# Toptachamann/Linear_Programming_Solver

Measured on AMD Instinct MI355X. Metric: simplex_pivots_per_sec, higher is better.
Workload: dtype f64

## Files before the change

### include/lpx.h

```cpp
#ifndef LPX_H
#define LPX_H

#include <stddef.h>
#include <stdint.h>

#ifdef __cplusplus
extern "C" {
#endif

#define LPX_ABI_VERSION 5

typedef enum lpx_status {
  LPX_OPTIMAL = 0,
  LPX_UNBOUNDED = 1,
  LPX_INFEASIBLE = 2,
  LPX_AUX_UNBOUNDED = 3,
  LPX_NO_DEGENERATE_PIVOT = 4,
  LPX_BAD_ARGUMENT = 5,
  LPX_RESTORE_INDEX_FAULT = 6,
  LPX_DEVICE_ERROR = 7,
  LPX_DIVIDE_BY_ZERO = 8,
  LPX_PIVOT_LIMIT = 9
} lpx_status;

const char* lpx_status_message(int status);
const char* lpx_last_error(void);
int lpx_abi_version(void);
int lpx_device_count(void);

typedef struct lpx_state lpx_state;

int lpx_state_create(int32_t m_local, int32_t n, const double* A, int64_t lda, const double* b,
                     const double* c, double v, const int32_t* perm, int32_t row0, int32_t m_global,
                     int device, lpx_state** out);
int lpx_state_create_from_device(int32_t m_local, int32_t n, const double* dA, int64_t lda,
                                 const double* db, const double* dc, double v, const int32_t* perm,
                                 int32_t row0, int32_t m_global, int device, lpx_state** out);
void lpx_state_destroy(lpx_state* s);
int lpx_state_set_stream(lpx_state* s, void* hip_stream);

int lpx_state_use_masked_stream(lpx_state* s, int32_t reserve_units, void** stream_out);

int lpx_state_set_pricing(lpx_state* s, int32_t pricing);

int lpx_get_entering(lpx_state* s, int32_t* entering);
int lpx_get_leaving(lpx_state* s, int32_t entering, int32_t* leaving, double* ratio);
int lpx_pivot(lpx_state* s, int32_t entering, int32_t leaving);

typedef enum lpx_option {
  LPX_OPT_BLOCK = 0,
  LPX_OPT_CHAIN = 1,
  LPX_OPT_OVERLAP = 2,
  LPX_OPT_OVERLAP_SERIAL = 3,
  LPX_OPT_OVERLAP_MASK = 4,
  LPX_OPT_CHAIN_WGS = 5,
  LPX_OPT_CHAIN_FENCES = 6,
  LPX_OPT_SWEEP_ROWS = 7,
  LPX_OPT_NT = 8,
  LPX_OPT_BATCH = 9,
  LPX_OPT_CHAIN_TRACE = 10,
  LPX_OPT_UPDATE_U = 11,
  LPX_OPT_UPDATE_ROWS = 12,
  LPX_OPT_A2_OFFSET = 13,
  LPX_OPT_SWEEP_FORM = 14,
  LPX_OPT_MULTI_ONEHOP = 15,
  LPX_OPT_SWEEP_CUS = 16,
  LPX_OPT_CHAIN_CUS = 17,
  LPX_OPT_FUSED = 18,
  LPX_OPT_CHAIN_FORM = 19,
  LPX_OPT_FIXUP_SIDE = 20,
  LPX_OPT_COUNT = 21
} lpx_option;
int lpx_state_set_option(lpx_state* s, int32_t key, int64_t value);
int lpx_state_get_option(const lpx_state* s, int32_t key, int64_t* value);

typedef struct lpx_state_info {
  int32_t block;
  int32_t chain_wgs;
  int32_t chain_wgs_requested;
  int32_t chain_resident_max;
  int32_t chain_blocks_per_cu;
  int32_t chain_stream_masked;
  int32_t chain_xcd_mask;
  int32_t sweep_xcd_mask;
  int32_t overlapped;
  int32_t nontemporal;
  int32_t sweep_rows;
  int32_t sweep_kernel;
  int32_t multi_onehop;
  int32_t sweep_clock_mhz;
  int32_t sweep_cus;
  int32_t arith_fused;
} lpx_state_info;
int lpx_state_get_info(lpx_state* s, lpx_state_info* out);
const char* lpx_sweep_kernel_name(int32_t code);
int lpx_state_read_chain_trace(lpx_state* s, int64_t* ticks, int32_t cap, int32_t* ndecisions);
int lpx_state_read_chain_trace_fine(lpx_state* s, int64_t* ticks, int32_t cap, int32_t* ndecisions, int32_t* stamps);

int lpx_state_set_block(lpx_state* s, int32_t pivots_per_sweep);
int lpx_state_get_block(const lpx_state* s);

int lpx_simplex_loop(lpx_state* s, int64_t max_pivots, int64_t* pivots_done, int32_t* status,
                     int32_t* track_slot);

int lpx_state_read(lpx_state* s, double* A, int64_t lda, double* b, double* c, double* v,
                   int32_t* perm);
int lpx_state_dims(const lpx_state* s, int32_t* m_local, int32_t* n, int32_t* row0, int32_t* m_global);
int lpx_state_checksum(lpx_state* s, uint64_t out[3]);

int lpx_profile_enable(lpx_state* s, int enable);
int lpx_profile_read(lpx_state* s, int64_t* launches, double* total_ms);

#define LPX_CAND_HEADER 8
int lpx_shard_begin(lpx_state* s, int64_t max_pivots, int32_t track_slot);
int lpx_shard_propose(lpx_state* s, double* d_candidate);
int lpx_shard_commit(lpx_state* s, const double* d_gathered, int32_t nranks);
int lpx_shard_probe(lpx_state* s, const double* d_gathered, int32_t nranks);
int lpx_shard_set_comm_stream(lpx_state* s, void* hip_stream);
int lpx_shard_set_pipeline(lpx_state* s, int32_t mode);
int lpx_shard_peek(lpx_state* s, double* d_candidate, int32_t slot, int32_t pending);
int lpx_shard_decide(lpx_state* s, const double* d_gathered, int32_t nranks, int32_t slot);
int lpx_shard_update(lpx_state* s, int32_t slot);
int lpx_shard_block_peek(lpx_state* s, double* d_candidate, int32_t slot);
int lpx_shard_block_decide(lpx_state* s, const double* d_gathered, int32_t nranks, int32_t slot);
int lpx_shard_block_sweep(lpx_state* s, int32_t nslots);
#define LPX_RUNNING (-1)
int lpx_shard_poll(lpx_state* s, int64_t* pivots_done, int32_t* status);

typedef struct lpx_solve_result {
  int32_t status;
  int32_t phase1_used;
  double objective;
  double objective_rounded;
  char objective_text[64];
  int64_t pivots_phase1;
  int64_t pivots_phase2;
  int32_t x0_slot;
  int32_t reserved;
  double seconds_total;
  double seconds_pivots;
} lpx_solve_result;

typedef struct lpx_solve_options {
  int32_t device;
  int32_t has_variable_names;
  int64_t max_pivots;
  const int32_t* restore_order;
  int32_t* perm_out;
  double* x_out;
  lpx_state** keep_state;
  int32_t pricing;
  int32_t restore_order_len;
  int32_t fused;
  int32_t reserved;
} lpx_solve_options;

int lpx_solve(int32_t m, int32_t n, const double* A, int64_t lda, const double* b, const double* c,
              int32_t maximize, const lpx_solve_options* opts, lpx_solve_result* result);

#define LPX_MAX_DEVICES 8
typedef struct lpx_multi lpx_multi;
int lpx_multi_create(int32_t m, int32_t n, const double* A, int64_t lda, const double* b, const double* c, double v,
                     const int32_t* perm, const int32_t* devices, int32_t n_dev, lpx_multi** out);
void lpx_multi_destroy(lpx_multi* s);
int lpx_multi_set_option(lpx_multi* s, int32_t key, int64_t value);
int lpx_multi_set_pricing(lpx_multi* s, int32_t pricing);
int lpx_multi_get_entering(lpx_multi* s, int32_t* entering);
int lpx_multi_get_leaving(lpx_multi* s, int32_t entering, int32_t* leaving, double* ratio);
int lpx_multi_pivot(lpx_multi* s, int32_t entering, int32_t leaving);
int lpx_multi_simplex_loop(lpx_multi* s, int64_t max_pivots, int64_t* pivots_done, int32_t* status,
                           int32_t* track_slot);
int lpx_multi_read(lpx_multi* s, double* A, int64_t lda, double* b, double* c, double* v, int32_t* perm);
int lpx_multi_checksum(lpx_multi* s, uint64_t out[3]);
int lpx_multi_profile_enable(lpx_multi* s, int enable);
int lpx_multi_profile_read(lpx_multi* s, int32_t shard, int64_t* launches, double* total_ms);
int lpx_multi_get_info(lpx_multi* s, lpx_state_info* out);
int lpx_solve_multi(int32_t m, int32_t n, const double* A, int64_t lda, const double* b, const double* c,
                    int32_t maximize, const lpx_solve_options* opts, const int32_t* devices, int32_t n_dev,
                    lpx_solve_result* result);

#define LPX_BATCH_LDS_BYTES 163840
int64_t lpx_batch_lds_bytes(int32_t m, int32_t n);
int64_t lpx_batch_solve_lds_bytes(int32_t m, int32_t n);

typedef struct lpx_batch lpx_batch;
int lpx_batch_create(int32_t count, int32_t m_max, int32_t n_max, const int32_t* m, const int32_t* n,
                     const double* A, int64_t lda, int64_t strideA, const double* b, const double* c,
                     const double* v, const int32_t* perm, int device, lpx_batch** out);
void lpx_batch_destroy(lpx_batch* s);
int lpx_batch_set_option(lpx_batch* s, int32_t key, int64_t value);
int lpx_batch_set_pricing(lpx_batch* s, int32_t pricing);
int lpx_batch_simplex_loop(lpx_batch* s, int64_t max_pivots, int64_t* pivots_done, int32_t* status, int32_t* track_slot);
int lpx_batch_read(lpx_batch* s, int32_t index, double* A, int64_t lda, double* b, double* c, double* v, int32_t* perm);
int lpx_batch_count(const lpx_batch* s);
int lpx_batch_shape(const lpx_batch* s, int32_t index, int32_t* m, int32_t* n);
int lpx_batch_solve(lpx_batch* s, const int32_t* maximize, int64_t max_pivots, const int32_t* restore_order,
                    const int32_t* restore_order_len, lpx_solve_result* results);
int lpx_solve_batch(int32_t count, int32_t m_max, int32_t n_max, const int32_t* m, const int32_t* n,
                    const double* A, int64_t lda, int64_t strideA, const double* b, const double* c,
                    const int32_t* maximize, const lpx_solve_options* opts, lpx_solve_result* results,
                    int32_t* n_in_batch);

int lpx_batch_solutions(lpx_batch* s, double* x_out, int32_t* perm_out);
int lpx_solve_batch_all(int32_t count, int32_t m_max, int32_t n_max, const int32_t* m, const int32_t* n,
                        const double* A, int64_t lda, int64_t strideA, const double* b, const double* c,
                        const int32_t* maximize, const lpx_solve_options* opts, lpx_solve_result* results,
                        double* x_out, int32_t* perm_out, int32_t* n_in_batch);

typedef struct lpx_scenarios lpx_scenarios;
int lpx_scenarios_create(int32_t m, int32_t n, const double* A, int64_t lda, int device, lpx_scenarios** out);
void lpx_scenarios_destroy(lpx_scenarios* s);
int lpx_scenarios_set_option(lpx_scenarios* s, int32_t key, int64_t value);
int lpx_scenarios_set_pricing(lpx_scenarios* s, int32_t pricing);
int lpx_scenarios_solve(lpx_scenarios* s, int32_t count, const double* b, int64_t ldb, const double* c, int64_t ldc,
                        const int32_t* maximize, int64_t max_pivots, const int32_t* restore_order, int32_t restore_order_len,
                        lpx_solve_result* results, double* x_out, int32_t* perm_out);
int lpx_solve_scenarios(int32_t m, int32_t n, const double* A, int64_t lda, int32_t count, const double* b, int64_t ldb,
                        const double* c, int64_t ldc, const int32_t* maximize, const lpx_solve_options* opts,
                        lpx_solve_result* results, double* x_out, int32_t* perm_out);

#define LPX_ROUTE_COLD 0
#define LPX_ROUTE_PRIMAL 1
#define LPX_ROUTE_DUAL 2
int lpx_scenarios_set_basis(lpx_scenarios* s, const int32_t* basis, int32_t* crash_pivots_out);
// ... 20 lines not shown
```

### linear_programming_solver_amd/_lib.py

```python
import ctypes as C
import os

_HERE = os.path.dirname(os.path.abspath(__file__))
LIB_PATH = os.environ.get("LPX_LIB_PATH") or os.path.join(_HERE, "liblpx.so")

OPTIMAL, UNBOUNDED, INFEASIBLE, AUX_UNBOUNDED, NO_DEGENERATE_PIVOT, BAD_ARGUMENT, RESTORE_INDEX_FAULT, \
    DEVICE_ERROR, DIVIDE_BY_ZERO, PIVOT_LIMIT = range(10)
CAND_HEADER = 8
BATCH_LDS_BYTES = 163840
ROUTES = ("cold", "primal", "dual")
PRICING = {"reference": 0, "first-positive": 0, "dantzig": 1, 0: 0, 1: 1}

OPTIONS = {"block": 0, "chain": 1, "overlap": 2, "overlap_serial": 3, "overlap_mask": 4, "chain_wgs": 5,
           "chain_fences": 6, "sweep_rows": 7, "nt": 8, "batch": 9, "chain_trace": 10, "update_u": 11,
           "update_rows": 12, "a2_offset": 13, "sweep_form": 14, "multi_onehop": 15, "sweep_cus": 16, "chain_cus": 17,
           "fused": 18, "chain_form": 19, "fixup_side": 20}

DEFAULT_FUSED = None


def set_default_arithmetic(mode):
    global DEFAULT_FUSED
    if mode not in ("auto", "plain", "fused"):
        raise ValueError('arithmetic mode is "auto", "plain" or "fused"')
    prev = "auto" if DEFAULT_FUSED is None else "fused" if DEFAULT_FUSED else "plain"
    DEFAULT_FUSED = None if mode == "auto" else mode == "fused"
    return prev


dp = C.POINTER(C.c_double)
ip = C.POINTER(C.c_int32)
i64p = C.POINTER(C.c_int64)


class SolveResult(C.Structure):
    _fields_ = [
        ("status", C.c_int32),
        ("phase1_used", C.c_int32),
        ("objective", C.c_double),
        ("objective_rounded", C.c_double),
        ("objective_text", C.c_char * 64),
        ("pivots_phase1", C.c_int64),
        ("pivots_phase2", C.c_int64),
        ("x0_slot", C.c_int32),
        ("reserved", C.c_int32),
        ("seconds_total", C.c_double),
        ("seconds_pivots", C.c_double),
    ]


class StateInfo(C.Structure):
    _fields_ = [(k, C.c_int32) for k in (
        "block", "chain_wgs", "chain_wgs_requested", "chain_resident_max", "chain_blocks_per_cu",
        "chain_stream_masked", "chain_xcd_mask", "sweep_xcd_mask", "overlapped", "nontemporal", "sweep_rows",
        "sweep_kernel", "multi_onehop", "sweep_clock_mhz", "sweep_cus", "arith_fused")]


class SolveOptions(C.Structure):
    _fields_ = [
        ("device", C.c_int32),
        ("has_variable_names", C.c_int32),
        ("max_pivots", C.c_int64),
        ("restore_order", ip),
        ("perm_out", ip),
        ("x_out", dp),
        ("keep_state", C.POINTER(C.c_void_p)),
        ("pricing", C.c_int32),
        ("restore_order_len", C.c_int32),
        ("fused", C.c_int32),
        ("reserved", C.c_int32),
    ]


SYMBOLS = [
    ("lpx_status_message", C.c_char_p, [C.c_int]),
    ("lpx_last_error", C.c_char_p, []),
    ("lpx_abi_version", C.c_int, []),
    ("lpx_device_count", C.c_int, []),
    ("lpx_state_create", C.c_int, [C.c_int32, C.c_int32, dp, C.c_int64, dp, dp, C.c_double, ip, C.c_int32,
                                   C.c_int32, C.c_int, C.POINTER(C.c_void_p)]),
    ("lpx_state_create_from_device", C.c_int, [C.c_int32, C.c_int32, C.c_void_p, C.c_int64, C.c_void_p,
                                               C.c_void_p, C.c_double, ip, C.c_int32, C.c_int32, C.c_int,
                                               C.POINTER(C.c_void_p)]),
    ("lpx_state_destroy", None, [C.c_void_p]),
    ("lpx_state_set_stream", C.c_int, [C.c_void_p, C.c_void_p]),
    ("lpx_state_use_masked_stream", C.c_int, [C.c_void_p, C.c_int32, C.POINTER(C.c_void_p)]),
    ("lpx_state_set_pricing", C.c_int, [C.c_void_p, C.c_int32]),
    ("lpx_state_set_block", C.c_int, [C.c_void_p, C.c_int32]),
    ("lpx_state_get_block", C.c_int, [C.c_void_p]),
    ("lpx_state_set_option", C.c_int, [C.c_void_p, C.c_int32, C.c_int64]),
    ("lpx_state_get_option", C.c_int, [C.c_void_p, C.c_int32, i64p]),
    ("lpx_state_get_info", C.c_int, [C.c_void_p, C.POINTER(StateInfo)]),
    ("lpx_sweep_kernel_name", C.c_char_p, [C.c_int32]),
    ("lpx_state_read_chain_trace", C.c_int, [C.c_void_p, i64p, C.c_int32, ip]),
    ("lpx_state_read_chain_trace_fine", C.c_int, [C.c_void_p, i64p, C.c_int32, ip, ip]),
    ("lpx_get_entering", C.c_int, [C.c_void_p, ip]),
    ("lpx_get_leaving", C.c_int, [C.c_void_p, C.c_int32, ip, dp]),
    ("lpx_pivot", C.c_int, [C.c_void_p, C.c_int32, C.c_int32]),
    ("lpx_simplex_loop", C.c_int, [C.c_void_p, C.c_int64, i64p, ip, ip]),
    ("lpx_state_read", C.c_int, [C.c_void_p, dp, C.c_int64, dp, dp, dp, ip]),
    ("lpx_state_dims", C.c_int, [C.c_void_p, ip, ip, ip, ip]),
    ("lpx_state_checksum", C.c_int, [C.c_void_p, C.POINTER(C.c_uint64)]),
    ("lpx_profile_enable", C.c_int, [C.c_void_p, C.c_int]),
    ("lpx_profile_read", C.c_int, [C.c_void_p, i64p, dp]),
    ("lpx_shard_begin", C.c_int, [C.c_void_p, C.c_int64, C.c_int32]),
    ("lpx_shard_propose", C.c_int, [C.c_void_p, C.c_void_p]),
    ("lpx_shard_commit", C.c_int, [C.c_void_p, C.c_void_p, C.c_int32]),
    ("lpx_shard_probe", C.c_int, [C.c_void_p, C.c_void_p, C.c_int32]),
    ("lpx_shard_set_comm_stream", C.c_int, [C.c_void_p, C.c_void_p]),
    ("lpx_shard_set_pipeline", C.c_int, [C.c_void_p, C.c_int32]),
    ("lpx_shard_peek", C.c_int, [C.c_void_p, C.c_void_p, C.c_int32, C.c_int32]),
    ("lpx_shard_decide", C.c_int, [C.c_void_p, C.c_void_p, C.c_int32, C.c_int32]),
    ("lpx_shard_update", C.c_int, [C.c_void_p, C.c_int32]),
    ("lpx_shard_block_peek", C.c_int, [C.c_void_p, C.c_void_p, C.c_int32]),
    ("lpx_shard_block_decide", C.c_int, [C.c_void_p, C.c_void_p, C.c_int32, C.c_int32]),
    ("lpx_shard_block_sweep", C.c_int, [C.c_void_p, C.c_int32]),
    ("lpx_shard_poll", C.c_int, [C.c_void_p, i64p, ip]),
    ("lpx_multi_create", C.c_int, [C.c_int32, C.c_int32, dp, C.c_int64, dp, dp, C.c_double, ip, ip, C.c_int32,
                                   C.POINTER(C.c_void_p)]),
    ("lpx_multi_destroy", None, [C.c_void_p]),
    ("lpx_multi_set_option", C.c_int, [C.c_void_p, C.c_int32, C.c_int64]),
    ("lpx_multi_set_pricing", C.c_int, [C.c_void_p, C.c_int32]),
    ("lpx_multi_get_entering", C.c_int, [C.c_void_p, ip]),
    ("lpx_multi_get_leaving", C.c_int, [C.c_void_p, C.c_int32, ip, dp]),
    ("lpx_multi_pivot", C.c_int, [C.c_void_p, C.c_int32, C.c_int32]),
    ("lpx_multi_simplex_loop", C.c_int, [C.c_void_p, C.c_int64, i64p, ip, ip]),
    ("lpx_multi_read", C.c_int, [C.c_void_p, dp, C.c_int64, dp, dp, dp, ip]),
    ("lpx_multi_checksum", C.c_int, [C.c_void_p, C.POINTER(C.c_uint64)]),
    ("lpx_multi_profile_enable", C.c_int, [C.c_void_p, C.c_int]),
    ("lpx_multi_profile_read", C.c_int, [C.c_void_p, C.c_int32, i64p, dp]),
    ("lpx_multi_get_info", C.c_int, [C.c_void_p, C.POINTER(StateInfo)]),
    ("lpx_solve_multi", C.c_int, [C.c_int32, C.c_int32, dp, C.c_int64, dp, dp, C.c_int32, C.POINTER(SolveOptions),
                                  ip, C.c_int32, C.POINTER(SolveResult)]),
    ("lpx_solve", C.c_int, [C.c_int32, C.c_int32, dp, C.c_int64, dp, dp, C.c_int32, C.POINTER(SolveOptions),
                            C.POINTER(SolveResult)]),
    ("lpx_restore_initial_lp", C.c_int, [C.c_void_p, dp, C.c_int32, C.c_int32, ip, C.c_int32]),
    ("lpx_java_default_name_order", C.c_int, [C.c_int32, ip]),
    ("lpx_transpose", C.c_int, [C.c_int32, C.c_int32, dp, C.c_int64, dp, C.c_int64, C.c_int]),
    ("lpx_batch_lds_bytes", C.c_int64, [C.c_int32, C.c_int32]),
    ("lpx_batch_create", C.c_int, [C.c_int32, C.c_int32, C.c_int32, ip, ip, dp, C.c_int64, C.c_int64, dp, dp, dp, ip,
                                   C.c_int, C.POINTER(C.c_void_p)]),
    ("lpx_batch_destroy", None, [C.c_void_p]),
    ("lpx_batch_set_option", C.c_int, [C.c_void_p, C.c_int32, C.c_int64]),
    ("lpx_batch_set_pricing", C.c_int, [C.c_void_p, C.c_int32]),
    ("lpx_batch_simplex_loop", C.c_int, [C.c_void_p, C.c_int64, i64p, ip, ip]),
    ("lpx_batch_read", C.c_int, [C.c_void_p, C.c_int32, dp, C.c_int64, dp, dp, dp, ip]),
    ("lpx_batch_count", C.c_int, [C.c_void_p]),
    ("lpx_solve_batch", C.c_int, [C.c_int32, C.c_int32, C.c_int32, ip, ip, dp, C.c_int64, C.c_int64, dp, dp, ip,
                                  C.POINTER(SolveOptions), C.POINTER(SolveResult), ip]),
    ("lpx_batch_solve_lds_bytes", C.c_int64, [C.c_int32, C.c_int32]),
    ("lpx_batch_shape", C.c_int, [C.c_void_p, C.c_int32, ip, ip]),
    ("lpx_batch_solutions", C.c_int, [C.c_void_p, dp, ip]),
    ("lpx_batch_solve", C.c_int, [C.c_void_p, ip, C.c_int64, ip, ip, C.POINTER(SolveResult)]),
    ("lpx_solve_batch_all", C.c_int, [C.c_int32, C.c_int32, C.c_int32, ip, ip, dp, C.c_int64, C.c_int64, dp, dp, ip,
                                      C.POINTER(SolveOptions), C.POINTER(SolveResult), dp, ip, ip]),
    ("lpx_scenarios_create", C.c_int, [C.c_int32, C.c_int32, dp, C.c_int64, C.c_int, C.POINTER(C.c_void_p)]),
    ("lpx_scenarios_destroy", None, [C.c_void_p]),
    ("lpx_scenarios_set_option", C.c_int, [C.c_void_p, C.c_int32, C.c_int64]),
    ("lpx_scenarios_set_pricing", C.c_int, [C.c_void_p, C.c_int32]),
    ("lpx_scenarios_solve", C.c_int, [C.c_void_p, C.c_int32, dp, C.c_int64, dp, C.c_int64, ip, C.c_int64, ip, C.c_int32,
                                      C.POINTER(SolveResult), dp, ip]),
    ("lpx_solve_scenarios", C.c_int, [C.c_int32, C.c_int32, dp, C.c_int64, C.c_int32, dp, C.c_int64, dp, C.c_int64, ip,
                                      C.POINTER(SolveOptions), C.POINTER(SolveResult), dp, ip]),
    ("lpx_scenarios_set_basis", C.c_int, [C.c_void_p, ip, ip]),
    ("lpx_scenarios_resolve", C.c_int, [C.c_void_p, C.c_int32, dp, C.c_int64, dp, C.c_int64, ip, C.c_int64, ip, C.c_int32,
                                        C.POINTER(SolveResult), dp, ip, ip]),
    ("lpx_solve_scenarios_from_basis", C.c_int, [C.c_int32, C.c_int32, dp, C.c_int64, ip, C.c_int32, dp, C.c_int64, dp,
                                                 C.c_int64, ip, C.POINTER(SolveOptions), C.POINTER(SolveResult), dp, ip,
                                                 ip]),
# ... 30 lines not shown
```

### linear_programming_solver_amd/csrc/lpx_dispatch.cpp

```cpp
#include "lpx_kernels.h"

#include <algorithm>

namespace lpxk {

#define LPX_PICK(B, f) ((B).fused ? fused::f : plain::f)

void launch_entering(const Buffers& B, int n, hipStream_t s, const LoopStart& start) { LPX_PICK(B, launch_entering)(B, n, s, start); }
void launch_entering_dantzig(const Buffers& B, int n, bool seed, hipStream_t s, const LoopStart& start) {
  LPX_PICK(B, launch_entering_dantzig)(B, n, seed, s, start);
}
void launch_ratio_gather(const Buffers& B, int m_local, int row0, const Geometry& g, int forced_e, hipStream_t s) {
  LPX_PICK(B, launch_ratio_gather)(B, m_local, row0, g, forced_e, s);
}
void launch_reduce_partials(const Buffers& B, const Geometry& g, hipStream_t s) {
  LPX_PICK(B, launch_reduce_partials)(B, g, s);
}
void launch_select_pivot(const Buffers& B, int n, int m_global, const Geometry& g, int forced_e, int forced_l,
                         hipStream_t s) {
  LPX_PICK(B, launch_select_pivot)(B, n, m_global, g, forced_e, forced_l, s);
}
void launch_update(const Buffers& B, int m_local, int n, int row0, const Geometry& g, bool nontemporal,
                   const double* prow, const LpxCtl* up, double* A_out, double* b_out, hipStream_t s) {
  LPX_PICK(B, launch_update)(B, m_local, n, row0, g, nontemporal, prow, up, A_out, b_out, s);
}
void launch_propose(const Buffers& B, int n, int row0, int m_local, const Geometry& g, double* d_candidate,
                    hipStream_t s) {
  LPX_PICK(B, launch_propose)(B, n, row0, m_local, g, d_candidate, s);
}
void launch_commit(const Buffers& B, int n, int m_global, const double* d_gathered, int nranks, double* prow,
                   LpxCtl* up, int up_parity, hipStream_t s) {
  LPX_PICK(B, launch_commit)(B, n, m_global, d_gathered, nranks, prow, up, up_parity, s);
}
void launch_peek(const Buffers& B, int n, int m_local, int row0, const double* prow_t, const double* col_t,
                 double* col_next, const LpxCtl* pend, double* d_candidate, hipStream_t s) {
  LPX_PICK(B, launch_peek)(B, n, m_local, row0, prow_t, col_t, col_next, pend, d_candidate, s);
}
void launch_block_peek(const Buffers& B, const BlockRing& R, int n, int m_local, int row0, int np, double* d_candidate,
                       hipStream_t s) {
  LPX_PICK(B, launch_block_peek)(B, R, n, m_local, row0, np, d_candidate, s);
}
void launch_block_decide(const Buffers& B, const BlockRing& R, int n, int m_global, const double* d_gathered, int nranks,
                         int slot, hipStream_t s) {
  LPX_PICK(B, launch_block_decide)(B, R, n, m_global, d_gathered, nranks, slot, s);
}
int launch_block_chain(const Buffers& B, const BlockRing& R, int n, int m, int nb, int half, int old_half, int n_old,
                       int b_from_tableau, int seq, int dantzig, int wgs, int fences, bool trace, LpxCtl* host_snap,
                       hipStream_t s, const MgPeers* mg, hipEvent_t stop) {
  return LPX_PICK(B, launch_block_chain)(B, R, n, m, nb, half, old_half, n_old, b_from_tableau, seq, dantzig, wgs, fences, trace,
                                  host_snap, s, mg, stop);
}
void preload_block_kernels(const Buffers& B, const BlockRing& R, hipStream_t s) {
  plain::preload_block_kernels(B, R, s);
  fused::preload_block_kernels(B, R, s);
}
unsigned* sweep_fail_word(const BlockRing& R, int64_t ld) { return plain::sweep_fail_word(R, ld); }
int64_t sweep_ticket_slots(int64_t ld) { return plain::sweep_ticket_slots(ld); }
int chain_blocks_per_cu() { return std::min(plain::chain_blocks_per_cu(), fused::chain_blocks_per_cu()); }
const char* sweep_kernel_name(int code) { return plain::sweep_kernel_name(code); }
int launch_block_sweep(const Buffers& B, const BlockRing& R, int n, int m_local, int row0, int K, int rows_per_wg,
                       bool nt, hipStream_t s, const double* A_src, const double* b_src, hipEvent_t after_sweep, int cus,
                       int form, int* kernel_used, const FixSide* side, hipEvent_t stop, hipEvent_t before_sweep) {
  return LPX_PICK(B, launch_block_sweep)(B, R, n, m_local, row0, K, rows_per_wg, nt, s, A_src, b_src, after_sweep, cus,
                                         form, kernel_used, side, stop, before_sweep);
}
void launch_fill_column(double* A, int64_t ld, int m, int col, double value, hipStream_t s) {
  plain::launch_fill_column(A, ld, m, col, value, s);
}
void launch_drop_column(double* A, int64_t ld, int m, int n_old, int col, hipStream_t s) {
  plain::launch_drop_column(A, ld, m, n_old, col, s);
}
void launch_restore_objective(const Buffers& B, int n, const RestoreEntry* d_entries, int n_entries, hipStream_t s) {
  LPX_PICK(B, launch_restore_objective)(B, n, d_entries, n_entries, s);
}
void launch_checksum(const Buffers& B, int m_local, int n, int row0, unsigned long long* d_out3, hipStream_t s) {
  plain::launch_checksum(B, m_local, n, row0, d_out3, s);
}
hipError_t launch_batch_simplex(const BatchArgs& a, hipStream_t s) {
  return a.fused ? fused::launch_batch_simplex(a, s) : plain::launch_batch_simplex(a, s);
}
int batch_blocks_per_cu(int threads, int lds_bytes) {
  return std::min(plain::batch_blocks_per_cu(threads, lds_bytes), fused::batch_blocks_per_cu(threads, lds_bytes));
}
hipError_t launch_batch_solve(const BatchSolveArgs& a, hipStream_t s) {
  return a.fused ? fused::launch_batch_solve(a, s) : plain::launch_batch_solve(a, s);
}
int batch_solve_blocks_per_cu(int threads, int lds_bytes) {
  return std::min(plain::batch_solve_blocks_per_cu(threads, lds_bytes), fused::batch_solve_blocks_per_cu(threads, lds_bytes));
}
hipError_t launch_batch_scenarios(const BatchScenarioArgs& a, hipStream_t s) {
  return a.fused ? fused::launch_batch_scenarios(a, s) : plain::launch_batch_scenarios(a, s);
}
int batch_scenarios_blocks_per_cu(int threads, int lds_bytes) {
  return std::min(plain::batch_scenarios_blocks_per_cu(threads, lds_bytes), fused::batch_scenarios_blocks_per_cu(threads, lds_bytes));
}
hipError_t launch_scenarios_crash(const ScenarioCrashArgs& a, hipStream_t s) {
  return a.fused ? fused::launch_scenarios_crash(a, s) : plain::launch_scenarios_crash(a, s);
}
hipError_t launch_batch_resolve(const BatchResolveArgs& a, hipStream_t s) {
  return a.fused ? fused::launch_batch_resolve(a, s) : plain::launch_batch_resolve(a, s);
}
int batch_resolve_blocks_per_cu(int threads, int lds_bytes) {
  return std::min(plain::batch_resolve_blocks_per_cu(threads, lds_bytes), fused::batch_resolve_blocks_per_cu(threads, lds_bytes));
}
void launch_transpose(const double* dA, int64_t lda, double* dAt, int64_t ldat, int m, int n, hipStream_t s) {
  plain::launch_transpose(dA, lda, dAt, ldat, m, n, s);
}

}
```

### linear_programming_solver_amd/csrc/lpx_engine.cpp

```cpp
#include <hip/hip_runtime.h>

#include <algorithm>
#include <chrono>
#include <cmath>
#include <cstdio>
#include <cstdlib>
#include <cstring>
#include <string>
#include <vector>

#include "../../include/lpx.h"
#include "lpx_kernels.h"
#include "lpx_internal.h"

using lpxk::Buffers;
using lpxk::Geometry;
using lpxk::LpxCtl;
using lpxk::RatioRow;

thread_local std::string g_last_error;

int fail(int status, const std::string& msg) {
  g_last_error = msg;
  return status;
}

extern "C" const char* lpx_status_message(int status) {
  switch (status) {
    case LPX_UNBOUNDED: return "This linear program is unbounded";
    case LPX_INFEASIBLE: return "This linear program is infeasible";
    case LPX_AUX_UNBOUNDED: return "Auxiliary lp is unbounded";
    case LPX_NO_DEGENERATE_PIVOT: return "Can't perform degenerate pivot";
    case LPX_BAD_ARGUMENT: return "IllegalArgumentException";
    case LPX_RESTORE_INDEX_FAULT: return "ArrayIndexOutOfBoundsException";
    case LPX_DEVICE_ERROR: return "HIP device error";
    case LPX_DIVIDE_BY_ZERO: return "Division by zero";
    default: return "";
  }
}

extern "C" const char* lpx_last_error(void) { return g_last_error.c_str(); }
extern "C" int lpx_abi_version(void) { return LPX_ABI_VERSION; }

extern "C" int lpx_device_count(void) {
  int n = 0;
  if (hipGetDeviceCount(&n) != hipSuccess) return -1;
  return n;
}

static int64_t round_up(int64_t x, int64_t q) { return (x + q - 1) / q * q; }

struct OptionSpec { const char* env; int64_t dflt, lo, hi; };
static const OptionSpec kOptionSpec[LPX_OPT_COUNT] = {
    {"LPX_BLOCK", 0, 0, lpxk::kBlockMax},
    {"LPX_CHAIN", 1, 0, 1},
    {"LPX_OVERLAP", 1, 0, 1},
    {"LPX_OVERLAP_SERIAL", 0, 0, 1},
    {"LPX_OVERLAP_MASK", 1, 0, 1},
    {"LPX_CHAIN_WGS", 0, 0, lpxk::kChainMaxWgs},
    {"LPX_CHAIN_FENCES", 2, 0, 3},
    {"LPX_SWEEP_ROWS", 0, 0, 8192},
    {"LPX_NT", -1, -1, 1},
    {"LPX_BATCH", 0, 0, 4096},
    {"LPX_CHAIN_TRACE", 0, 0, 1},
    {"LPX_U", 1, 1, 4},
    {"LPX_ROWS_PER_TILE", 2, 2, 256},
    {"LPX_A2_OFFSET", 512, 0, 1 << 20},
    {"LPX_SWEEP_FORM", 0, 0, 4},
    {"LPX_MULTI_ONEHOP", 0, 0, 1},
    {"LPX_SWEEP_CUS", 0, 0, 256},
    {"LPX_CHAIN_CUS", 0, 0, 16},
    {"LPX_FUSED", 2, 0, 2},
    {"LPX_CHAIN_FORM", 1, 0, 1},
    {"LPX_FIXUP_SIDE", 4, 0, 4},
};

static const int64_t* env_defaults() {
  static int64_t d[LPX_OPT_COUNT];
  static const bool once = [] {
    for (int k = 0; k < LPX_OPT_COUNT; k++) {
      const OptionSpec& sp = kOptionSpec[k];
      int64_t v = sp.dflt;
      const char* e = getenv(sp.env);
      if (e && *e) v = std::max(sp.lo, std::min(sp.hi, (int64_t)atoll(e)));
      d[k] = v;
    }
    return true;
  }();
  (void)once;
  return d;
}

void resolve_arithmetic(lpx_state* s) {
  const int64_t v = s->opt[LPX_OPT_FUSED];
  const double bytes = 8.0 * (double)s->m * (double)s->B.ld;
  const bool by_size = s->m == s->m_global && !s->multi_shard && bytes >= 0.5 * 1073741824.0;
  s->B.fused = v == 1 || (v == 2 && by_size);
}

static Geometry choose_geometry(int m, int64_t ld, const int64_t* opt) {
  Geometry g{};
  int U = (int)opt[LPX_OPT_UPDATE_U];
  if (U != 1 && U != 2 && U != 4) U = 1;
  g.U = U;
  const int W = 512 * U;
  g.nstrips = (int)((ld + W - 1) / W);
  int R = (int)opt[LPX_OPT_UPDATE_ROWS];
  if (R < 2) R = 2;
  if (R > 256) R = 256;
  if (R & 1) R += 1;
  g.rows_per_tile = R;
  g.ntiles = m > 0 ? (m + R - 1) / R : 0;
  return g;
}

static void apply_layout_options(lpx_state* s) {
  s->g = choose_geometry(s->m, s->B.ld, s->opt);
  const int64_t bytes = (int64_t)s->m * s->B.ld * 8;
  const int64_t nt = s->opt[LPX_OPT_NT];
  s->nontemporal = nt < 0 ? bytes > (192ll << 20) : nt != 0;
  s->info.nontemporal = s->nontemporal ? 1 : 0;
}

static int enqueue_ctl_fetch(lpx_state* s) {
  HIP_TRY(hipMemcpyAsync(s->h_ctl, s->B.ctl, sizeof(LpxCtl), hipMemcpyDeviceToHost, s->stream));
  unsigned* const fw = lpxk::sweep_fail_word(s->R, s->B.ld);
  unsigned* const h_fw = reinterpret_cast<unsigned*>(reinterpret_cast<char*>(s->h_ctl) + sizeof(LpxCtl));
  if (fw) HIP_TRY(hipMemcpyAsync(h_fw, fw, sizeof(unsigned), hipMemcpyDeviceToHost, s->stream));
  return 0;
}
static int check_fetched_fail_word(lpx_state* s) {
  unsigned* const fw = lpxk::sweep_fail_word(s->R, s->B.ld);
  unsigned* const h_fw = reinterpret_cast<unsigned*>(reinterpret_cast<char*>(s->h_ctl) + sizeof(LpxCtl));
  if (fw && *h_fw) {
    const unsigned f = *h_fw;
    *h_fw = 0;
    (void)hipMemset(fw, 0, sizeof(unsigned));
    return fail(LPX_DEVICE_ERROR, "k_sweep64_pull: a hand-over wait between the two stages hit its spin bound (code " +
                                      std::to_string(f) + "); the tableau of this handle is not valid");
  }
  return 0;
}
int sync_ctl_to_host(lpx_state* s) {
  if (int rc = enqueue_ctl_fetch(s)) return rc;
  HIP_TRY(hipStreamSynchronize(s->stream));
  return check_fetched_fail_word(s);
}

int push_ctl(lpx_state* s) {
  HIP_TRY(hipMemcpyAsync(s->B.ctl, s->h_ctl, sizeof(LpxCtl), hipMemcpyHostToDevice, s->stream));
  return 0;
}

static void free_block_ring(lpx_state* s) {
  (void)hipFree(s->R.prow);
  (void)hipFree(s->R.col);
  (void)hipFree(s->R.col0);
  (void)hipFree(s->R.row0);
  (void)hipFree(s->R.up);
  (void)hipFree(s->R.chain_part_a);
  (void)hipFree(s->R.chain_part_b);
  (void)hipFree(s->R.chain_bar);
  (void)hipFree(s->R.chain_own_col);
  (void)hipFree(s->R.chain_own_prow);
  (void)hipFree(s->R.chain_own_dvc);
  (void)hipFree(s->R.chain_own_b);
  (void)hipFree(s->R.chain_own_rs);
  (void)hipFree(s->R.chain_dbg);
  (void)hipFree(s->R.census);
  (void)hipFree(const_cast<double*>(s->R.zeros));
  (void)hipFree(s->R.tickets);
  (void)hipFree(s->R.sweep_fail);
  (void)hipFree(s->R.clk);
  (void)hipFree(s->R.col_packed);
  (void)hipFree(s->R.fix_col);
  (void)hipFree(s->R.fix_row);
  (void)hipFree(s->R.mg_mail);
  (void)hipFree(s->R.mg_arrive);
  (void)hipFree(s->R.mg_candrow);
  (void)hipFree(s->R.mg_arrive2);
  (void)hipFree(s->d_cand);
  s->R = lpxk::BlockRing{};
  s->d_cand = nullptr;
}

void free_state(lpx_state* s) {
  if (!s) return;
  (void)hipSetDevice(s->device);
  if (s->stream) (void)hipStreamSynchronize(s->stream);
  for (hipEvent_t e : s->ev) (void)hipEventDestroy(e);
  (void)hipFree(s->A_base[0]);
  (void)hipFree(s->A_base[1]);
  (void)hipFree(s->b_base[0]);
  (void)hipFree(s->b_base[1]);
  (void)hipFree(s->B.c);
  (void)hipFree(s->B.prow);
  (void)hipFree(s->B.col[0]);
  (void)hipFree(s->B.col[1]);
  (void)hipFree(s->B.partial);
  (void)hipFree(s->B.perm);
  (void)hipFree(s->B.ctl);
  (void)hipFree(s->d_sum);
  (void)hipFree(s->ring);
  (void)hipFree(s->prow2);
  free_block_ring(s);
  if (s->ev_upd) (void)hipEventDestroy(s->ev_upd);

  if (s->ev_peek) (void)hipEventDestroy(s->ev_peek);
  if (s->ev_decide) (void)hipEventDestroy(s->ev_decide);
  if (s->h_ctl) (void)hipHostFree(s->h_ctl);
  if (s->h_snap) (void)hipHostFree(s->h_snap);
  for (hipEvent_t e : s->ev_batch) if (e) (void)hipEventDestroy(e);
  if (s->ov_chain) (void)hipStreamDestroy(s->ov_chain);
  if (s->ov_sweep) (void)hipStreamDestroy(s->ov_sweep);
  for (hipEvent_t e : s->ev_ov_chain) if (e) (void)hipEventDestroy(e);
  for (hipEvent_t e : s->ev_ov_sweep) if (e) (void)hipEventDestroy(e);
  for (hipEvent_t e : s->ev_ov_join) if (e) (void)hipEventDestroy(e);
  for (hipStream_t t : s->ov_fix) if (t) (void)hipStreamDestroy(t);
  for (hipEvent_t e : s->ev_ov_fix) if (e) (void)hipEventDestroy(e);
  for (hipEvent_t e : s->ev_ov_pack) if (e) (void)hipEventDestroy(e);
  if (s->own_stream) (void)hipStreamDestroy(s->own_stream);
  delete s;
}

int alloc_state(int32_t m_local, int32_t n, int32_t n_cap, int32_t row0, int32_t m_global, int device,
                       lpx_state** out) {
  if (m_local < 0 || n < 0 || n_cap < n || row0 < 0 || m_global < m_local || row0 + m_local > m_global)
    return fail(LPX_BAD_ARGUMENT, "lpx_state_create: bad dimensions");
  int ndev = 0;
  HIP_TRY(hipGetDeviceCount(&ndev));
  if (device < 0 || device >= ndev) return fail(LPX_BAD_ARGUMENT, "lpx_state_create: no such device");
  HIP_TRY(hipSetDevice(device));
  lpx_state* s = new lpx_state();
  s->device = device;
  s->m = m_local; s->n = n; s->n_cap = n_cap; s->row0 = row0; s->m_global = m_global;
  const int64_t ld = std::max<int64_t>(16, round_up(n_cap, 16));
  const int64_t mp = std::max<int64_t>(2, round_up(m_local, 2)) + 2;
  s->B.ld = ld;
  memcpy(s->opt, env_defaults(), sizeof s->opt);
  resolve_arithmetic(s);
  s->B.chain_form = (int)s->opt[LPX_OPT_CHAIN_FORM];
  apply_layout_options(s);
#define ALLOC(ptr, count, type)                                                            \
  do {                                                                                     \
    hipError_t _e = hipMalloc((void**)&(ptr), std::max<size_t>(1, (size_t)(count)) * sizeof(type)); \
    if (_e != hipSuccess) { free_state(s); return fail(LPX_DEVICE_ERROR, std::string("hipMalloc: ") + hipGetErrorString(_e)); } \
    _e = hipMemset((ptr), 0, std::max<size_t>(1, (size_t)(count)) * sizeof(type));          \
    if (_e != hipSuccess) { free_state(s); return fail(LPX_DEVICE_ERROR, std::string("hipMemset: ") + hipGetErrorString(_e)); } \
  } while (0)
  ALLOC(s->B.A, mp * ld, double);
  s->A_base[0] = s->B.A;
  ALLOC(s->B.b, mp, double);
  s->b_base[0] = s->B.b;
  ALLOC(s->B.c, ld, double);
  ALLOC(s->B.prow, ld, double);
  ALLOC(s->B.col[0], mp, double);
  ALLOC(s->B.col[1], mp, double);
  ALLOC(s->B.partial, std::max(1, (m_local + 1) / 2 + 1), RatioRow);
  ALLOC(s->B.perm, (int64_t)n_cap + m_global, int32_t);
  ALLOC(s->B.ctl, 1, LpxCtl);
  ALLOC(s->d_sum, 4, unsigned long long);
  ALLOC(s->ring, 2, LpxCtl);
  ALLOC(s->prow2, ld, double);
#undef ALLOC
  hipError_t e = hipHostMalloc((void**)&s->h_ctl, sizeof(LpxCtl) + 16, hipHostMallocDefault);
  if (e != hipSuccess) { free_state(s); return fail(LPX_DEVICE_ERROR, "hipHostMalloc failed"); }
  memset(s->h_ctl, 0, sizeof(LpxCtl) + 16);
  if (hipHostMalloc((void**)&s->h_snap, 2 * sizeof(LpxCtl), hipHostMallocDefault) != hipSuccess ||
      hipEventCreateWithFlags(&s->ev_batch[0], hipEventDisableTiming) != hipSuccess ||
      hipEventCreateWithFlags(&s->ev_batch[1], hipEventDisableTiming) != hipSuccess) {
    free_state(s);
    return fail(LPX_DEVICE_ERROR, "pinned snapshot / event allocation failed");
  }
  e = hipStreamCreateWithFlags(&s->own_stream, hipStreamNonBlocking);
  if (e != hipSuccess) { free_state(s); return fail(LPX_DEVICE_ERROR, "hipStreamCreate failed"); }
  s->stream = s->own_stream;
  if (hipEventCreateWithFlags(&s->ev_peek, hipEventDisableTiming) != hipSuccess ||
      hipEventCreateWithFlags(&s->ev_upd, hipEventDisableTiming) != hipSuccess ||
      hipEventCreateWithFlags(&s->ev_decide, hipEventDisableTiming) != hipSuccess) {
    free_state(s);
    return fail(LPX_DEVICE_ERROR, "hipEventCreate failed");
  }
  HIP_TRY(hipDeviceSynchronize());
  *out = s;
  return 0;
}

void init_ctl(lpx_state* s, double v) {
  LpxCtl& c = *s->h_ctl;
  memset(&c, 0, sizeof c);
  c.v = v;
  c.e_next = -1; c.e_cur = -1; c.l = -1;
  c.status = lpxk::kRunning;
  c.track = -1;
  c.max_pivots = -1;
  c.e_min = INT32_MAX;
  c.ticket = 0;
}

int upload_common(lpx_state* s, const double* A, int64_t lda, const double* b, const double* c, double v,
                         const int32_t* perm, hipMemcpyKind kind) {
  const int32_t m = s->m, n = s->n;
  if (m > 0 && n > 0) {
    if (lda < n) return fail(LPX_BAD_ARGUMENT, "lpx_state_create: lda < n");
    HIP_TRY(hipMemcpy2DAsync(s->B.A, s->B.ld * sizeof(double), A, lda * sizeof(double), (size_t)n * sizeof(double),
                             (size_t)m, kind, s->stream));
  }
  if (m > 0) HIP_TRY(hipMemcpyAsync(s->B.b, b, (size_t)m * sizeof(double), kind, s->stream));
  if (n > 0) HIP_TRY(hipMemcpyAsync(s->B.c, c, (size_t)n * sizeof(double), kind, s->stream));
  std::vector<int32_t> p((size_t)n + s->m_global);
  for (size_t i = 0; i < p.size(); i++) p[i] = perm ? perm[i] : (int32_t)i;
  if (!p.empty())
    HIP_TRY(hipMemcpyAsync(s->B.perm, p.data(), p.size() * sizeof(int32_t), hipMemcpyHostToDevice, s->stream));
  init_ctl(s, v);
  if (int rc = push_ctl(s)) return rc;
  HIP_TRY(hipStreamSynchronize(s->stream));
  return 0;
}

extern "C" int lpx_state_create(int32_t m_local, int32_t n, const double* A, int64_t lda, const double* b,
                                const double* c, double v, const int32_t* perm, int32_t row0, int32_t m_global,
                                int device, lpx_state** out) {
  if (!out) return fail(LPX_BAD_ARGUMENT, "lpx_state_create: out is NULL");
  *out = nullptr;
  if ((m_local > 0 && n > 0 && !A) || (m_local > 0 && !b) || (n > 0 && !c))
    return fail(LPX_BAD_ARGUMENT, "lpx_state_create: NULL array");
  lpx_state* s = nullptr;
  if (int rc = alloc_state(m_local, n, n, row0, m_global, device, &s)) return rc;
  if (int rc = upload_common(s, A, lda, b, c, v, perm, hipMemcpyHostToDevice)) { free_state(s); return rc; }
  *out = s;
  return 0;
}

extern "C" int lpx_state_create_from_device(int32_t m_local, int32_t n, const double* dA, int64_t lda,
                                            const double* db, const double* dc, double v, const int32_t* perm,
                                            int32_t row0, int32_t m_global, int device, lpx_state** out) {
  if (!out) return fail(LPX_BAD_ARGUMENT, "lpx_state_create_from_device: out is NULL");
  *out = nullptr;
  if ((m_local > 0 && n > 0 && !dA) || (m_local > 0 && !db) || (n > 0 && !dc))
    return fail(LPX_BAD_ARGUMENT, "lpx_state_create_from_device: NULL array");
  lpx_state* s = nullptr;
  if (int rc = alloc_state(m_local, n, n, row0, m_global, device, &s)) return rc;
  if (int rc = upload_common(s, dA, lda, db, dc, v, perm, hipMemcpyDeviceToDevice)) { free_state(s); return rc; }
  *out = s;
  return 0;
}

extern "C" void lpx_state_destroy(lpx_state* s) { free_state(s); }

extern "C" int lpx_state_set_stream(lpx_state* s, void* hip_stream) {
  if (!s) return fail(LPX_BAD_ARGUMENT, "NULL state");
  HIP_TRY(hipSetDevice(s->device));
  HIP_TRY(hipStreamSynchronize(s->stream));
  s->stream = hip_stream ? (hipStream_t)hip_stream : s->own_stream;
  return 0;
}

extern "C" int lpx_state_dims(const lpx_state* s, int32_t* m_local, int32_t* n, int32_t* row0, int32_t* m_global) {
  if (!s) return fail(LPX_BAD_ARGUMENT, "NULL state");
  if (m_local) *m_local = s->m;
  if (n) *n = s->n;
  if (row0) *row0 = s->row0;
  if (m_global) *m_global = s->m_global;
  return 0;
}

int launch_update_profiled(lpx_state* s, const double* prow, const LpxCtl* up,
                                  const Buffers* Bin, double* A_out, double* b_out) {
  if (!prow) prow = s->B.prow;
  if (!up) up = s->B.ctl;
  const Buffers& BB = Bin ? *Bin : s->B;
  if (s->prof > 0 && (s->prof_seq++ % s->prof) == 0) {
    if (s->ev_used + 2 > s->ev.size()) {
// ... 33 lines not shown
  if (int rc = drain_profile(s)) return rc;
  s->prof = enable > 0 ? enable : 0;
  s->prof_seq = 0;
  s->prof_launches = 0;
  s->prof_ms = 0.0;
  return 0;
}

extern "C" int lpx_profile_read(lpx_state* s, int64_t* launches, double* total_ms) {
  if (!s) return fail(LPX_BAD_ARGUMENT, "NULL state");
  HIP_TRY(hipSetDevice(s->device));
  if (int rc = drain_profile(s)) return rc;
  if (launches) *launches = s->prof_launches;
  if (total_ms) *total_ms = s->prof_ms;
  s->prof_launches = 0;
  s->prof_ms = 0.0;
  return 0;
}

void launch_seed_entering(lpx_state* s, const lpxk::LoopStart& start) {
  if (s->pricing == 1) lpxk::launch_entering_dantzig(s->B, s->n, true, s->stream, start);
  else lpxk::launch_entering(s->B, s->n, s->stream, start);
}

extern "C" int lpx_state_set_pricing(lpx_state* s, int32_t pricing) {
  if (!s || (pricing != 0 && pricing != 1)) return fail(LPX_BAD_ARGUMENT, "lpx_state_set_pricing: bad argument");
  s->pricing = pricing;
  return 0;
}

static int require_single(lpx_state* s, const char* who) {
  if (!s) return fail(LPX_BAD_ARGUMENT, std::string(who) + ": NULL state");
  if (s->row0 != 0 || s->m_global != s->m)
    return fail(LPX_BAD_ARGUMENT, std::string(who) + ": not available on a row-block shard");
  return 0;
}

int set_running(lpx_state* s, int64_t max_pivots, int32_t track) {
  if (int rc = sync_ctl_to_host(s)) return rc;
  s->h_ctl->status = lpxk::kRunning;
  s->h_ctl->do_update = 0;
  s->h_ctl->pivots = 0;
  s->h_ctl->max_pivots = max_pivots;
  s->h_ctl->track = track;
  s->h_ctl->e_min = INT32_MAX;
  s->h_ctl->ticket = 0;
  return push_ctl(s);
}

extern "C" int lpx_get_entering(lpx_state* s, int32_t* entering) {
  if (!s || !entering) return fail(LPX_BAD_ARGUMENT, "lpx_get_entering: NULL argument");
  HIP_TRY(hipSetDevice(s->device));
  if (int rc = set_running(s, -1, -1)) return rc;
  launch_seed_entering(s);
  HIP_TRY(hipGetLastError());
  if (int rc = sync_ctl_to_host(s)) return rc;
  *entering = s->h_ctl->e_next;
  return 0;
}

extern "C" int lpx_get_leaving(lpx_state* s, int32_t entering, int32_t* leaving, double* ratio) {
  if (!s || !leaving) return fail(LPX_BAD_ARGUMENT, "lpx_get_leaving: NULL argument");
  if (!(entering >= 0 && entering < s->n))
    return fail(LPX_BAD_ARGUMENT, "lpx_get_leaving: entering outside [0, n)");
  HIP_TRY(hipSetDevice(s->device));
  if (int rc = set_running(s, -1, -1)) return rc;
  lpxk::launch_ratio_gather(s->B, s->m, s->row0, s->g, entering, s->stream);
  lpxk::launch_reduce_partials(s->B, s->g, s->stream);
  HIP_TRY(hipGetLastError());
  if (int rc = sync_ctl_to_host(s)) return rc;
  *leaving = s->h_ctl->l;
  if (ratio) *ratio = s->h_ctl->ratio;
  return 0;
}

extern "C" int lpx_pivot(lpx_state* s, int32_t entering, int32_t leaving) {
  if (int rc = require_single(s, "lpx_pivot")) return rc;
  if (!(entering >= 0 && entering < s->n) || !(leaving >= 0 && leaving < s->m))
    return fail(LPX_BAD_ARGUMENT, "lpx_pivot: index out of range");
  HIP_TRY(hipSetDevice(s->device));
  if (int rc = set_running(s, -1, -1)) return rc;
  lpxk::launch_ratio_gather(s->B, s->m, s->row0, s->g, entering, s->stream);
  lpxk::launch_select_pivot(s->B, s->n, s->m_global, s->g, entering, leaving, s->stream);
  if (int rc = launch_update_profiled(s)) return rc;
  HIP_TRY(hipGetLastError());
  if (int rc = sync_ctl_to_host(s)) return rc;
  if (s->h_ctl->status == LPX_DIVIDE_BY_ZERO) return fail(LPX_DIVIDE_BY_ZERO, "lpx_pivot: pivot element is zero");
  return 0;
}

hipError_t peer_visible_malloc(const lpx_state* s, void** ptr, size_t bytes) {
  if (s->peer_written) return hipExtMallocWithFlags(ptr, bytes, hipDeviceMallocFinegrained);
  return hipMalloc(ptr, bytes);
}

int32_t state_n(const lpx_state* s) { return s->n; }

static int build_block_ring(lpx_state* s);
int ensure_block_ring(lpx_state* s) {
  if (s->R.prow) return 0;
  const int rc = build_block_ring(s);
  if (rc) {
    const std::string why = g_last_error;
    free_block_ring(s);
    if (s->peer_written) return fail(rc, (why + " (ring of a multi-GPU shard: peer-written buffers need fine-grained device memory)").c_str());
    g_last_error = why;
  }
  return rc;
}
static int build_block_ring(lpx_state* s) {
  const int64_t mp = std::max<int64_t>(2, round_up(s->m, 2)) + 2;
  s->R.mp = mp;
  const size_t K = 2 * lpxk::kBlockMax;
  HIP_TRY(peer_visible_malloc(s, (void**)&s->R.prow, K * (size_t)s->B.ld * sizeof(double)));
  HIP_TRY(peer_visible_malloc(s, &s->R.mg_mail, 2 * lpxk::kMaxDevices * 32));
  HIP_TRY(peer_visible_malloc(s, (void**)&s->R.mg_arrive, lpxk::kChainMaxWgs * sizeof(unsigned long long)));
  HIP_TRY(hipMemsetAsync(s->R.mg_mail, 0, 2 * lpxk::kMaxDevices * 32, s->stream));
  HIP_TRY(hipMemsetAsync(s->R.mg_arrive, 0, lpxk::kChainMaxWgs * sizeof(unsigned long long), s->stream));
  if (s->m != s->m_global || s->peer_written || s->multi_shard) {
    const size_t rows_bytes = 2 * (size_t)lpxk::kMaxDevices * (size_t)s->B.ld * sizeof(double);
    const size_t words_bytes = 2 * (size_t)lpxk::kMaxDevices * lpxk::kChainMaxWgs * sizeof(unsigned long long);
    HIP_TRY(peer_visible_malloc(s, (void**)&s->R.mg_candrow, rows_bytes));
    HIP_TRY(peer_visible_malloc(s, (void**)&s->R.mg_arrive2, words_bytes));
    HIP_TRY(hipMemsetAsync(s->R.mg_candrow, 0, rows_bytes, s->stream));
    HIP_TRY(hipMemsetAsync(s->R.mg_arrive2, 0, words_bytes, s->stream));
  }
  HIP_TRY(hipMalloc((void**)&s->R.col, K * (size_t)mp * sizeof(double)));
  HIP_TRY(hipMalloc((void**)&s->R.col0, K * (size_t)mp * sizeof(double)));
  HIP_TRY(hipMalloc((void**)&s->R.row0, K * (size_t)s->B.ld * sizeof(double)));
  HIP_TRY(hipMemsetAsync(s->R.col0, 0, K * (size_t)mp * sizeof(double), s->stream));
  HIP_TRY(hipMemsetAsync(s->R.row0, 0, K * (size_t)s->B.ld * sizeof(double), s->stream));
  HIP_TRY(hipMalloc((void**)&s->R.up, K * sizeof(LpxCtl)));
  HIP_TRY(hipMalloc(&s->R.chain_part_a, 2 * lpxk::kChainMaxWgs * 64));
  HIP_TRY(hipMemsetAsync(s->R.chain_part_a, 0, 2 * lpxk::kChainMaxWgs * 64, s->stream));
  HIP_TRY(hipMalloc(&s->R.chain_part_b, lpxk::kChainMaxWgs * 16));
  HIP_TRY(hipMalloc((void**)&s->R.chain_bar, 512));
  HIP_TRY(hipMemsetAsync(s->R.chain_bar, 0, 512, s->stream));
  HIP_TRY(hipMalloc((void**)&s->R.chain_own_col, K * (size_t)mp * sizeof(double)));
  HIP_TRY(hipMalloc((void**)&s->R.chain_own_prow, K * (size_t)s->B.ld * sizeof(double)));
  HIP_TRY(hipMalloc((void**)&s->R.chain_own_dvc, K * (size_t)mp * sizeof(double)));
  HIP_TRY(hipMalloc((void**)&s->R.chain_own_b, (size_t)mp * sizeof(double)));
  HIP_TRY(hipMalloc((void**)&s->R.chain_own_rs, (size_t)(mp + s->B.ld) * sizeof(int32_t)));
  HIP_TRY(hipMemsetAsync(s->R.chain_own_rs, 0xff, (size_t)(mp + s->B.ld) * sizeof(int32_t), s->stream));
  HIP_TRY(hipMemsetAsync(s->R.chain_own_col, 0, K * (size_t)mp * sizeof(double), s->stream));
  HIP_TRY(hipMemsetAsync(s->R.chain_own_prow, 0, K * (size_t)s->B.ld * sizeof(double), s->stream));
  HIP_TRY(hipMalloc((void**)&s->R.chain_dbg, 16 * lpxk::kBlockMax * sizeof(long long)));
  HIP_TRY(hipMemsetAsync(s->R.chain_dbg, 0, 16 * lpxk::kBlockMax * sizeof(long long), s->stream));
  HIP_TRY(hipMalloc((void**)&s->R.census, (lpxk::kChainMaxWgs + 2 + 1200) * sizeof(unsigned)));
  HIP_TRY(hipMemsetAsync(s->R.census, 0, (lpxk::kChainMaxWgs + 2 + 1200) * sizeof(unsigned), s->stream));
  HIP_TRY(hipMalloc((void**)&s->R.zeros, 256));
  HIP_TRY(hipMemsetAsync(const_cast<double*>(s->R.zeros), 0, 256, s->stream));
  HIP_TRY(hipMalloc((void**)&s->R.tickets, 2 * (size_t)lpxk::sweep_ticket_slots(s->B.ld) * 128));
  HIP_TRY(hipMemsetAsync(s->R.tickets, 0, 2 * (size_t)lpxk::sweep_ticket_slots(s->B.ld) * 128, s->stream));
  HIP_TRY(hipMalloc((void**)&s->R.sweep_fail, 128));
  HIP_TRY(hipMemsetAsync(s->R.sweep_fail, 0, 128, s->stream));
  HIP_TRY(hipMalloc((void**)&s->R.clk, 256));
  HIP_TRY(hipMemsetAsync(s->R.clk, 0, 256, s->stream));
  HIP_TRY(hipMalloc((void**)&s->R.col_packed, 2 * (size_t)(mp / 4 + 1) * 4 * lpxk::kColPackedRowBytes));
  HIP_TRY(hipMemsetAsync(s->R.col_packed, 0, 2 * (size_t)(mp / 4 + 1) * 4 * lpxk::kColPackedRowBytes, s->stream));
  HIP_TRY(hipMalloc((void**)&s->d_cand, (size_t)(LPX_CAND_HEADER + s->B.ld) * sizeof(double)));
  HIP_TRY(hipMemsetAsync(s->R.prow, 0, K * (size_t)s->B.ld * sizeof(double), s->stream));
  HIP_TRY(hipMemsetAsync(s->R.col, 0, K * (size_t)mp * sizeof(double), s->stream));
  HIP_TRY(hipMemsetAsync(s->R.up, 0, K * sizeof(LpxCtl), s->stream));
  HIP_TRY(hipMemsetAsync(s->d_cand, 0, (size_t)(LPX_CAND_HEADER + s->B.ld) * sizeof(double), s->stream));
  lpxk::preload_block_kernels(s->B, s->R, s->stream);
  return 0;
}

int ensure_spare_tableau(lpx_state* s) {
  if (s->A2) return 0;
  const int64_t mp = std::max<int64_t>(2, round_up(s->m, 2)) + 2;
  const int64_t off = s->opt[LPX_OPT_A2_OFFSET];
  HIP_TRY(hipMalloc((void**)&s->A_base[1], (size_t)(mp * s->B.ld + off) * sizeof(double)));
  s->A2 = s->A_base[1] + off;
  HIP_TRY(hipMalloc((void**)&s->b_base[1], (size_t)mp * sizeof(double)));
  s->b2 = s->b_base[1];
  HIP_TRY(hipMemset(s->A2, 0, (size_t)(mp * s->B.ld) * sizeof(double)));
  HIP_TRY(hipMemset(s->b2, 0, (size_t)mp * sizeof(double)));
  HIP_TRY(hipDeviceSynchronize());
  return 0;
}

constexpr double kBlock128MinSweepUs = 1400.0;
constexpr int64_t kBlock128MinBudget = 256;
int choose_block(const lpx_state* s, int64_t max_pivots) {
  int K = (int)s->opt[LPX_OPT_BLOCK];
  if (K == 0) {
    const double sweep_us = 16.0 * (double)s->m * (double)s->B.ld / 6.0e6;
    if (sweep_us < 6.3) K = s->R.prow ? 16 : 1;
    else if (sweep_us < 10.0) K = 16;
    else K = 32;
    if (sweep_us >= 2500.0 && s->m % 4 == 0 && s->B.ld >= 512) K = 64;
    if (s->B.fused && sweep_us >= 300.0 && s->m % 16 == 0 && s->B.ld >= 512 && s->m_global == s->m) K = 64;
    if (K == 64 && s->B.fused && sweep_us >= kBlock128MinSweepUs && s->B.ld % 512 == 0 && s->m_global == s->m && !s->multi_shard &&
        s->opt[LPX_OPT_CHAIN] != 0 && s->opt[LPX_OPT_OVERLAP] != 0 && (max_pivots < 0 || max_pivots >= kBlock128MinBudget))
      K = 128;
  }
#ifdef LPX_WITH_VARIANTS
  if (s->B.chain_form != 1) K = std::min(K, 64);
#endif
  if (!s->opt[LPX_OPT_CHAIN] || s->m_global != s->m) K = std::min(K, (int)lpxk::kShardBlockMax);
  return std::max(1, std::min(K, (int)lpxk::kBlockMax));
}

int block_len(int K, int64_t max_pivots, int64_t decided) {
  if (max_pivots < 0) return K;
  const int64_t room = max_pivots + 1 - decided;
  return (int)std::max<int64_t>(0, std::min<int64_t>(K, room));
}

int clamp_chain_wgs(lpx_state* s, int want, int cus) {
  const int per_cu = lpxk::chain_blocks_per_cu();
  const int cap = std::max(1, per_cu * std::max(1, cus));
  s->info.chain_blocks_per_cu = per_cu;
  s->info.chain_resident_max = cap;
  s->info.chain_wgs_requested = want;
  const int G = std::max(1, std::min(std::min(want, cap), (int)lpxk::kChainMaxWgs));
  s->info.chain_wgs = G;
  return G;
}

int device_cus(const lpx_state* s) {
  int ncu = 0;
  if (hipDeviceGetAttribute(&ncu, hipDeviceAttributeMultiprocessorCount, s->device) != hipSuccess) ncu = 0;
  return ncu;
}

int launch_sweep_profiled(lpx_state* s, int K, hipStream_t stream, const Buffers& B, const lpxk::BlockRing& R,
                                 const double* A_src, const double* b_src, const lpxk::FixSide* side, hipEvent_t stop) {
  const bool sample = s->prof > 0 && (s->prof_seq++ % s->prof) == 0;
  if (sample) {
    if (s->ev_used + 2 > s->ev.size()) {
      for (int k = 0; k < 512; k++) {
        hipEvent_t e;
        HIP_TRY(hipEventCreate(&e));
        s->ev.push_back(e);
      }
    }
  }
  const int cus = (stream == s->ov_sweep && s->ov_masked) ? s->ov_sweep_cus : device_cus(s);
  int kernel_used = 0;
  s->info.sweep_cus = cus;
  s->info.sweep_rows = lpxk::launch_block_sweep(B, R, s->n, s->m, s->row0, K, (int)s->opt[LPX_OPT_SWEEP_ROWS],
                                                s->nontemporal, stream, A_src, b_src,
                                                sample ? s->ev[s->ev_used + 1] : nullptr, cus,
                                                (int)s->opt[LPX_OPT_SWEEP_FORM], &kernel_used, side, stop,
                                                sample ? s->ev[s->ev_used] : nullptr);
  s->info.sweep_kernel = kernel_used;
  if (sample) s->ev_used += 2;
  HIP_TRY(hipGetLastError());
  return 0;
}
static int launch_sweep_profiled(lpx_state* s, int K) {
  return launch_sweep_profiled(s, K, s->stream, s->B, s->R, nullptr, nullptr, nullptr, nullptr);
}

lpxk::BlockRing ring_half(const lpx_state* s, int h) {
  lpxk::BlockRing R = s->R;
  const int64_t o = (int64_t)h * lpxk::kBlockMax;
  R.prow += o * s->B.ld;
  R.row0 += o * s->B.ld;
  R.col += o * R.mp;
  R.col0 += o * R.mp;
  if (R.fix_col) R.fix_col += o * R.mp;
  if (R.fix_row) R.fix_row += o * s->B.ld;
  if (R.col_packed) R.col_packed += (int64_t)h * (R.mp / 4 + 1) * (4 * lpxk::kColPackedRowBytes / sizeof(double));
  if (R.tickets) R.tickets += (int64_t)h * lpxk::sweep_ticket_slots(s->B.ld) * 32;
  R.up += o;
  return R;
}

#ifndef LPX_CHAIN_CUS_PER_XCD
#define LPX_CHAIN_CUS_PER_XCD 4
#endif
static int chain_cus_per_xcd(const lpx_state* s, int per_xcd) {
  int k = LPX_CHAIN_CUS_PER_XCD;
  const int64_t work = std::max<int64_t>(s->m, s->B.ld);
  const double bytes = 8.0 * (double)s->m * (double)s->B.ld;
  if (!s->multi_shard && work > 8192 && bytes <= 1.5 * 1073741824.0) k = 8;
  if (!s->multi_shard && work > 8192 && s->B.fused) k = 8;
  if (s->opt[LPX_OPT_CHAIN_CUS] > 0) k = std::max(4, (int)s->opt[LPX_OPT_CHAIN_CUS] / 4 * 4);
  return std::max(1, std::min(k, (per_xcd - 1) / 4 * 4));
}
int ensure_overlap_streams(lpx_state* s) {
  if (s->ov_chain) return 0;
  hipDeviceProp_t prop;
  HIP_TRY(hipGetDeviceProperties(&prop, s->device));
  const int ncu = prop.multiProcessorCount;
  const int per_xcd = ncu / 8;
  std::vector<uint32_t> m_sweep((ncu + 31) / 32, 0u), m_chain((ncu + 31) / 32, 0u);
  const int kChainCusPerXcd = chain_cus_per_xcd(s, per_xcd);
  int sweep_per_xcd = per_xcd - kChainCusPerXcd;
  if (s->opt[LPX_OPT_SWEEP_CUS] > 0) sweep_per_xcd = std::max(1, std::min(sweep_per_xcd, (int)s->opt[LPX_OPT_SWEEP_CUS] / 8));
  for (int cu = 0; cu < ncu; cu++) {
    if (cu / 8 >= per_xcd - kChainCusPerXcd) m_chain[cu / 32] |= 1u << (cu % 32);
    else if (cu / 8 < sweep_per_xcd) m_sweep[cu / 32] |= 1u << (cu % 32);
  }
  bool masked = false;
  if (s->opt[LPX_OPT_OVERLAP_MASK] != 0 && ncu >= 64) {
    masked = hipExtStreamCreateWithCUMask(&s->ov_chain, (uint32_t)m_chain.size(), m_chain.data()) == hipSuccess &&
             hipExtStreamCreateWithCUMask(&s->ov_sweep, (uint32_t)m_sweep.size(), m_sweep.data()) == hipSuccess;
    if (!masked) {
      (void)hipGetLastError();
      if (s->ov_chain) { (void)hipStreamDestroy(s->ov_chain); s->ov_chain = nullptr; }
      if (s->ov_sweep) { (void)hipStreamDestroy(s->ov_sweep); s->ov_sweep = nullptr; }
    }
  }
  if (!masked) {
    int lo = 0, hi = 0;
    HIP_TRY(hipDeviceGetStreamPriorityRange(&lo, &hi));
    HIP_TRY(hipStreamCreateWithPriority(&s->ov_chain, hipStreamNonBlocking, hi));
    HIP_TRY(hipStreamCreateWithFlags(&s->ov_sweep, hipStreamNonBlocking));
  }
  s->ov_masked = masked;
  s->ov_chain_cus = masked ? 8 * kChainCusPerXcd : ncu;
  s->ov_sweep_cus = masked ? 8 * sweep_per_xcd : ncu;
  for (int k = 0; k < 2; k++) {
    HIP_TRY(hipEventCreateWithFlags(&s->ev_ov_chain[k], hipEventDisableTiming));
    HIP_TRY(hipEventCreateWithFlags(&s->ev_ov_sweep[k], hipEventDisableTiming));
  }
  for (int k = 0; k < 3; k++) HIP_TRY(hipEventCreateWithFlags(&s->ev_ov_join[k], hipEventDisableTiming));
  return 0;
}

int ensure_fix_side(lpx_state* s, int mode) {
  if (mode < 1 || mode > 3) return fail(LPX_BAD_ARGUMENT, "ensure_fix_side: mode");
  const size_t K = 2 * lpxk::kBlockMax;
  if (!s->R.fix_col) {
    HIP_TRY(hipMalloc((void**)&s->R.fix_col, K * (size_t)s->R.mp * sizeof(double)));
    HIP_TRY(hipMemsetAsync(s->R.fix_col, 0, K * (size_t)s->R.mp * sizeof(double), s->stream));
  }
  if (!s->R.fix_row) {
    HIP_TRY(hipMalloc((void**)&s->R.fix_row, K * (size_t)s->B.ld * sizeof(double)));
    HIP_TRY(hipMemsetAsync(s->R.fix_row, 0, K * (size_t)s->B.ld * sizeof(double), s->stream));
  }
  for (int k = 0; k < 2; k++) {
    if (!s->ev_ov_fix[k]) HIP_TRY(hipEventCreateWithFlags(&s->ev_ov_fix[k], hipEventDisableTiming));
    if (!s->ev_ov_pack[k]) HIP_TRY(hipEventCreateWithFlags(&s->ev_ov_pack[k], hipEventDisableTiming));
  }
  if (s->ov_fix[mode]) return 0;
  bool made = false;
  if (s->ov_masked && mode != 3) {
    hipDeviceProp_t prop;
    HIP_TRY(hipGetDeviceProperties(&prop, s->device));
    const int ncu = prop.multiProcessorCount, per_xcd = ncu / 8;
    const int chain_per_xcd = s->ov_chain_cus / 8, sweep_per_xcd = s->ov_sweep_cus / 8;
    std::vector<uint32_t> mask((ncu + 31) / 32, 0u);
    for (int cu = 0; cu < ncu; cu++) {
      const bool chain_cu = cu / 8 >= per_xcd - chain_per_xcd, sweep_cu = !chain_cu && cu / 8 < sweep_per_xcd;
      if (mode == 1 ? sweep_cu : chain_cu) mask[cu / 32] |= 1u << (cu % 32);
    }
    made = hipExtStreamCreateWithCUMask(&s->ov_fix[mode], (uint32_t)mask.size(), mask.data()) == hipSuccess;
    if (!made) { (void)hipGetLastError(); s->ov_fix[mode] = nullptr; }
  }
  if (!made) HIP_TRY(hipStreamCreateWithFlags(&s->ov_fix[mode], hipStreamNonBlocking));
  return 0;
}

static int blocked_loop_overlapped(lpx_state* s, int K, int64_t max_pivots, const lpxk::LoopStart& start) {
  if (int rc = ensure_block_ring(s)) return rc;
  if (int rc = ensure_spare_tableau(s)) return rc;
  if (int rc = ensure_overlap_streams(s)) return rc;
  launch_seed_entering(s, start);
  HIP_TRY(hipEventRecord(s->ev_ov_join[0], s->stream));
  HIP_TRY(hipStreamWaitEvent(s->ov_chain, s->ev_ov_join[0], 0));
  HIP_TRY(hipStreamWaitEvent(s->ov_sweep, s->ev_ov_join[0], 0));
  LpxCtl* h2 = s->h_snap;
  LpxCtl* d_snap = nullptr;
  HIP_TRY(hipHostGetDevicePointer((void**)&d_snap, s->h_snap, 0));
  const int64_t work = std::max<int64_t>(s->m, s->B.ld);
  const int chain_cap = s->ov_masked ? std::max(32, s->ov_chain_cus) : 32;
  int auto_wgs = (int)std::min<int64_t>(chain_cap, std::max<int64_t>(1, (work + 255) / 256));
  if (s->pricing == 0 && auto_wgs >= 8) auto_wgs += 1;
  const int chain_wgs = clamp_chain_wgs(s, s->opt[LPX_OPT_CHAIN_WGS] > 0 ? (int)s->opt[LPX_OPT_CHAIN_WGS] : auto_wgs,
                                        s->ov_chain_cus);
  const int fences = (int)s->opt[LPX_OPT_CHAIN_FENCES];
  const bool trace = s->opt[LPX_OPT_CHAIN_TRACE] != 0;
  s->info.chain_stream_masked = s->ov_masked ? 1 : 0;
  s->info.overlapped = 1;
  double* Abuf[2] = {s->B.A, s->A2};
  double* bbuf[2] = {s->B.b, s->b2};
  int64_t decided = 0;
  int nb_prev = 0, nblk = 0;
  const bool serial = s->opt[LPX_OPT_OVERLAP_SERIAL] != 0;
  int fix_mode = serial ? 0 : (int)s->opt[LPX_OPT_FIXUP_SIDE];
  if (fix_mode == 4) fix_mode = 8.0 * (double)s->m * (double)s->B.ld >= 2.0 * 1073741824.0 ? 2 : 0;
  if (fix_mode > 0 && ensure_fix_side(s, fix_mode) != 0) {
    (void)hipGetLastError();
    fix_mode = 0;
  }
  auto issue_block = [&](int k) -> int {
    const int nb = block_len(K, max_pivots, decided);
    if (nb <= 0) return 1;
    const int h = k & 1;
    Buffers Brd = s->B;
    if (serial) {
      if (k >= 1) HIP_TRY(hipStreamWaitEvent(s->ov_chain, s->ev_ov_sweep[h ^ 1], 0));
      Brd.A = Abuf[h];
      Brd.b = bbuf[h];
      s->info.chain_wgs = lpxk::launch_block_chain(Brd, s->R, s->n, s->m, nb, h, h ^ 1, 0, 1, s->chain_seq++, s->pricing == 1,
                                                   chain_wgs, fences, trace, d_snap + h, s->ov_chain, nullptr, s->ev_ov_chain[h]);
    } else {
      if (k >= 2) HIP_TRY(hipStreamWaitEvent(s->ov_chain, s->ev_ov_sweep[h], 0));
      Brd.A = Abuf[k == 0 ? 0 : (k - 1) & 1];
      Brd.b = bbuf[k == 0 ? 0 : (k - 1) & 1];
      s->info.chain_wgs = lpxk::launch_block_chain(Brd, s->R, s->n, s->m, nb, h, h ^ 1, k > 0 ? nb_prev : 0, k == 0,
                                                   s->chain_seq++, s->pricing == 1, chain_wgs, fences, trace, d_snap + h,
                                                   s->ov_chain, nullptr, s->ev_ov_chain[h]);
    }
    s->chain_nb_last = nb;
    if (max_pivots >= 0 && decided == max_pivots) {
      decided += nb;
      return 0;
    }
    HIP_TRY(hipStreamWaitEvent(s->ov_sweep, s->ev_ov_chain[h], 0));
    Buffers Bdst = s->B;
    Bdst.A = Abuf[h ^ 1];
    Bdst.b = bbuf[h ^ 1];
    const lpxk::FixSide side{fix_mode > 0 ? s->ov_fix[fix_mode] : nullptr, s->ev_ov_chain[h], s->ev_ov_fix[h], s->ev_ov_pack[h]};
    if (int rc = launch_sweep_profiled(s, nb, s->ov_sweep, Bdst, ring_half(s, h), Abuf[h], bbuf[h], fix_mode > 0 ? &side : nullptr,
                                       s->ev_ov_sweep[h])) return rc;
    decided += nb;
    nb_prev = nb;
    nblk = k + 1;
    return 0;
  };
  int rc = issue_block(0);
  if (rc == 1) rc = 0;
  for (int k = 1; rc == 0; k++) {
    const int r = issue_block(k);
    if (r != 0 && r != 1) { rc = r; break; }
    hipError_t e = hipEventSynchronize(s->ev_ov_chain[(k - 1) & 1]);
    if (e != hipSuccess) { rc = fail(LPX_DEVICE_ERROR, hipGetErrorString(e)); break; }
    if (h2[(k - 1) & 1].status != lpxk::kRunning || r == 1) break;
  }
  (void)hipEventRecord(s->ev_ov_join[1], s->ov_chain);
  (void)hipEventRecord(s->ev_ov_join[2], s->ov_sweep);
  (void)hipStreamWaitEvent(s->stream, s->ev_ov_join[1], 0);
  (void)hipStreamWaitEvent(s->stream, s->ev_ov_join[2], 0);
  if (nblk & 1) {
    std::swap(s->B.A, s->A2);
    std::swap(s->B.b, s->b2);
  }
  if (rc == 0) rc = enqueue_ctl_fetch(s);
  hipError_t e2 = hipStreamSynchronize(s->stream);
  if (rc == 0 && e2 != hipSuccess) rc = fail(LPX_DEVICE_ERROR, hipGetErrorString(e2));
  return rc;
}

static int blocked_loop(lpx_state* s, int K, int64_t max_pivots, const lpxk::LoopStart& start) {
  const bool one_block = max_pivots >= 0 && max_pivots + 1 <= K;
  if (s->opt[LPX_OPT_CHAIN] != 0 && s->opt[LPX_OPT_OVERLAP] != 0 && s->row0 == 0 && s->m == s->m_global && !one_block) {
    if (s->A2 || ensure_spare_tableau(s) == 0) return blocked_loop_overlapped(s, K, max_pivots, start);
    (void)hipGetLastError();
    if (s->A_base[1]) { (void)hipFree(s->A_base[1]); s->A_base[1] = nullptr; }
    if (s->b_base[1]) { (void)hipFree(s->b_base[1]); s->b_base[1] = nullptr; }
    s->A2 = nullptr;
    s->b2 = nullptr;
  }
  if (int rc = ensure_block_ring(s)) return rc;
  launch_seed_entering(s, start);
  hipEvent_t* evs = s->ev_batch;
  LpxCtl* h2 = s->h_snap;
  int64_t decided = 0;
  const bool fused = s->opt[LPX_OPT_CHAIN] != 0 && s->row0 == 0 && s->m == s->m_global;
  const int64_t work = std::max<int64_t>(s->m, s->B.ld);
  const int auto_wgs = (int)std::min<int64_t>(64, std::max<int64_t>(1, (work + 255) / 256));
  const int chain_wgs = fused ? clamp_chain_wgs(s, s->opt[LPX_OPT_CHAIN_WGS] > 0 ? (int)s->opt[LPX_OPT_CHAIN_WGS] : auto_wgs,
                                                device_cus(s))
                              : 0;
  const int fences = (int)s->opt[LPX_OPT_CHAIN_FENCES];
  const bool trace = s->opt[LPX_OPT_CHAIN_TRACE] != 0;
  s->info.chain_stream_masked = 0;
  s->info.overlapped = 0;
  LpxCtl* d_snap = nullptr;
  if (fused) HIP_TRY(hipHostGetDevicePointer((void**)&d_snap, s->h_snap, 0));
  auto issue_block = [&](int slot) -> int {
    const int nb = block_len(K, max_pivots, decided);
    if (fused && nb > 0) {
      s->info.chain_wgs = lpxk::launch_block_chain(s->B, s->R, s->n, s->m, nb, 0, 0, 0, 1, s->chain_seq++, s->pricing == 1,
                                                   chain_wgs, fences, trace, d_snap + slot, s->stream);
      s->chain_nb_last = nb;
    } else {
      for (int k = 0; k < nb; k++) {
        lpxk::launch_block_peek(s->B, s->R, s->n, s->m, s->row0, k, s->d_cand, s->stream);
        lpxk::launch_block_decide(s->B, s->R, s->n, s->m_global, s->d_cand, 1, k, s->stream);
        if (s->pricing == 1) lpxk::launch_entering_dantzig(s->B, s->n, false, s->stream);
      }
    }
    const bool probe_only = max_pivots >= 0 && decided == max_pivots;
    decided += nb;
    if (nb > 0 && !probe_only) {
      if (int rc = launch_sweep_profiled(s, nb)) return rc;
    }
    if (!fused)
      HIP_TRY(hipMemcpyAsync(&h2[slot], s->B.ctl, sizeof(LpxCtl), hipMemcpyDeviceToHost, s->stream));
    HIP_TRY(hipEventRecord(evs[slot], s->stream));
    return 0;
  };
  int rc = issue_block(0);
  int cur = 0;
  while (rc == 0) {
    rc = issue_block(cur ^ 1);
    if (rc) break;
    hipError_t e = hipEventSynchronize(evs[cur]);
    if (e != hipSuccess) { rc = fail(LPX_DEVICE_ERROR, hipGetErrorString(e)); break; }
    if (h2[cur].status != lpxk::kRunning) break;
    cur ^= 1;
  }
  if (rc == 0) rc = enqueue_ctl_fetch(s);
  hipError_t e2 = hipStreamSynchronize(s->stream);
  if (rc == 0 && e2 != hipSuccess) rc = fail(LPX_DEVICE_ERROR, hipGetErrorString(e2));
  return rc;
}

extern "C" int lpx_state_get_block(const lpx_state* s) { return s ? choose_block(s, -1) : -1; }

extern "C" int lpx_shard_block_peek(lpx_state* s, double* d_candidate, int32_t slot) {
  if (!s || !d_candidate || slot < 0 || slot >= lpxk::kShardBlockMax)
    return fail(LPX_BAD_ARGUMENT, "lpx_shard_block_peek: bad argument");
  HIP_TRY(hipSetDevice(s->device));
  if (int rc = ensure_block_ring(s)) return rc;
  lpxk::launch_block_peek(s->B, s->R, s->n, s->m, s->row0, slot, d_candidate, s->stream);
  HIP_TRY(hipGetLastError());
  return 0;
}

extern "C" int lpx_shard_block_decide(lpx_state* s, const double* d_gathered, int32_t nranks, int32_t slot) {
  if (!s || !d_gathered || nranks < 1 || slot < 0 || slot >= lpxk::kShardBlockMax)
    return fail(LPX_BAD_ARGUMENT, "lpx_shard_block_decide: bad argument");
  HIP_TRY(hipSetDevice(s->device));
  if (int rc = ensure_block_ring(s)) return rc;
  lpxk::launch_block_decide(s->B, s->R, s->n, s->m_global, d_gathered, nranks, slot, s->stream);
  if (s->pricing == 1) lpxk::launch_entering_dantzig(s->B, s->n, false, s->stream);
  HIP_TRY(hipGetLastError());
  return 0;
}

extern "C" int lpx_shard_block_sweep(lpx_state* s, int32_t nslots) {
  if (!s || nslots < 0 || nslots > lpxk::kShardBlockMax) return fail(LPX_BAD_ARGUMENT, "lpx_shard_block_sweep: bad argument");
  HIP_TRY(hipSetDevice(s->device));
  if (nslots == 0) return 0;
  if (int rc = ensure_block_ring(s)) return rc;
  return launch_sweep_profiled(s, nslots);
}

extern "C" int lpx_state_set_block(lpx_state* s, int32_t pivots_per_sweep) {
  if (!s || pivots_per_sweep < 0 || pivots_per_sweep > lpxk::kBlockMax)
    return fail(LPX_BAD_ARGUMENT, "lpx_state_set_block: 0 (auto), 1 (off) .. 128");
  s->opt[LPX_OPT_BLOCK] = pivots_per_sweep;
  s->loop_block = 0;
  return 0;
}

extern "C" int lpx_state_set_option(lpx_state* s, int32_t key, int64_t value) {
  if (!s || key < 0 || key >= LPX_OPT_COUNT) return fail(LPX_BAD_ARGUMENT, "lpx_state_set_option: unknown option");
  const OptionSpec& sp = kOptionSpec[key];
  if (value < sp.lo || value > sp.hi) return fail(LPX_BAD_ARGUMENT, std::string("lpx_state_set_option: value out of range for ") + sp.env);
  if (key == LPX_OPT_UPDATE_U && value == 3) return fail(LPX_BAD_ARGUMENT, "lpx_state_set_option: UPDATE_U is 1, 2 or 4");
  if (key == LPX_OPT_A2_OFFSET && s->A2) return fail(LPX_BAD_ARGUMENT, "lpx_state_set_option: the second tableau exists already");
  if ((key == LPX_OPT_CHAIN_CUS || key == LPX_OPT_SWEEP_CUS) && s->ov_chain && value != s->opt[key])
    return fail(LPX_BAD_ARGUMENT, "lpx_state_set_option: the CU-masked stream pair of this handle exists already (set CHAIN_CUS / SWEEP_CUS before the first blocked loop)");
  s->opt[key] = value;
  s->loop_block = 0;
  if (key == LPX_OPT_CHAIN_FORM) s->B.chain_form = (int)value;
  if (key == LPX_OPT_FUSED) resolve_arithmetic(s);
  if (key == LPX_OPT_UPDATE_U || key == LPX_OPT_UPDATE_ROWS || key == LPX_OPT_NT) apply_layout_options(s);
  return 0;
}

extern "C" int lpx_state_get_option(const lpx_state* s, int32_t key, int64_t* value) {
  if (!s || !value || key < 0 || key >= LPX_OPT_COUNT) return fail(LPX_BAD_ARGUMENT, "lpx_state_get_option: bad argument");
  *value = s->opt[key];
  return 0;
}

extern "C" int lpx_state_get_info(lpx_state* s, lpx_state_info* out) {
  if (!s || !out) return fail(LPX_BAD_ARGUMENT, "lpx_state_get_info: NULL argument");
  HIP_TRY(hipSetDevice(s->device));
  s->info.block = s->loop_block > 0 ? s->loop_block : choose_block(s, -1);
  s->info.arith_fused = s->B.fused ? 1 : 0;
  s->info.chain_xcd_mask = 0;
  s->info.sweep_xcd_mask = 0;
  if (s->R.census) {
    HIP_TRY(hipStreamSynchronize(s->stream));
    std::vector<unsigned> h(lpxk::kChainMaxWgs + 2);
    HIP_TRY(hipMemcpy(h.data(), s->R.census, h.size() * sizeof(unsigned), hipMemcpyDeviceToHost));
    for (int w = 0; w < s->info.chain_wgs && w < (int)lpxk::kChainMaxWgs; w++)
      if (h[w]) s->info.chain_xcd_mask |= 1 << ((h[w] - 1) & 15);
    s->info.sweep_xcd_mask = (int32_t)h[lpxk::kChainMaxWgs];
  }
  s->info.sweep_clock_mhz = 0;
// ... 381 lines not shown
```

### linear_programming_solver_amd/csrc/lpx_internal.h

```cpp
#pragma once
#include <hip/hip_runtime.h>

#include <string>
#include <vector>

#include "../../include/lpx.h"
#include "lpx_kernels.h"

using lpxk::Buffers;
using lpxk::Geometry;
using lpxk::LpxCtl;
using lpxk::RatioRow;

int fail(int status, const std::string& msg);

#define HIP_TRY(expr)                                                                         \
  do {                                                                                        \
    hipError_t _e = (expr);                                                                   \
    if (_e != hipSuccess)                                                                     \
      return fail(LPX_DEVICE_ERROR, std::string(#expr) + ": " + hipGetErrorString(_e));       \
  } while (0)

struct DeviceRestore {
  int d = -1;
  DeviceRestore() { if (hipGetDevice(&d) != hipSuccess) { d = -1; (void)hipGetLastError(); } }
  ~DeviceRestore() { if (d >= 0) (void)hipSetDevice(d); }
};

struct lpx_state {
  int device = 0;
  hipStream_t own_stream = nullptr;
  hipStream_t stream = nullptr;
  int32_t m = 0;
  int32_t n = 0;
  int32_t row0 = 0, m_global = 0;
  int32_t n_cap = 0;
  Buffers B{};
  Geometry g{};
  bool nontemporal = false;
  int pricing = 0;
  int64_t opt[LPX_OPT_COUNT] = {};
  lpx_state_info info{};
  int loop_block = 0;
  int chain_nb_last = 0;
  bool peer_written = false;
  bool multi_shard = false;
  lpxk::BlockRing R{};
  int chain_seq = 0;
  hipStream_t ov_chain = nullptr, ov_sweep = nullptr;
  bool ov_masked = false;
  int ov_chain_cus = 0;
  int ov_sweep_cus = 0;
  hipEvent_t ev_ov_chain[2] = {nullptr, nullptr}, ev_ov_sweep[2] = {nullptr, nullptr}, ev_ov_join[3] = {nullptr, nullptr, nullptr};
  hipStream_t ov_fix[4] = {nullptr, nullptr, nullptr, nullptr};
  hipEvent_t ev_ov_fix[2] = {nullptr, nullptr};
  hipEvent_t ev_ov_pack[2] = {nullptr, nullptr};
  double* d_cand = nullptr;
  LpxCtl* h_ctl = nullptr;
  LpxCtl* h_snap = nullptr;
  hipEvent_t ev_batch[2] = {nullptr, nullptr};
  LpxCtl* ring = nullptr;
  double* prow2 = nullptr;
  hipStream_t comm_stream = nullptr;
  hipEvent_t ev_peek = nullptr, ev_decide = nullptr, ev_upd = nullptr;
  int pipeline = 1;
  double* A2 = nullptr;
  double* A_base[2] = {nullptr, nullptr};
  double* b_base[2] = {nullptr, nullptr};
  double* b2 = nullptr;
  bool upd_recorded = false;
  bool settled = true;
  unsigned long long* d_sum = nullptr;
  int prof = 0;
  int64_t prof_seq = 0;
  std::vector<hipEvent_t> ev;
  size_t ev_used = 0;
  int64_t prof_launches = 0;
  double prof_ms = 0.0;
};


int sync_ctl_to_host(lpx_state* s);
int push_ctl(lpx_state* s);
void free_state(lpx_state* s);
int alloc_state(int32_t m_local, int32_t n, int32_t n_cap, int32_t row0, int32_t m_global, int device, lpx_state** out);
int upload_common(lpx_state* s, const double* A, int64_t lda, const double* b, const double* c, double v,
                  const int32_t* perm, hipMemcpyKind kind);
void init_ctl(lpx_state* s, double v);
int set_running(lpx_state* s, int64_t max_pivots, int32_t track);
void resolve_arithmetic(lpx_state* s);
int ensure_block_ring(lpx_state* s);
int ensure_spare_tableau(lpx_state* s);
int ensure_overlap_streams(lpx_state* s);
hipError_t peer_visible_malloc(const lpx_state* s, void** ptr, size_t bytes);
int32_t state_n(const lpx_state* s);
int choose_block(const lpx_state* s, int64_t max_pivots = -1);
int block_len(int K, int64_t max_pivots, int64_t decided);
int clamp_chain_wgs(lpx_state* s, int want, int cus);
int device_cus(const lpx_state* s);
int launch_sweep_profiled(lpx_state* s, int K, hipStream_t stream, const Buffers& B, const lpxk::BlockRing& R,
                          const double* A_src, const double* b_src, const lpxk::FixSide* side = nullptr,
                          hipEvent_t stop = nullptr);
int ensure_fix_side(lpx_state* s, int mode);
lpxk::BlockRing ring_half(const lpx_state* s, int h);
void launch_seed_entering(lpx_state* s, const lpxk::LoopStart& start = lpxk::LoopStart{});
int launch_update_profiled(lpx_state* s, const double* prow = nullptr, const LpxCtl* up = nullptr,
                           const Buffers* Bin = nullptr, double* A_out = nullptr, double* b_out = nullptr);

int multi_create(int32_t m, int32_t n, int32_t n_cap, const double* A, int64_t lda, const double* b, const double* c,
                 double v, const int32_t* perm, const int32_t* devices, int32_t n_dev, lpx_multi** out);
namespace lpx_internal {
int multi_shards(lpx_multi* M);
lpx_state* multi_shard(lpx_multi* M, int r);
int multi_device(lpx_multi* M, int r);
int32_t multi_row_start(lpx_multi* M, int r);
int multi_owner(lpx_multi* M, int32_t row);
void multi_set_n(lpx_multi* M, int32_t n);
}
```

### linear_programming_solver_amd/csrc/lpx_kernels.h

```cpp
#pragma once
#include <hip/hip_runtime.h>
#include <stdint.h>

namespace lpxk {

constexpr int kRunning = -1;
constexpr double kEps = 1e-9;
constexpr double kInf = 1e50;

struct RatioRow {
  double ratio;
  int32_t row;
  int32_t pad;
};

struct LpxCtl {
  double v;
  double p;
  double bl;
  double pc;
  double ratio;
  int32_t e_next;
  int32_t e_cur;
  int32_t l;
  int32_t status;
  int32_t do_update;
  int32_t track;
  int32_t parity;
  int32_t e_min;
  int32_t ticket;
  int32_t reserved;
  int64_t pivots;
  int64_t max_pivots;
};

struct LoopStart { int32_t reset = 0; int32_t track = -1; int64_t max_pivots = -1; };

struct Geometry {
  int U;
  int rows_per_tile;
  int nstrips, ntiles;
};

struct Buffers {
  double* A;
  int64_t ld;
  double* b;
  double* c;
  double* prow;
  double* col[2];
  RatioRow* partial;
  int32_t* perm;
  LpxCtl* ctl;
  int chain_form;
  int fused;
};

constexpr int kBlockMax = 128;
constexpr int kShardBlockMax = 32;
constexpr int kChainMaxWgs = 256;
constexpr int kMaxDevices = 8;
struct BlockRing {
  double* prow;
  double* col;
  double* col0;
  double* row0;
  LpxCtl* up;
  int64_t mp;
  void* chain_part_a;
  void* chain_part_b;
  unsigned* chain_bar;
  double* chain_own_col;
  double* chain_own_prow;
  double* chain_own_dvc;
  double* chain_own_b;
  int32_t* chain_own_rs;
  long long* chain_dbg;
  unsigned* census;
  double* fix_col;
  double* fix_row;
  double* col_packed;
  unsigned* tickets;
  unsigned* sweep_fail;
  long long* clk;
  const double* zeros;
  void* mg_mail;
  unsigned long long* mg_arrive;
  double* mg_candrow;
  unsigned long long* mg_arrive2;
};
struct MgPeers {
  int n_dev, dev;
  int row0, m_global;
  int mail_slot0;
  void* mail[kMaxDevices];
  double* prow[kMaxDevices];
  unsigned long long* arrive[kMaxDevices];
  int onehop;
  double* candrow[kMaxDevices];
  unsigned long long* arrive2[kMaxDevices];
  unsigned spin_max;
};
enum SweepKernel { kSweepNone = 0, kSweepTiles = 1, kSweepMulti = 2, kSweepSteady = 3, kSweepPipe64 = 4, kSweepDma = 5, kSweepPull = 6, kSweepPull64 = 7, kSweepOne64 = 8, kSweepMfma64 = 9, kSweepMfma642 = 10, kSweepMfma128 = 11 };
struct FixSide { hipStream_t stream; hipEvent_t ready, done, packed; };
constexpr int kColPackedRowBytes = 1024;
constexpr int kSweep128Ranges = 3;
struct RestoreEntry { int32_t is_basic; int32_t index; double k; };

constexpr int kBatchLdsMax = 163840;
constexpr int kBatchScratchBytes = 512;
struct BatchLayout {
  int64_t ld, b, c, v, perm, image, col;
  int64_t lds_bytes;
};
__host__ __device__ inline BatchLayout batch_layout(int64_t m, int64_t n) {
  BatchLayout L;
  L.ld = n | 1;
  L.b = m * L.ld;
  L.c = L.b + m;
  L.v = L.c + n;
  L.perm = (L.v + 2) & ~(int64_t)1;
  L.image = L.perm + (((n + m + 1) / 2 + 1) & ~(int64_t)1);
  L.col = L.image;
  L.lds_bytes = 8 * (L.image + ((m + 1) & ~(int64_t)1)) + kBatchScratchBytes;
  return L;
}
struct BatchArgs {
  int32_t count;
  const int32_t* m;
  const int32_t* n;
  const int64_t* offset;
  double* image;
  int64_t* pivots;
  int32_t* status;
  int32_t* track;
  int64_t max_pivots;
  int32_t dantzig;
  int32_t fused;
  int32_t lds_bytes;
  int32_t threads;
};
struct BatchSolveLayout {
  BatchLayout aux;
  int64_t c0, order, slot;
  int64_t lds_bytes;
};
__host__ __device__ inline BatchSolveLayout batch_solve_layout(int64_t m, int64_t n) {
  BatchSolveLayout W;
  W.aux = batch_layout(m, n + 1);
  W.c0 = W.aux.lds_bytes / 8;
  W.order = W.c0 + ((n + 1) & ~(int64_t)1);
  W.slot = W.order + (n + 1) / 2;
  W.lds_bytes = 8 * (W.order + ((n + 1) & ~(int64_t)1));
  return W;
}
struct BatchSolveArgs {
  int32_t count;
  const int32_t* m;
  const int32_t* n;
  const int64_t* offset;
  double* image;
  const int32_t* maximize;
  const int32_t* phase1;
  const int32_t* order;
  const int32_t* order_len;
  int64_t order_pitch;
  int32_t* status;
  int32_t* phase1_used;
  int32_t* x0_slot;
  int32_t* n_final;
  int64_t* pivots1;
  int64_t* pivots2;
  double* v;
  int64_t max_pivots;
  int32_t dantzig;
  int32_t fused;
  int32_t lds_bytes;
  int32_t threads;
};
struct BatchScenarioArgs {
  int32_t count;
  int32_t m, n;
  const double* A;
  const double* b;
  const double* c;
  int64_t ldb, ldc;
  const int32_t* flags;
  const int32_t* order;
  int32_t order_len;
  int32_t* status;
  int32_t* phase1_used;
  int32_t* x0_slot;
  int32_t* n_final;
  int64_t* pivots1;
  int64_t* pivots2;
  double* v;
  double* x_out;
  int32_t* perm_out;
  int64_t max_pivots;
  int32_t dantzig;
  int32_t fused;
  int32_t lds_bytes;
  int32_t threads;
};
__host__ __device__ inline int64_t eta_stride(int64_t m, int64_t n) { return m + n + 4; }
struct ScenarioCrashArgs {
  int32_t count;
  int32_t m, n;
  const double* A;
  const int32_t* wanted;
  double* A_out;
  int32_t* perm_out;
  double* eta;
  int32_t* info;
  int32_t fused;
  int32_t lds_bytes;
  int32_t threads;
};
struct BatchResolveArgs : BatchScenarioArgs {
  const int32_t* perm0;
  const double* eta;
  int32_t n_eta;
  int32_t* route;
};

namespace plain {
#include "lpx_launchers.inc"
}
namespace fused {
#include "lpx_launchers.inc"
}
#include "lpx_launchers.inc"

}
```

### linear_programming_solver_amd/csrc/lpx_kernels.hip

```cpp
#include "lpx_kernels.h"

#include <hip/hip_ext.h>

#include <atomic>

#include <limits.h>
#include <stdint.h>
#include <stdlib.h>

#include <algorithm>
#include <type_traits>

#ifndef LPX_FUSED
#define LPX_FUSED 0
#endif

namespace lpxk {
#if LPX_FUSED
namespace fused {
#else
namespace plain {
#endif

typedef double d2 __attribute__((ext_vector_type(2)));
// ... 787 lines not shown
                     R.prow + (int64_t)slot * B.ld, B.perm, B.ctl, R.up + slot, 0);
}

int launch_block_chain(const Buffers& B, const BlockRing& R, int n, int m, int nb, int half, int old_half, int n_old,
                        int b_from_tableau, int seq, int dantzig, int wgs, int fences, bool trace, LpxCtl* host_snap,
                        hipStream_t s, const MgPeers* mg, hipEvent_t stop) {
  const int64_t work = std::max<int64_t>(m, B.ld);
  int G = wgs > 0 ? wgs : (int)std::min<int64_t>(64, std::max<int64_t>(1, (work + 511) / 512));
  G = std::max(1, std::min(G, kChainMaxWgs));
#ifdef LPX_WITH_VARIANTS
  const bool form2 = B.chain_form == 1 && (mg == nullptr || !mg->onehop);
#else
  const bool form2 = mg == nullptr || (B.chain_form == 1 && !mg->onehop);
#endif
  if (form2 && mg == nullptr) {
    const int64_t rows_wgs = (m + kChain2Threads - 1) / kChain2Threads;
    const int64_t cols_wgs = (std::max<int64_t>(B.ld - 256, 0) + kChain2Threads - 1) / kChain2Threads + 1;
    G = (int)std::max<int64_t>(1, std::min<int64_t>(G, std::max(rows_wgs, cols_wgs)));
  }
  const int64_t K = kBlockMax;
  const bool wide = nb > 32 || n_old > 32;
  const bool wide128 = nb > 64 || n_old > 64;
  ChainArgs P{};
  P.A = B.A; P.b = B.b; P.ld = B.ld; P.mp = R.mp; P.n = n; P.m = m;
  P.c = B.c; P.perm = B.perm; P.ctl = B.ctl;
  const int64_t ho = half * K, oo = old_half * K;
  P.prow = R.prow + ho * B.ld; P.col = R.col + ho * R.mp; P.col0 = R.col0 + ho * R.mp; P.row0 = R.row0 + ho * B.ld;
  P.own_col = R.chain_own_col + ho * R.mp; P.own_prow = R.chain_own_prow + ho * B.ld;
  P.own_dvc = R.chain_own_dvc + ho * R.mp; P.up = R.up + ho;
  P.prow_o = R.prow + oo * B.ld; P.col_o = R.col + oo * R.mp;
  P.own_col_o = R.chain_own_col + oo * R.mp; P.own_prow_o = R.chain_own_prow + oo * B.ld;
  P.own_dvc_o = R.chain_own_dvc + oo * R.mp; P.up_o = R.up + oo;
  P.n_old = n_old; P.own_b = R.chain_own_b; P.b_from_tableau = b_from_tableau; P.nb = nb;
  P.own_rs_a = R.chain_own_rs; P.own_rs_b = R.chain_own_rs + R.mp;
  P.partA = reinterpret_cast<ChainPart*>(R.chain_part_a); P.partB = reinterpret_cast<RatioRow*>(R.chain_part_b);
  P.bar = R.chain_bar + 32 * (seq & 1); P.bar_next = R.chain_bar + 32 * ((seq + 1) & 1);
  P.hand = reinterpret_cast<unsigned long long*>(R.chain_bar + 64);
  P.hand_base = (unsigned)(seq + 1) * (unsigned)kBlockMax;
  P.dantzig = dantzig; P.fences = fences; P.host_snap = host_snap; P.dbg = trace ? R.chain_dbg : nullptr;
  P.spin_max = (mg && mg->spin_max) ? mg->spin_max : (1u << 22);
#ifdef LPX_DIAG_BUILD
  static const int chain_diag = getenv("LPX_CHAIN_DIAG") ? atoi(getenv("LPX_CHAIN_DIAG")) : 0;
  P.diag = chain_diag;
#endif
  P.census = R.census;
  if (mg) {
    P.shard_row0 = mg->row0; P.m_global = mg->m_global; P.n_dev = mg->n_dev; P.dev = mg->dev;
    P.mail_slot0 = mg->mail_slot0;
    P.onehop = mg->onehop;
    for (int d = 0; d < mg->n_dev && d < kMaxDevices; ++d) {
      P.mail_peer[d] = reinterpret_cast<MgMail*>(mg->mail[d]);
      P.prow_peer[d] = mg->prow[d] + ho * B.ld;
      P.arrive_peer[d] = mg->arrive[d];
      P.candrow_peer[d] = mg->candrow[d];
      P.arrive2_peer[d] = mg->arrive2[d];
    }
    if (form2) {
      if (wide) LPX_LAUNCH_STOP((k_block_chain2_t<64, kChain2Threads, true>), dim3(G), dim3(kChain2Threads), s, stop, P);
      else LPX_LAUNCH_STOP((k_block_chain2_t<32, kChain2Threads, true>), dim3(G), dim3(kChain2Threads), s, stop, P);
    } else LPX_LAUNCH_STOP((k_block_chain_t<true, 32>), dim3(G), dim3(256), s, stop, P);
  } else if (form2) {
    P.m_global = m; P.n_dev = 1;
#ifdef LPX_CHAIN2_ONE_XCD
    G = std::min(G, 32);
    if (wide128) hipLaunchKernelGGL((k_block_decide128<kChain2Threads>), dim3(8 * G), dim3(kChain2Threads), 0, s, P);
    else if (wide) hipLaunchKernelGGL((k_block_chain2_t<64, kChain2Threads, false>), dim3(8 * G), dim3(kChain2Threads), 0, s, P);
    else hipLaunchKernelGGL((k_block_chain2_t<32, kChain2Threads, false>), dim3(8 * G), dim3(kChain2Threads), 0, s, P);
    if (stop) (void)hipEventRecord(stop, s);
#else
    if (wide128) LPX_LAUNCH_STOP((k_block_decide128<kChain2Threads>), dim3(G), dim3(kChain2Threads), s, stop, P);
    else if (wide) LPX_LAUNCH_STOP((k_block_chain2_t<64, kChain2Threads, false>), dim3(G), dim3(kChain2Threads), s, stop, P);
    else LPX_LAUNCH_STOP((k_block_chain2_t<32, kChain2Threads, false>), dim3(G), dim3(kChain2Threads), s, stop, P);
#endif
  } else {
#ifdef LPX_WITH_VARIANTS
    P.m_global = m; P.n_dev = 1;
    if (wide) LPX_LAUNCH_STOP((k_block_chain_t<false, 64>), dim3(G), dim3(256), s, stop, P);
    else LPX_LAUNCH_STOP((k_block_chain_t<false, 32>), dim3(G), dim3(256), s, stop, P);
#else
    if (stop) (void)hipEventRecord(stop, s);
#endif
  }
  return G;
}

int64_t sweep_ticket_slots(int64_t ld) { return kSweep128Ranges * std::max<int64_t>(ld / 64, 4) + 4; }
unsigned* sweep_fail_word(const BlockRing& R, int64_t ld) {
#ifdef LPX_WITH_VARIANTS
  (void)ld;
  return R.sweep_fail;
#else
  (void)R; (void)ld;
  return nullptr;
#endif
}

void preload_block_kernels(const Buffers& B, const BlockRing& R, hipStream_t s) {
  static std::atomic<unsigned> done{0};
  int dev = 0;
  if (hipGetDevice(&dev) != hipSuccess || dev < 0 || dev >= 32) return;
  if (done.fetch_or(1u << dev) & (1u << dev)) return;
  double* const A = B.A;
  const int64_t ld = B.ld;
  unsigned* const no_census = nullptr;
#define LPX_EACH_NT_OOP(X) X(true, true) X(true, false) X(false, true) X(false, false)
#define LPX_PRE_TILES(K_, NT_, OOP_) \
  hipLaunchKernelGGL((k_update_tiles<K_, NT_, OOP_>), dim3(1), dim3(256), 0, s, A, A, ld, 0, R.prow, R.col, R.mp, R.up, 0, 16, 1, no_census);
#define LPX_PRE_T2(NT_, OOP_) LPX_PRE_TILES(2, NT_, OOP_)
#define LPX_PRE_T4(NT_, OOP_) LPX_PRE_TILES(4, NT_, OOP_)
#define LPX_PRE_T8(NT_, OOP_) LPX_PRE_TILES(8, NT_, OOP_)
#define LPX_PRE_T16(NT_, OOP_) LPX_PRE_TILES(16, NT_, OOP_)
#define LPX_PRE_T32(NT_, OOP_) LPX_PRE_TILES(32, NT_, OOP_)
#define LPX_PRE_MULTI(NT_, OOP_) \
  hipLaunchKernelGGL((k_update_multi<32, NT_, OOP_>), dim3(1), dim3(256), 0, s, A, A, ld, 0, R.prow, R.col, R.mp, R.up, 0, 64, 1, no_census, 0, 0);
#define LPX_PRE_STEADY(NT_, OOP_) \
  hipLaunchKernelGGL((k_sweep32_steady<NT_, OOP_>), dim3(1), dim3(256), 0, s, A, A, ld, 0, R.prow, R.col, R.mp, R.up, 0, 48, 1);
#define LPX_PRE_PIPE(NT_, OOP_) \
  hipLaunchKernelGGL((k_sweep64_pipe<NT_, OOP_>), dim3(1), dim3(512), 0, s, A, A, ld, 0, R.prow, R.col, R.mp, R.up, 0, 48, 1);
#define LPX_PRE_DMA(NT_, OOP_) \
  hipLaunchKernelGGL((k_sweep32_dma<NT_, OOP_>), dim3(1), dim3(256), 0, s, A, A, ld, 0, R.prow, R.col, R.mp, R.up, 0, 2, 1, 1, R.zeros, 0);
  LPX_EACH_NT_OOP(LPX_PRE_T2) LPX_EACH_NT_OOP(LPX_PRE_T4) LPX_EACH_NT_OOP(LPX_PRE_T8) LPX_EACH_NT_OOP(LPX_PRE_T16)
  LPX_EACH_NT_OOP(LPX_PRE_T32) LPX_EACH_NT_OOP(LPX_PRE_MULTI)
#ifdef LPX_WITH_VARIANTS
  LPX_EACH_NT_OOP(LPX_PRE_STEADY) LPX_EACH_NT_OOP(LPX_PRE_PIPE) LPX_EACH_NT_OOP(LPX_PRE_DMA)
#endif
#define LPX_PRE_PULL(NT_, OOP_) \
  hipLaunchKernelGGL((k_sweep32_pull<NT_, OOP_>), dim3(1), dim3(256), 0, s, A, A, ld, 0, R.prow, R.col, R.mp, R.up, 0, 1, R.col_packed, R.tickets, (long long*)nullptr);
  if (R.tickets && R.col_packed) {
    LPX_EACH_NT_OOP(LPX_PRE_PULL)
    hipLaunchKernelGGL(k_pack_multipliers<32>, dim3(1), dim3(256), 0, s, R.col, R.mp, R.up, 0, 0, R.col_packed, R.tickets, 0, (long long*)nullptr);
    hipLaunchKernelGGL(k_pack_multipliers<64>, dim3(1), dim3(256), 0, s, R.col, R.mp, R.up, 0, 0, R.col_packed, R.tickets, 0, (long long*)nullptr);
#ifdef LPX_WITH_VARIANTS
#define LPX_PRE_PULL64(NT_, OOP_) \
    hipLaunchKernelGGL((k_sweep64_pull<NT_, OOP_>), dim3(1), dim3(256), 0, s, A, A, ld, 0, R.prow, R.up, 0, 1, R.col_packed, R.tickets, (sweep_fail_word)(R, ld));
    LPX_EACH_NT_OOP(LPX_PRE_PULL64)
#undef LPX_PRE_PULL64
#endif
#define LPX_PRE_ONE64(NT_, OOP_) \
    hipLaunchKernelGGL((k_sweep64_one<NT_, OOP_>), dim3(1), dim3(256), 0, s, A, A, ld, 0, R.prow, R.up, 0, 1, R.col_packed, R.tickets, (long long*)nullptr);
    LPX_EACH_NT_OOP(LPX_PRE_ONE64)
#undef LPX_PRE_ONE64
#if LPX_FUSED
    hipLaunchKernelGGL(k_pack_multipliers_mfma, dim3(1), dim3(256), 0, s, R.col, R.mp, R.up, 0, 0, R.col_packed, R.tickets, 0, (long long*)nullptr, 0);
#ifdef LPX_WITH_VARIANTS
#define LPX_PRE_MFMA64(NT_, OOP_) \
    hipLaunchKernelGGL((k_sweep64_mfma<NT_, OOP_>), dim3(1), dim3(256), 0, s, A, A, ld, 0, R.prow, R.up, 0, 1, R.col_packed, R.tickets);
    LPX_EACH_NT_OOP(LPX_PRE_MFMA64)
#undef LPX_PRE_MFMA64
#endif
#define LPX_PRE_MFMA642(NT_, OOP_) \
    hipLaunchKernelGGL((k_sweep64_mfma2<NT_, OOP_>), dim3(1), dim3(256), 0, s, A, A, ld, 0, R.prow, R.up, 0, 1, R.col_packed, R.tickets, 33, (long long*)nullptr);
    LPX_EACH_NT_OOP(LPX_PRE_MFMA642)
#undef LPX_PRE_MFMA642
    hipLaunchKernelGGL(k_pack_multipliers_mfma128, dim3(1), dim3(256), 0, s, R.col, R.mp, R.up, 0, 0, R.col_packed, R.tickets, 0, (long long*)nullptr);
#define LPX_PRE_MFMA128(NT_, OOP_) \
    hipLaunchKernelGGL((k_sweep128_mfma<NT_, OOP_>), dim3(1), dim3(256), 0, s, A, A, ld, 0, R.prow, R.up, 0, 0, R.col_packed, R.tickets, 1);
    LPX_EACH_NT_OOP(LPX_PRE_MFMA128)
#undef LPX_PRE_MFMA128
#endif
  }
#undef LPX_PRE_PULL
#undef LPX_PRE_DMA
#undef LPX_PRE_PIPE
#undef LPX_PRE_STEADY
#undef LPX_PRE_MULTI
#undef LPX_PRE_T32
#undef LPX_PRE_T16
#undef LPX_PRE_T8
#undef LPX_PRE_T4
#undef LPX_PRE_T2
#undef LPX_PRE_TILES
#undef LPX_EACH_NT_OOP
  hipLaunchKernelGGL(k_block_fixup, dim3(1, 1, 3), dim3(256), 0, s, A, ld, 0, 0, 0, B.b, R.prow, R.col, R.col0, R.row0,
                     R.mp, R.up, 0, B.b, (long long*)nullptr, (double*)nullptr, (double*)nullptr);
  hipLaunchKernelGGL(k_block_fixup_scatter, dim3(1, 1, 2), dim3(256), 0, s, A, ld, 0, 0, (const double*)nullptr, (const double*)nullptr,
                     R.mp, R.up, 0, (long long*)nullptr);
  ChainArgs P{};
  P.ctl = B.ctl; P.up = R.up; P.nb = 0;
  P.bar = R.chain_bar; P.bar_next = R.chain_bar + 32;
  P.spin_max = 1u << 22;
#ifdef LPX_WITH_VARIANTS
  hipLaunchKernelGGL((k_block_chain_t<false, 32>), dim3(1), dim3(256), 0, s, P);
  hipLaunchKernelGGL((k_block_chain_t<false, 64>), dim3(1), dim3(256), 0, s, P);
#endif
  hipLaunchKernelGGL((k_block_chain_t<true, 32>), dim3(1), dim3(256), 0, s, P);
  hipLaunchKernelGGL((k_block_chain2_t<32, kChain2Threads, false>), dim3(1), dim3(kChain2Threads), 0, s, P);
  hipLaunchKernelGGL((k_block_chain2_t<64, kChain2Threads, false>), dim3(1), dim3(kChain2Threads), 0, s, P);
  hipLaunchKernelGGL((k_block_chain2_t<32, kChain2Threads, true>), dim3(1), dim3(kChain2Threads), 0, s, P);
  hipLaunchKernelGGL((k_block_decide128<kChain2Threads>), dim3(1), dim3(kChain2Threads), 0, s, P);
  (void)hipGetLastError();
}

int chain_blocks_per_cu() {
  int nb = 0;
  int nw = 0;
  int n2 = 0, n3 = 0;
  if (hipOccupancyMaxActiveBlocksPerMultiprocessor(&nb, (k_block_chain_t<true, 32>), 256, 0) != hipSuccess ||
      hipOccupancyMaxActiveBlocksPerMultiprocessor(&nw, (k_block_chain2_t<32, kChain2Threads, false>), kChain2Threads, 0) != hipSuccess ||
      hipOccupancyMaxActiveBlocksPerMultiprocessor(&n2, (k_block_chain2_t<64, kChain2Threads, true>), kChain2Threads, 0) != hipSuccess ||
      hipOccupancyMaxActiveBlocksPerMultiprocessor(&n3, (k_block_decide128<kChain2Threads>), kChain2Threads, 0) != hipSuccess) {
    (void)hipGetLastError();
    nb = nw = n2 = n3 = 1;
  }
  return std::max(1, std::min(std::min(nb, nw), std::min(n2, n3)));
}

template <int K>
static void launch_sweep_tiles(const Buffers& B, const BlockRing& R, int m_local, int kmax, int rows_per_tile, bool nt,
                               const double* A_src, hipStream_t s) {
  const int nstrips = (int)((B.ld + 511) / 512);
  const int ntiles = (m_local + rows_per_tile - 1) / rows_per_tile;
  const dim3 grid(nstrips * ntiles), block(256);
#define LPX_LAUNCH_SWEEP(NT_, OOP_)                                                                              \
  hipLaunchKernelGGL((k_update_tiles<K, NT_, OOP_>), grid, block, 0, s, B.A, A_src, B.ld, m_local, R.prow, R.col, \
                     R.mp, R.up, kmax, rows_per_tile, nstrips, R.census ? R.census + kChainMaxWgs : nullptr)
  if (A_src) { if (nt) LPX_LAUNCH_SWEEP(true, true); else LPX_LAUNCH_SWEEP(false, true); }
  else { if (nt) LPX_LAUNCH_SWEEP(true, false); else LPX_LAUNCH_SWEEP(false, false); }
#undef LPX_LAUNCH_SWEEP
}

template <int K>
static void launch_sweep_k(const Buffers& B, const BlockRing& R, int m_local, int kmax, int rows_per_wg, bool nt,
                           const double* A_src, hipStream_t s, int complement = 0, int slot0 = 0) {
  const int nstrips = (int)((B.ld + 511) / 512);
  const int ngroups = (m_local + rows_per_wg - 1) / rows_per_wg;
  const dim3 grid(nstrips * ngroups), block(256);
#define LPX_LAUNCH_SWEEP(NT_, OOP_)                                                                              \
  hipLaunchKernelGGL((k_update_multi<K, NT_, OOP_>), grid, block, 0, s, B.A, A_src, B.ld, m_local, R.prow, R.col, \
                     R.mp, R.up, kmax, rows_per_wg, nstrips, R.census ? R.census + kChainMaxWgs : nullptr, complement, \
                     slot0)
  if (A_src) { if (nt) LPX_LAUNCH_SWEEP(true, true); else LPX_LAUNCH_SWEEP(false, true); }
  else { if (nt) LPX_LAUNCH_SWEEP(true, false); else LPX_LAUNCH_SWEEP(false, false); }
#undef LPX_LAUNCH_SWEEP
}

static hipStream_t pack_stream(const FixSide* side, hipStream_t s) { return (side && side->stream && side->packed) ? side->stream : s; }
static hipEvent_t pack_stop(const FixSide* side) { return (side && side->stream && side->packed) ? side->packed : nullptr; }
static void pack_done(const FixSide* side, hipStream_t s) {
  if (pack_stop(side)) (void)hipStreamWaitEvent(s, side->packed, 0);
}

static void launch_sweep_pull(const Buffers& B, const BlockRing& R, int m_local, int kmax, bool nt, const double* A_src,
                              hipStream_t s, int slots = 512, const FixSide* side = nullptr, hipEvent_t t0 = nullptr,
                              hipEvent_t t1 = nullptr) {
  const int nstrips_full = (int)(B.ld / 512);
  const int nbt = m_local / 4;
  const int G = std::max(1, std::min(nbt, slots / std::max(1, nstrips_full)));
  LPX_LAUNCH_STOP(k_pack_multipliers<32>, dim3((nbt + 7) / 8), dim3(256), pack_stream(side, s), pack_stop(side), R.col, R.mp, R.up, kmax, nbt, R.col_packed,
                     R.tickets, nstrips_full * 4, (long long*)nullptr);
  pack_done(side, s);
  const dim3 grid(nstrips_full * G), block(256);
#define LPX_LAUNCH_PULL(NT_, OOP_)                                                                                \
  LPX_LAUNCH_TIMED((k_sweep32_pull<NT_, OOP_>), grid, block, s, t0, t1, B.A, A_src, B.ld, m_local, R.prow, R.col, R.mp, \
                   R.up, kmax, nstrips_full, R.col_packed, R.tickets, R.clk)
  if (A_src) { if (nt) LPX_LAUNCH_PULL(true, true); else LPX_LAUNCH_PULL(false, true); }
  else { if (nt) LPX_LAUNCH_PULL(true, false); else LPX_LAUNCH_PULL(false, false); }
#undef LPX_LAUNCH_PULL
}

static void launch_sweep64_one(const Buffers& B, const BlockRing& R, int m_local, int kmax, bool nt, const double* A_src,
                               hipStream_t s, int slots = 512, const FixSide* side = nullptr, hipEvent_t t0 = nullptr,
                               hipEvent_t t1 = nullptr) {
  const int nstrips_full = (int)(B.ld / 512);
  const int ngroups = nstrips_full * 2;
  const int nbt = m_local / 4;
  const int G = std::max(1, std::min(nbt, slots / std::max(1, ngroups)));
  LPX_LAUNCH_STOP(k_pack_multipliers<64>, dim3((nbt + 3) / 4), dim3(256), pack_stream(side, s), pack_stop(side), R.col, R.mp, R.up, kmax, nbt, R.col_packed,
                     R.tickets, nstrips_full * 8, (long long*)nullptr);
  pack_done(side, s);
  const dim3 grid(ngroups * G), block(256);
#define LPX_LAUNCH_ONE64(NT_, OOP_)                                                                               \
  LPX_LAUNCH_TIMED((k_sweep64_one<NT_, OOP_>), grid, block, s, t0, t1, B.A, A_src, B.ld, m_local, R.prow, R.up, kmax, \
                   nstrips_full, R.col_packed, R.tickets, R.clk)
  if (A_src) { if (nt) LPX_LAUNCH_ONE64(true, true); else LPX_LAUNCH_ONE64(false, true); }
  else { if (nt) LPX_LAUNCH_ONE64(true, false); else LPX_LAUNCH_ONE64(false, false); }
#undef LPX_LAUNCH_ONE64
}

#if LPX_FUSED
static void launch_sweep64_mfma(const Buffers& B, const BlockRing& R, int m_local, int kmax, bool nt, const double* A_src,
                                hipStream_t s, int slots = 256, bool two_waves = false, int kmin = 33, const FixSide* side = nullptr,
                                hipEvent_t t0 = nullptr, hipEvent_t t1 = nullptr) {
  const int nstrips_full = (int)(B.ld / 512);
  const int ngroups = nstrips_full * 2;
  const int ntiles = m_local / 16;
  const int G = std::max(1, std::min(ntiles, slots / std::max(1, ngroups)));
  LPX_LAUNCH_STOP(k_pack_multipliers_mfma, dim3(ntiles), dim3(256), pack_stream(side, s), pack_stop(side), R.col, R.mp, R.up, kmax, ntiles, R.col_packed,
                     R.tickets, nstrips_full * 8, two_waves ? (long long*)nullptr : R.clk, two_waves ? 1 : 0);
  pack_done(side, s);
  if (two_waves) {
    const int ng2 = nstrips_full * 4;
    const int G2 = std::max(1, std::min(ntiles, 2 * slots / std::max(1, ng2)));
    const dim3 grid2(ng2 * G2), block2(256);
#define LPX_LAUNCH_MFMA642(NT_, OOP_)                                                                               \
    LPX_LAUNCH_TIMED((k_sweep64_mfma2<NT_, OOP_>), grid2, block2, s, t0, t1, B.A, A_src, B.ld, m_local, R.prow, R.up, kmax, \
                     nstrips_full, R.col_packed, R.tickets, kmin, R.clk)
    if (A_src) { if (nt) LPX_LAUNCH_MFMA642(true, true); else LPX_LAUNCH_MFMA642(false, true); }
    else { if (nt) LPX_LAUNCH_MFMA642(true, false); else LPX_LAUNCH_MFMA642(false, false); }
#undef LPX_LAUNCH_MFMA642
    return;
  }
#ifdef LPX_WITH_VARIANTS
  const dim3 grid(ngroups * G), block(256);
#define LPX_LAUNCH_MFMA64(NT_, OOP_)                                                                               \
  hipLaunchKernelGGL((k_sweep64_mfma<NT_, OOP_>), grid, block, 0, s, B.A, A_src, B.ld, m_local, R.prow, R.up, kmax, \
                     nstrips_full, R.col_packed, R.tickets)
  if (A_src) { if (nt) LPX_LAUNCH_MFMA64(true, true); else LPX_LAUNCH_MFMA64(false, true); }
  else { if (nt) LPX_LAUNCH_MFMA64(true, false); else LPX_LAUNCH_MFMA64(false, false); }
#undef LPX_LAUNCH_MFMA64
#else
  (void)G;
#endif
}
#endif

#if LPX_FUSED
static void launch_sweep128_mfma(const Buffers& B, const BlockRing& R, int m_local, int kmax, bool nt, const double* A_src,
                                 hipStream_t s, int cus, const FixSide* side, hipEvent_t t0, hipEvent_t t1) {
  const int nsub = (int)(B.ld / 64);
  const int ntiles = m_local / 16;
  const int nranges = std::max(1, std::min(kSweep128Ranges, ntiles));
  LPX_LAUNCH_STOP(k_pack_multipliers_mfma128, dim3(ntiles), dim3(256), pack_stream(side, s), pack_stop(side), R.col, R.mp, R.up, kmax,
                  ntiles, R.col_packed, R.tickets, 1 + nsub * nranges, R.clk);
  pack_done(side, s);
  const dim3 grid(std::max(1, std::min(2 * cus, nsub * nranges))), block(256);
#define LPX_LAUNCH_MFMA128(NT_, OOP_)                                                                                    \
  LPX_LAUNCH_TIMED((k_sweep128_mfma<NT_, OOP_>), grid, block, s, t0, t1, B.A, A_src, B.ld, m_local, R.prow, R.up, kmax, nsub, \
                   R.col_packed, R.tickets, nranges)
  if (A_src) { if (nt) LPX_LAUNCH_MFMA128(true, true); else LPX_LAUNCH_MFMA128(false, true); }
  else { if (nt) LPX_LAUNCH_MFMA128(true, false); else LPX_LAUNCH_MFMA128(false, false); }
#undef LPX_LAUNCH_MFMA128
}
#endif

static int choose_sweep_rows(int m_local, int64_t ld, int K, int cus) {
  const int64_t nstrips = (ld + 511) / 512;
  const int64_t slots = std::max(1, 2 * cus);
  const int prologue_rows = std::max(8, (K * 3) / 2);
  int best_rows = kSweepChunk;
  int64_t best_cost = INT64_MAX;
  const int max_rows = (int)std::min<int64_t>(4096, (((int64_t)1 << 32) - 1) / (ld * 8) / kSweepChunk * kSweepChunk);
  for (int rows = kSweepChunk; rows <= std::max(kSweepChunk, max_rows); rows += kSweepChunk) {
    const int64_t groups = (m_local + rows - 1) / rows;
    const int64_t rounds = (nstrips * groups + slots - 1) / slots;
    const int64_t want_rounds = (int64_t)m_local * nstrips >= 3 * slots * kSweepChunk ? 3 : 1;
    const int64_t cost = std::max(rounds, want_rounds) * (rows + prologue_rows);
    if (cost < best_cost || (cost == best_cost && rows > best_rows)) { best_cost = cost; best_rows = rows; }
    if (groups == 1) break;
  }
  return best_rows;
}

const char* sweep_kernel_name(int code) {
  switch (code) {
    case kSweepTiles: return "k_update_tiles";
    case kSweepMulti: return "k_update_multi";
    case kSweepSteady: return "k_sweep32_steady";
    case kSweepPipe64: return "k_sweep64_pipe";
    case kSweepDma: return "k_sweep32_dma";
    case kSweepPull: return "k_sweep32_pull";
    case kSweepPull64: return "k_sweep64_pull";
    case kSweepOne64: return "k_sweep64_one";
    case kSweepMfma64: return "k_sweep64_mfma";
    case kSweepMfma642: return "k_sweep64_mfma2";
    case kSweepMfma128: return "k_sweep128_mfma";
    default: return "";
  }
}

#ifdef LPX_WITH_VARIANTS
#define LPX_VARIANT_PART 6
#include "variants/lpx_variants.inc"
#undef LPX_VARIANT_PART
#endif

int launch_block_sweep(const Buffers& B, const BlockRing& R, int n, int m_local, int row0, int K, int rows_per_wg,
                       bool nt, hipStream_t s, const double* A_src, const double* b_src, hipEvent_t after_sweep,
                       int cus, int form, int* kernel_used, const FixSide* side, hipEvent_t stop, hipEvent_t before_sweep) {
  int used = kSweepNone;
  if (kernel_used) *kernel_used = used;
  if (K < 1) {
    if (before_sweep) (void)hipEventRecord(before_sweep, s);
    if (after_sweep) (void)hipEventRecord(after_sweep, s);
    if (stop) (void)hipEventRecord(stop, s);
    return 0;
  }
  bool timed_own = false, bracket_open = false;
  auto bracket = [&]() { if (before_sweep && !bracket_open) { (void)hipEventRecord(before_sweep, s); bracket_open = true; } };
  if (cus <= 0) {
    int dev = 0;
    (void)hipGetDevice(&dev);
    if (hipDeviceGetAttribute(&cus, hipDeviceAttributeMultiprocessorCount, dev) != hipSuccess || cus <= 0) cus = 256;
  }
  const bool side_fix = side && side->stream && R.fix_col && R.fix_row;
  if (side_fix) (void)hipStreamWaitEvent(side->stream, side->ready, 0);
  else side = nullptr;
  if (K <= 16) {
    bracket();
    int rows_per_tile = rows_per_wg <= 0 ? 16 : rows_per_wg;
    rows_per_tile = std::max(8, std::min(rows_per_tile, kSweepMaxRows)) & ~7;
    while (rows_per_tile > 8 && (int64_t)rows_per_tile * B.ld * 8 >= (int64_t)1 << 32) rows_per_tile -= 8;
    if (K <= 2) launch_sweep_tiles<2>(B, R, m_local, K, rows_per_tile, nt, A_src, s);
    else if (K <= 4) launch_sweep_tiles<4>(B, R, m_local, K, rows_per_tile, nt, A_src, s);
    else if (K <= 8) launch_sweep_tiles<8>(B, R, m_local, K, rows_per_tile, nt, A_src, s);
    else launch_sweep_tiles<16>(B, R, m_local, K, rows_per_tile, nt, A_src, s);
    rows_per_wg = rows_per_tile;
    used = kSweepTiles;
  } else if (K > 64) {
    bool mfma128 = false;
#if LPX_FUSED
    mfma128 = form != 3 && m_local % 16 == 0 && m_local >= 16 && B.ld % 512 == 0 && 16 * B.ld * 8 + 1024 < ((int64_t)1 << 32) &&
              R.tickets && R.col_packed;
#endif
    if (mfma128) {
#if LPX_FUSED
      timed_own = before_sweep && after_sweep;
      if (!timed_own) bracket();
      launch_sweep128_mfma(B, R, m_local, K, nt, A_src, s, cus, side, timed_own ? before_sweep : nullptr, timed_own ? after_sweep : nullptr);
#endif
      rows_per_wg = 16;
      used = kSweepMfma128;
    } else {
      bracket();
      int rows = choose_sweep_rows(m_local, B.ld, 32, cus);
      while (rows > kSweepChunk && (int64_t)rows * B.ld * 8 >= (int64_t)1 << 32) rows -= kSweepChunk;
      for (int slot0 = 0; slot0 < K; slot0 += 32) launch_sweep_k<32>(B, R, m_local, K, rows, nt, slot0 == 0 ? A_src : nullptr, s, 0, slot0);
      rows_per_wg = rows;
      used = kSweepMulti;
    }
  } else if (K > 32) {
    const int nstrips_full = (int)(B.ld / 512);
    const bool geom = m_local % 4 == 0 && nstrips_full >= 1 && 3 * B.ld * 8 + 1024 < ((int64_t)1 << 32);
#ifdef LPX_WITH_VARIANTS
    const bool pull = geom && form != 1 && R.tickets && R.col_packed;
    const bool pipe = geom && !pull && K == 64;
    const bool one = pull && form != 2;
    [[maybe_unused]] const bool mfma_form = form == 0 || form == 4;
    const bool mfma2 = form == 0;
#else
    const bool pull = geom && R.tickets && R.col_packed;
    const bool pipe = false;
    const bool one = pull;
    [[maybe_unused]] const bool mfma_form = form != 3;
    const bool mfma2 = true;
#endif
    bool mfma = false;
#if LPX_FUSED
    mfma = one && mfma_form && m_local % 16 == 0 && 16 * B.ld * 8 + 1024 < ((int64_t)1 << 32);
#endif
    int rows64 = 0;
    const bool whole = mfma && mfma2 && B.ld % 512 == 0;
    timed_own = whole && before_sweep && after_sweep;
    if (!timed_own) bracket();
    if (mfma) {
#if LPX_FUSED
      launch_sweep64_mfma(B, R, m_local, K, nt, A_src, s, cus, mfma2, whole ? 1 : 33, side, timed_own ? before_sweep : nullptr,
                          timed_own ? after_sweep : nullptr);
#endif
      rows64 = 16;
    } else if (one) {
      launch_sweep64_one(B, R, m_local, K, nt, A_src, s, 2 * cus, side);
      rows64 = 4;
    }
#ifdef LPX_WITH_VARIANTS
    else if (pull) {
      launch_sweep64_pull(B, R, m_local, K, nt, A_src, s, 2 * cus);
      rows64 = 4;
    } else if (pipe) {
      rows64 = rows_per_wg > 0 ? std::max(4, rows_per_wg / 4 * 4) : choose_pipe_rows(m_local, nstrips_full, cus);
      while (rows64 > 4 && (int64_t)rows64 * B.ld * 8 >= (int64_t)1 << 32) rows64 -= 4;
      launch_sweep64_pipe(B, R, m_local, K, rows64, nt, A_src, s);
    }
#endif
    const int complement = pull ? 34 : (pipe ? 65 : 0);
    int rows = choose_sweep_rows(m_local, B.ld, 32, cus);
    while (rows > kSweepChunk && (int64_t)rows * B.ld * 8 >= (int64_t)1 << 32) rows -= kSweepChunk;
    if (!whole) {
      launch_sweep_k<32>(B, R, m_local, K, rows, nt, A_src, s, complement, 0);
      launch_sweep_k<32>(B, R, m_local, K, rows, nt, nullptr, s, complement, 32);
    }
    rows_per_wg = (pull || pipe) ? rows64 : rows;
    used = mfma ? (mfma2 ? kSweepMfma642 : kSweepMfma64) : one ? kSweepOne64 : (pull ? kSweepPull64 : (pipe ? kSweepPipe64 : kSweepMulti));
  } else if (K < kMaxBlock && !(m_local % 4 == 0 && B.ld >= 512)) {
    bracket();
    const int64_t nstrips = (B.ld + 511) / 512;
    int rows_per_tile = 16;
    for (int rows : {64, 32})
      if ((int64_t)((m_local + rows - 1) / rows) * nstrips >= 4096) { rows_per_tile = rows; break; }
    while (rows_per_tile > 8 && (int64_t)rows_per_tile * B.ld * 8 >= (int64_t)1 << 32) rows_per_tile -= 8;
    launch_sweep_tiles<32>(B, R, m_local, K, rows_per_tile, nt, A_src, s);
    rows_per_wg = rows_per_tile;
    used = kSweepTiles;
  } else {
    if (rows_per_wg <= 0) rows_per_wg = choose_sweep_rows(m_local, B.ld, K, cus);
    rows_per_wg = std::max(kSweepChunk, (rows_per_wg + kSweepChunk - 1) / kSweepChunk * kSweepChunk);
    while (rows_per_wg > kSweepChunk && (int64_t)rows_per_wg * B.ld * 8 >= (int64_t)1 << 32) rows_per_wg -= kSweepChunk;
    const bool wide32 = 3 * B.ld * 8 + 1024 >= ((int64_t)1 << 32);
    const bool pullable = m_local % 4 == 0 && B.ld >= 512 && !wide32 && R.zeros && R.tickets && R.col_packed;
    bool done = false;
#ifdef LPX_WITH_VARIANTS
    const bool variant32 = m_local % 4 == 0 && B.ld >= 512 && (form == 1 || form == 2 || !pullable);
#else
    const bool variant32 = false;
#endif
    timed_own = !variant32 && pullable && B.ld % 512 == 0 && before_sweep && after_sweep;
    if (!timed_own) bracket();
#ifdef LPX_WITH_VARIANTS
    if (variant32) {
      int rows48 = choose_pipe_rows(m_local, (int)(B.ld / 512), 2 * cus, 48);
      while (rows48 > 4 && (int64_t)rows48 * B.ld * 8 >= (int64_t)1 << 32) rows48 -= 4;
      if (form == 2 && pullable) {
        launch_sweep_dma(B, R, m_local, K, rows48, nt, A_src, s, 2 * cus);
        used = kSweepDma;
      } else {
        launch_sweep_steady(B, R, m_local, K, rows48, nt, A_src, s);
        used = kSweepSteady;
      }
      if (B.ld % 512 != 0) launch_sweep_k<32>(B, R, m_local, K, rows_per_wg, nt, A_src, s, 1);
      rows_per_wg = rows48;
      done = true;
    }
#endif
    if (!done && pullable) {
      launch_sweep_pull(B, R, m_local, K, nt, A_src, s, 2 * cus, side, timed_own ? before_sweep : nullptr, timed_own ? after_sweep : nullptr);
      used = kSweepPull;
      if (B.ld % 512 != 0) launch_sweep_k<32>(B, R, m_local, K, rows_per_wg, nt, A_src, s, 1);
      rows_per_wg = 4;
    } else if (!done) {
      launch_sweep_k<32>(B, R, m_local, K, rows_per_wg, nt, A_src, s);
      used = kSweepMulti;
    }
  }
  if (kernel_used) *kernel_used = used;
  if (after_sweep && !timed_own) { bracket(); (void)hipEventRecord(after_sweep, s); }
  const bool probed = used == kSweepPull || used == kSweepPull64 || used == kSweepOne64 || used == kSweepMfma64 || used == kSweepMfma642;
  const int gx = (int)((std::max<int64_t>(m_local, B.ld) + 255) / 256);
  if (side_fix) {
    LPX_LAUNCH_STOP(k_block_fixup, dim3(gx, (K + kFixChunk - 1) / kFixChunk, 3), dim3(256), side->stream, side->done, B.A, B.ld, n, m_local, row0,
                    B.b, R.prow, R.col, R.col0, R.row0, R.mp, R.up, K, b_src ? b_src : B.b, (long long*)nullptr, R.fix_col, R.fix_row);
    (void)hipStreamWaitEvent(s, side->done, 0);
  }
  const bool memset_behind = !probed && R.clk && used != kSweepMfma128;
  hipEvent_t last_stop = memset_behind ? nullptr : stop;
  if (side_fix) {
    LPX_LAUNCH_STOP(k_block_fixup_scatter, dim3(gx, (K + kFixChunk - 1) / kFixChunk, 2), dim3(256), s, last_stop, B.A, B.ld, m_local, row0,
                    (const double*)R.fix_col, (const double*)R.fix_row, R.mp, R.up, K, probed ? R.clk : (long long*)nullptr);
  } else {
    LPX_LAUNCH_STOP(k_block_fixup, dim3(gx, (K + kFixChunk - 1) / kFixChunk, 3), dim3(256), s, last_stop, B.A, B.ld, n, m_local, row0, B.b, R.prow, R.col,
                    R.col0, R.row0, R.mp, R.up, K, b_src ? b_src : B.b, probed ? R.clk : (long long*)nullptr, (double*)nullptr, (double*)nullptr);
  }
  if (memset_behind) {
    (void)hipMemsetAsync(R.clk, 0, 256, s);
    if (stop) (void)hipEventRecord(stop, s);
  }
  return rows_per_wg;
}

void launch_fill_column(double* A, int64_t ld, int m, int col, double value, hipStream_t s) {
  if (m <= 0) return;
  hipLaunchKernelGGL(k_fill_column, dim3((m + 255) / 256), dim3(256), 0, s, A, ld, m, col, value);
}

void launch_drop_column(double* A, int64_t ld, int m, int n_old, int col, hipStream_t s) {
  if (m <= 0) return;
  hipLaunchKernelGGL(k_drop_column, dim3(m), dim3(256), 0, s, A, ld, m, n_old, col);
}

void launch_restore_objective(const Buffers& B, int n, const RestoreEntry* d_entries, int n_entries, hipStream_t s) {
  const int blocks = n > 0 ? (n + 255) / 256 : 1;
  hipLaunchKernelGGL(k_restore_objective, dim3(blocks), dim3(256), 0, s, B.A, B.ld, B.b, B.c, n, d_entries,
                     n_entries, B.ctl);
}

void launch_checksum(const Buffers& B, int m_local, int n, int row0, unsigned long long* d_out3, hipStream_t s) {
  hipLaunchKernelGGL(k_checksum, dim3(1024), dim3(256), 0, s, B.A, B.ld, m_local, n, row0, B.b, B.c, d_out3);
}

void launch_transpose(const double* dA, int64_t lda, double* dAt, int64_t ldat, int m, int n, hipStream_t s) {
  if (m <= 0 || n <= 0) return;
  hipLaunchKernelGGL(k_transpose, dim3((n + 63) / 64, (m + 63) / 64), dim3(256), 0, s, dA, lda, dAt, ldat, m, n);
}

#include "lpx_batch.inc"

}
}
```

### linear_programming_solver_amd/csrc/lpx_launchers.inc

```
void launch_entering(const Buffers& B, int n, hipStream_t s, const LoopStart& start = LoopStart{});
void launch_entering_dantzig(const Buffers& B, int n, bool seed, hipStream_t s, const LoopStart& start = LoopStart{});
void launch_ratio_gather(const Buffers& B, int m_local, int row0, const Geometry& g, int forced_e, hipStream_t s);
void launch_reduce_partials(const Buffers& B, const Geometry& g, hipStream_t s);
void launch_select_pivot(const Buffers& B, int n, int m_global, const Geometry& g, int forced_e, int forced_l,
                         hipStream_t s);
void launch_update(const Buffers& B, int m_local, int n, int row0, const Geometry& g, bool nontemporal,
                   const double* prow, const LpxCtl* up, double* A_out, double* b_out, hipStream_t s);
void launch_propose(const Buffers& B, int n, int row0, int m_local, const Geometry& g, double* d_candidate,
                    hipStream_t s);
void launch_commit(const Buffers& B, int n, int m_global, const double* d_gathered, int nranks, double* prow,
                   LpxCtl* up, int up_parity, hipStream_t s);
void launch_peek(const Buffers& B, int n, int m_local, int row0, const double* prow_t, const double* col_t,
                 double* col_next, const LpxCtl* pend, double* d_candidate, hipStream_t s);
void launch_block_peek(const Buffers& B, const BlockRing& R, int n, int m_local, int row0, int np, double* d_candidate,
                       hipStream_t s);
void launch_block_decide(const Buffers& B, const BlockRing& R, int n, int m_global, const double* d_gathered, int nranks,
                         int slot, hipStream_t s);
int launch_block_chain(const Buffers& B, const BlockRing& R, int n, int m, int nb, int half, int old_half, int n_old,
                        int b_from_tableau, int seq, int dantzig, int wgs, int fences, bool trace, LpxCtl* host_snap,
                        hipStream_t s, const MgPeers* mg = nullptr, hipEvent_t stop = nullptr);
void preload_block_kernels(const Buffers& B, const BlockRing& R, hipStream_t s);
unsigned* sweep_fail_word(const BlockRing& R, int64_t ld);
int64_t sweep_ticket_slots(int64_t ld);
int chain_blocks_per_cu();
const char* sweep_kernel_name(int code);
int launch_block_sweep(const Buffers& B, const BlockRing& R, int n, int m_local, int row0, int K, int rows_per_wg,
                       bool nt, hipStream_t s, const double* A_src = nullptr, const double* b_src = nullptr,
                       hipEvent_t after_sweep = nullptr, int cus = 0, int form = 0, int* kernel_used = nullptr,
                       const FixSide* side = nullptr, hipEvent_t stop = nullptr, hipEvent_t before_sweep = nullptr);
void launch_fill_column(double* A, int64_t ld, int m, int col, double value, hipStream_t s);
void launch_drop_column(double* A, int64_t ld, int m, int n_old, int col, hipStream_t s);
void launch_restore_objective(const Buffers& B, int n, const RestoreEntry* d_entries, int n_entries, hipStream_t s);
void launch_checksum(const Buffers& B, int m_local, int n, int row0, unsigned long long* d_out3, hipStream_t s);
hipError_t launch_batch_simplex(const BatchArgs& a, hipStream_t s);
int batch_blocks_per_cu(int threads, int lds_bytes);
hipError_t launch_batch_solve(const BatchSolveArgs& a, hipStream_t s);
int batch_solve_blocks_per_cu(int threads, int lds_bytes);
hipError_t launch_batch_scenarios(const BatchScenarioArgs& a, hipStream_t s);
int batch_scenarios_blocks_per_cu(int threads, int lds_bytes);
hipError_t launch_scenarios_crash(const ScenarioCrashArgs& a, hipStream_t s);
hipError_t launch_batch_resolve(const BatchResolveArgs& a, hipStream_t s);
int batch_resolve_blocks_per_cu(int threads, int lds_bytes);
void launch_transpose(const double* dA, int64_t lda, double* dAt, int64_t ldat, int m, int n, hipStream_t s);
```

### linear_programming_solver_amd/csrc/lpx_sweeps.inc

```
constexpr int kSweepMaxRows = 128;
#ifndef LPX_SWEEP_NBUF
#define LPX_SWEEP_NBUF 2
#endif

__device__ __forceinline__ int ring_count(const LpxCtl* __restrict__ ring, int kcap, int kmax, int* sh_np) {
  if (threadIdx.x < 64) {
    const int lane = threadIdx.x;
    const bool ok = lane < kcap && lane < kmax && ring[lane].do_update != 0;
    const unsigned long long mask = __ballot(ok);
    if (lane == 0) *sh_np = (~mask == 0ull) ? 64 : (__ffsll((long long)~mask) - 1);
  }
  __syncthreads();
  return *sh_np;
}
__device__ __forceinline__ int ring_count128(const LpxCtl* __restrict__ ring, int kmax, int* sh_np) {
  if (threadIdx.x < 64) {
    const int lane = threadIdx.x;
    const unsigned long long m0 = __ballot(lane < kmax && ring[lane].do_update != 0);
    const unsigned long long m1 = __ballot(lane + 64 < kmax && ring[lane + 64].do_update != 0);
    const int n0 = (~m0 == 0ull) ? 64 : (__ffsll((long long)~m0) - 1);
    const int n1 = (~m1 == 0ull) ? 64 : (__ffsll((long long)~m1) - 1);
    if (lane == 0) *sh_np = n0 < 64 ? n0 : 64 + n1;
  }
  __syncthreads();
// ... 750 lines not shown
  }
  if (blockIdx.x == 0)
    for (int u = threadIdx.x; u < nsub; u += 256) tickets[u * 32] = 0u;
  const int tile = blockIdx.x;
  if (tile >= ntiles) return;
#pragma unroll
  for (int q = 0; q < 4; ++q) {
    const int idx = q * 256 + threadIdx.x;
    const int g = idx >> 6, l = idx & 63, k = l >> 4, i = l & 15;
    const int s = 4 * g + k;
    const double c = s < np ? col_ring[(int64_t)s * mp + (int64_t)tile * 16 + i] : 0.0;
    colM[(int64_t)tile * 1024 + (pairs ? (g >> 1) * 128 + 2 * l + (g & 1) : idx)] = -c;
  }
}

#ifdef LPX_WITH_VARIANTS
#define LPX_VARIANT_PART 4
#include "variants/lpx_variants.inc"
#undef LPX_VARIANT_PART
#endif


constexpr int kMfma2LdsBytes = 2 * 16 * 4 * 64 * 8;
static_assert(2 * kMfma2LdsBytes <= 160 * 1024, "two workgroups per CU");
typedef unsigned v2u __attribute__((ext_vector_type(2)));
typedef unsigned v4u __attribute__((ext_vector_type(4)));
template <bool NT, bool OOP>
__global__ __launch_bounds__(256, 2) void k_sweep64_mfma2(double* A, const double* Asrc,
                                                          int64_t ld, int m_local,
                                                          const double* __restrict__ prow_ring,
                                                          const LpxCtl* __restrict__ ring, int kmax, int nstrips_full,
                                                          const double* colM,
                                                          unsigned* tickets, int kmin, long long* clk) {
  constexpr int NG = 16, CT = 4;
  constexpr int kRsrcWord3 = 0x00020000;
  constexpr int kAuxNt = NT ? 2 : 0;
  __shared__ __attribute__((aligned(16))) double sh_b[2 * NG * CT * 64];
  __shared__ int sh_np;
  sweep_front_stamp(clk);
  const int np = ring_count(ring, 64, kmax, &sh_np);
  if (np < kmin) return;
  const int lane = threadIdx.x & 63;
  const int wave = __builtin_amdgcn_readfirstlane((int)(threadIdx.x >> 6));
  const int ngroups = nstrips_full * 4;
  const int grp = (ngroups % 8 == 0)
                      ? (int)(((blockIdx.x >> 3) + (blockIdx.x & 7) * (unsigned)(ngroups / 8)) % (unsigned)ngroups)
                      : (int)(blockIdx.x % (unsigned)ngroups);
  const int ntiles = 2 * (m_local / 16);
  unsigned* const ctr = tickets + grp * 32;
  const int64_t row_bytes = ld * 8;
  char* const dst_base = reinterpret_cast<char*>(A + grp * 128);
  const char* const src_base = OOP ? reinterpret_cast<const char*>(Asrc + grp * 128) : dst_base;
  const uint32_t rb32 = (uint32_t)row_bytes;
  const uint32_t off_c = (uint32_t)(lane >> 4) * rb32 + (uint32_t)(lane & 15) * 8u;
  const uint32_t off_a = (uint32_t)lane * 8u;
  for (int q = wave; q < 2 * NG * CT; q += 4) {
    const int h = q / (NG * CT), g = (q / CT) % NG, ct = q % CT;
    const int s = 4 * g + (lane >> 4);
    sh_b[q * 64 + lane] = s < np ? prow_ring[(int64_t)s * ld + grp * 128 + h * 64 + ct * 16 + (lane & 15)] : 0.0;
  }
  __syncthreads();
  auto load_tile = [&](int t, d4v (&c)[CT], double (&a)[NG]) {
    const int tt = max(0, min(t, ntiles - 1));
    const __amdgpu_buffer_rsrc_t rc = __builtin_amdgcn_make_buffer_rsrc(
        const_cast<char*>(src_base) + (int64_t)(tt >> 1) * 16 * row_bytes + (tt & 1) * 512, 0, -1, kRsrcWord3);
#pragma unroll
    for (int r = 0; r < 4; ++r)
#pragma unroll
      for (int ct = 0; ct < CT; ++ct)
        c[ct][r] = __builtin_bit_cast(double, __builtin_amdgcn_raw_buffer_load_b64(rc, off_c + (uint32_t)ct * 128u,
                                                                                    (int)((uint32_t)(4 * r) * rb32), kAuxNt));
    const __amdgpu_buffer_rsrc_t ra = __builtin_amdgcn_make_buffer_rsrc(
        const_cast<double*>(colM) + (int64_t)(tt >> 1) * 1024, 0, -1, kRsrcWord3);
#pragma unroll
    for (int p = 0; p < NG / 2; ++p) {
      const v4u x = __builtin_amdgcn_raw_buffer_load_b128(ra, 2u * off_a + (uint32_t)(p & 3) * 1024u, (p >> 2) * 4096, 0);
      a[2 * p] = __builtin_bit_cast(double, v2u{x[0], x[1]});
      a[2 * p + 1] = __builtin_bit_cast(double, v2u{x[2], x[3]});
    }
  };
#define LPX_MFMA_FENCE __builtin_amdgcn_sched_barrier(0)
  auto work_tile = [&](int t, d4v (&c)[CT], const double (&a)[NG]) {
    const double* const bl = sh_b + (max(0, min(t, ntiles - 1)) & 1) * (NG * CT * 64) + lane;
#pragma unroll
    for (int g = 0; g < NG; ++g)
#pragma unroll
      for (int ct = 0; ct < CT; ++ct) {
        c[ct] = __builtin_amdgcn_mfma_f64_16x16x4f64(a[g], bl[(g * CT + ct) * 64], c[ct], 0, 0, 0);
      }
    __builtin_amdgcn_sched_group_barrier(0x100, 2, 0);
#pragma unroll
    for (int g = 0; g < NG; ++g) {
      if (g + 1 < NG) __builtin_amdgcn_sched_group_barrier(0x100, 2, 0);
      __builtin_amdgcn_sched_group_barrier(0x008, 4, 0);
    }
    const int tt = max(0, min(t, ntiles - 1));
    char* const out = dst_base + (int64_t)(tt >> 1) * 16 * row_bytes + (tt & 1) * 512;
    const __amdgpu_buffer_rsrc_t rd = __builtin_amdgcn_make_buffer_rsrc(out, 0, __builtin_amdgcn_readfirstlane((unsigned)t < (unsigned)ntiles ? -1 : 0), kRsrcWord3);
#pragma unroll
    for (int r = 0; r < 4; ++r)
#pragma unroll
      for (int ct = 0; ct < CT; ++ct)
        __builtin_amdgcn_raw_buffer_store_b64(__builtin_bit_cast(v2u, (double)c[ct][r]), rd, off_c + (uint32_t)ct * 128u,
                                              (int)((uint32_t)(4 * r) * rb32), kAuxNt);
  };
  constexpr int kStepOps = 16 + 8 + 16;
  static_assert(kStepOps + 1 <= 63, "vmcnt is six bits wide");
  auto take = [&](unsigned& tk) -> int {
    asm volatile("s_waitcnt vmcnt(%0)" :: "n"(kStepOps + 1) : "memory");
    return ticket_take(tk);
  };
  d4v c0[CT], c1[CT], c2[CT];
  double a0[NG], a1[NG], a2[NG];
  int t0, t1;
  unsigned k0, k1, k2;
  {
    ticket_pull(k0, ctr); ticket_pull(k1, ctr);
    asm volatile("s_waitcnt vmcnt(0)" ::: "memory");
    t0 = ticket_take(k0); t1 = ticket_take(k1);
  }
  if (t0 >= ntiles) return;
  load_tile(t0, c0, a0);
  load_tile(t1, c1, a1);
  ticket_pull(k2, ctr);
  __builtin_amdgcn_s_waitcnt(0x0F70);
#pragma unroll 1
  do {
    ticket_pull(k0, ctr);
    const int t2 = take(k2);
    load_tile(t2, c2, a2);
    LPX_MFMA_FENCE;
    work_tile(t0, c0, a0);
    LPX_MFMA_FENCE;
    ticket_pull(k1, ctr);
    const int t3 = take(k0);
    load_tile(t3, c0, a0);
    LPX_MFMA_FENCE;
    work_tile(t1, c1, a1);
    LPX_MFMA_FENCE;
    ticket_pull(k2, ctr);
    const int t4 = take(k1);
    load_tile(t4, c1, a1);
    LPX_MFMA_FENCE;
    work_tile(t2, c2, a2);
    LPX_MFMA_FENCE;
    t0 = t3; t1 = t4;
  } while (t0 < ntiles);
}

#undef LPX_MFMA_FENCE
__global__ __launch_bounds__(256) void k_pack_multipliers_mfma128(const double* __restrict__ col_ring, int64_t mp,
                                                                  const LpxCtl* __restrict__ ring, int kmax, int ntiles,
                                                                  double* __restrict__ colM, unsigned* __restrict__ tickets, int nctr,
                                                                  long long* __restrict__ clk) {
  __shared__ int sh_np;
  const int np = ring_count128(ring, kmax, &sh_np);
  if (blockIdx.x == 0)
    for (int u = threadIdx.x; u < nctr; u += 256) tickets[u * 32] = 0u;
  if (clk && blockIdx.x == 0 && threadIdx.x < 32) clk[threadIdx.x] = 0;
  const int tile = blockIdx.x;
  if (tile >= ntiles) return;
#pragma unroll
  for (int q = 0; q < 8; ++q) {
    const int idx = q * 256 + threadIdx.x;
    const int g = idx >> 6, l = idx & 63, k = l >> 4, i = l & 15;
    const int s = 4 * g + k;
    const double c = s < np ? col_ring[(int64_t)s * mp + (int64_t)tile * 16 + i] : 0.0;
    colM[(int64_t)tile * 2048 + (g >> 1) * 128 + 2 * l + (g & 1)] = -c;
  }
}
#define LPX_MFMA_FENCE __builtin_amdgcn_sched_barrier(0)
template <bool NT, bool OOP>
__global__ __launch_bounds__(256, 2) void k_sweep128_mfma(double* A, const double* Asrc,
                                                          int64_t ld, int m_local,
                                                          const double* __restrict__ prow_ring,
                                                          const LpxCtl* __restrict__ ring, int kmax, int nsub,
                                                          const double* colM,
                                                          unsigned* tickets, int nranges) {
  constexpr int NG = 32, CT = 4;
  constexpr int kRsrcWord3 = 0x00020000;
  constexpr int kAuxNt = NT ? 2 : 0;
  __shared__ __attribute__((aligned(16))) double sh_b[NG * CT * 64];
  __shared__ int sh_np, sh_chunk;
  const int np = ring_count128(ring, kmax, &sh_np);
  if (np < 1 && !OOP) return;
  const int lane = threadIdx.x & 63;
  const int wave = __builtin_amdgcn_readfirstlane((int)(threadIdx.x >> 6));
  const int rowblocks = m_local / 16;
  const int per_range = (rowblocks + nranges - 1) / nranges;
  const int nchunks = nsub * nranges;
  const int64_t row_bytes = ld * 8;
  const uint32_t rb32 = (uint32_t)row_bytes;
  const uint32_t off_c = (uint32_t)(lane >> 4) * rb32 + (uint32_t)(lane & 15) * 8u;
  const uint32_t off_a = (uint32_t)lane * 8u;
  int sub_loaded = -1;
  for (;;) {
    if (threadIdx.x == 0) sh_chunk = (int)atomicAdd(tickets, 1u);
    __syncthreads();
    const int chunk = __builtin_amdgcn_readfirstlane(sh_chunk);
    if (chunk >= nchunks) return;
    const int sub = chunk % nsub, range = chunk / nsub;
    const int rb0 = range * per_range;
    const int ntiles = min(rowblocks, rb0 + per_range) - rb0;
    if (sub != sub_loaded) {
      for (int q = wave; q < NG * CT; q += 4) {
        const int g = q / CT, ct = q % CT;
        const int s = 4 * g + (lane >> 4);
        sh_b[q * 64 + lane] = s < np ? prow_ring[(int64_t)s * ld + sub * 64 + ct * 16 + (lane & 15)] : 0.0;
      }
      sub_loaded = sub;
    }
    __syncthreads();
    if (ntiles > 0) {
      unsigned* const ctr = tickets + 32 * (1 + chunk);
      char* const dst_base = reinterpret_cast<char*>(A + sub * 64) + (int64_t)rb0 * 16 * row_bytes;
      const char* const src_base = OOP ? reinterpret_cast<const char*>(Asrc + sub * 64) + (int64_t)rb0 * 16 * row_bytes : dst_base;
      const double* const colM0 = colM + (int64_t)rb0 * 2048;
      auto load_tile = [&](int t, d4v (&c)[CT], double (&a)[NG]) {
        const int tt = max(0, min(t, ntiles - 1));
        const __amdgpu_buffer_rsrc_t rc = __builtin_amdgcn_make_buffer_rsrc(
            const_cast<char*>(src_base) + (int64_t)tt * 16 * row_bytes, 0, -1, kRsrcWord3);
#pragma unroll
        for (int r = 0; r < 4; ++r)
#pragma unroll
          for (int ct = 0; ct < CT; ++ct)
            c[ct][r] = __builtin_bit_cast(double, __builtin_amdgcn_raw_buffer_load_b64(rc, off_c + (uint32_t)ct * 128u,
                                                                                         (int)((uint32_t)(4 * r) * rb32), kAuxNt));
        const __amdgpu_buffer_rsrc_t ra = __builtin_amdgcn_make_buffer_rsrc(
            const_cast<double*>(colM0) + (int64_t)tt * 2048, 0, -1, kRsrcWord3);
#pragma unroll
        for (int p = 0; p < NG / 2; ++p) {
          const v4u x = __builtin_amdgcn_raw_buffer_load_b128(ra, 2u * off_a + (uint32_t)(p & 3) * 1024u, (p >> 2) * 4096, 0);
          a[2 * p] = __builtin_bit_cast(double, v2u{x[0], x[1]});
          a[2 * p + 1] = __builtin_bit_cast(double, v2u{x[2], x[3]});
        }
      };
      auto work_tile = [&](int t, d4v (&c)[CT], const double (&a)[NG]) {
        const double* const bl = sh_b + lane;
#pragma unroll
        for (int g = 0; g < NG; ++g)
#pragma unroll
          for (int ct = 0; ct < CT; ++ct)
            c[ct] = __builtin_amdgcn_mfma_f64_16x16x4f64(a[g], bl[(g * CT + ct) * 64], c[ct], 0, 0, 0);
        __builtin_amdgcn_sched_group_barrier(0x100, 2, 0);
#pragma unroll
        for (int g = 0; g < NG; ++g) {
          if (g + 1 < NG) __builtin_amdgcn_sched_group_barrier(0x100, 2, 0);
          __builtin_amdgcn_sched_group_barrier(0x008, 4, 0);
        }
        const int tt = max(0, min(t, ntiles - 1));
        char* const out = dst_base + (int64_t)tt * 16 * row_bytes;
        const __amdgpu_buffer_rsrc_t rd = __builtin_amdgcn_make_buffer_rsrc(out, 0, __builtin_amdgcn_readfirstlane((unsigned)t < (unsigned)ntiles ? -1 : 0), kRsrcWord3);
#pragma unroll
        for (int r = 0; r < 4; ++r)
#pragma unroll
          for (int ct = 0; ct < CT; ++ct)
            __builtin_amdgcn_raw_buffer_store_b64(__builtin_bit_cast(v2u, (double)c[ct][r]), rd, off_c + (uint32_t)ct * 128u,
                                                  (int)((uint32_t)(4 * r) * rb32), kAuxNt);
      };
      constexpr int kStepOps = 16 + 16 + 16;
      auto take = [&](unsigned& tk) -> int {
        asm volatile("s_waitcnt vmcnt(%0)" :: "n"(kStepOps + 1) : "memory");
        return ticket_take(tk);
      };
      d4v c0[CT], c1[CT];
      double a0[NG], a1[NG];
      unsigned ka, kb = 0;
      ticket_pull(ka, ctr);
      asm volatile("s_waitcnt vmcnt(0)" ::: "memory");
      int t0 = ticket_take(ka);
      if (t0 < ntiles) {
        load_tile(t0, c0, a0);
        ticket_pull(ka, ctr);
        __builtin_amdgcn_s_waitcnt(0x0F70);
#pragma unroll 1
        do {
          ticket_pull(kb, ctr);
          const int t1 = take(ka);
          load_tile(t1, c1, a1);
          LPX_MFMA_FENCE;
          work_tile(t0, c0, a0);
          LPX_MFMA_FENCE;
          ticket_pull(ka, ctr);
          const int t2 = take(kb);
          load_tile(t2, c0, a0);
          LPX_MFMA_FENCE;
          work_tile(t1, c1, a1);
          LPX_MFMA_FENCE;
          t0 = t2;
        } while (t0 < ntiles);
      }
      asm volatile("s_waitcnt vmcnt(0)" ::: "memory");
      asm volatile("" : "+v"(ka), "+v"(kb) :: "memory");
    }
    __syncthreads();
  }
}
#undef LPX_MFMA_FENCE
#ifdef LPX_WITH_VARIANTS
#define LPX_VARIANT_PART 7
#include "variants/lpx_variants.inc"
#undef LPX_VARIANT_PART
#endif
#endif

#ifdef LPX_WITH_VARIANTS
#define LPX_VARIANT_PART 5
#include "variants/lpx_variants.inc"
#undef LPX_VARIANT_PART
#endif

__device__ __forceinline__ double apply_pivot(double v, int i, int j, int l_r, int e_r, double p_r, double ce,
                                              double pr_j) {
  if (i == l_r) return pr_j;
  if (j == e_r) return -__ddiv_rn(ce, p_r);
  return submul(v, ce, pr_j);
}

constexpr int kFixChunk = 8;
__device__ __forceinline__ void fix_pick_chains(const int* keys, int np, int* sh_pick, int* sh_npick) {
  const int q = threadIdx.x;
  const int key = keys[q], key_hi = keys[64 + q];
  bool keep = q < np, keep_hi = 64 + q < np;
  for (int r = q + 1; r < np; ++r) keep = keep && keys[r] != key;
  for (int r = 64 + q + 1; r < np; ++r) keep_hi = keep_hi && keys[r] != key_hi;
  const unsigned long long mask = __ballot(keep), mask_hi = __ballot(keep_hi);
  const unsigned long long below = (1ull << q) - 1ull;
  if (keep) sh_pick[__popcll(mask & below)] = q;
  if (keep_hi) sh_pick[__popcll(mask) + __popcll(mask_hi & below)] = 64 + q;
  const int npick = __popcll(mask) + __popcll(mask_hi);
  if (q < kFixChunk) sh_pick[npick + q] = 0;
  if (q == 0) *sh_npick = npick;
}
__global__ __launch_bounds__(256) void k_block_fixup(double* __restrict__ A, int64_t ld, int n, int m_local, int row0,
                                                     double* b, const double* __restrict__ prow_ring,
                                                     const double* __restrict__ col_ring,
                                                     const double* __restrict__ col0_ring,
                                                     const double* __restrict__ row0_ring, int64_t mp,
                                                     const LpxCtl* __restrict__ ring, int kmax,
                                                     const double* b_src, long long* __restrict__ clk,
                                                     double* __restrict__ img_col, double* __restrict__ img_row) {
  static_assert(kBlockMax == 128, "two words of hit ballots: lane u asks for pending pivots u and 64 + u");
  if (clk && blockIdx.x < 8 && blockIdx.y == 0 && blockIdx.z == 0 && threadIdx.x == 0) {
    const unsigned x = xcc_id() & 7u;
    clk[x * 4 + 2] = __builtin_amdgcn_s_memtime(); clk[x * 4 + 3] = wall_clock64();
  }
  __shared__ double sh_p[kBlockMax], sh_bl[kBlockMax];
  __shared__ __attribute__((aligned(16))) double sh_x[kBlockMax][kFixChunk];
  __shared__ int sh_e[kBlockMax], sh_l[kBlockMax], sh_eq[kBlockMax], sh_pick[kBlockMax + kFixChunk];
  __shared__ int sh_np, sh_npick;
  const int s0 = blockIdx.y * kFixChunk, job = blockIdx.z;
  if ((int64_t)blockIdx.x * blockDim.x >= (job == 1 ? ld : (int64_t)m_local) || (job == 2 && s0 != 0)) return;
  const int np = ring_count128(ring, kmax, &sh_np);
  if (job == 2 ? s0 != 0 : s0 >= np) return;
  if ((int)threadIdx.x < kBlockMax) {
    const bool live = (int)threadIdx.x < np;
    const LpxCtl& q = ring[live ? threadIdx.x : 0];
    sh_e[threadIdx.x] = live ? q.e_cur : -1;
    sh_l[threadIdx.x] = live ? q.l - row0 : -1;
    sh_p[threadIdx.x] = live ? q.p : 1.0;
    sh_bl[threadIdx.x] = live ? q.bl : 0.0;
  }
  __syncthreads();
  if (job != 2 && threadIdx.x < 64) fix_pick_chains(job == 1 ? sh_l : sh_e, np, sh_pick, &sh_npick);
  __syncthreads();
  const int npick = job == 2 ? 0 : sh_npick;
  if (job != 2 && s0 >= npick) return;
  const int t = blockIdx.x * blockDim.x + threadIdx.x;
  const int ns = min(kFixChunk, npick - s0);
  int pk[kFixChunk];
#pragma unroll
  for (int q = 0; q < kFixChunk; ++q) pk[q] = sh_pick[(job == 2 ? 0 : s0) + q];
  const int lane = threadIdx.x & 63;
  const int t_wave = t - lane;
  if (job == 0) {
    for (int idx = threadIdx.x; idx < np * kFixChunk; idx += blockDim.x) {
      const int r = idx / kFixChunk, q = idx % kFixChunk;
      sh_x[r][q] = q < ns ? prow_ring[(int64_t)r * ld + sh_e[sh_pick[s0 + q]]] : 0.0;
    }
    if ((int)threadIdx.x < np) {
      int mask = 0;
      for (int q = 0; q < ns; ++q) mask |= (sh_e[sh_pick[s0 + q]] == sh_e[threadIdx.x]) << q;
      sh_eq[threadIdx.x] = mask;
    }
    __syncthreads();
    const unsigned long long hit = __ballot((unsigned)(sh_l[lane] - t_wave) < 64u);
    const unsigned long long hit_hi = __ballot((unsigned)(sh_l[64 + lane] - t_wave) < 64u);
    if (t < m_local) {
      double v[kFixChunk];
#pragma unroll
      for (int q = 0; q < kFixChunk; ++q) v[q] = q < ns ? col0_ring[(int64_t)pk[q] * mp + t] : 0.0;
      double cv[8], cvn[8];
#pragma unroll
      for (int u = 0; u < 8; ++u) cv[u] = (u < np) ? col_ring[(int64_t)u * mp + t] : 0.0;
      for (int r0 = 0; r0 < np; r0 += 8) {
#pragma unroll
        for (int u = 0; u < 8; ++u) cvn[u] = (r0 + 8 + u < np) ? col_ring[(int64_t)(r0 + 8 + u) * mp + t] : 0.0;
#pragma unroll
        for (int u = 0; u < 8; ++u) {
          const int r = r0 + u;
          if (r < np) {
            double x[kFixChunk];
#pragma unroll
            for (int q = 0; q < kFixChunk; ++q) x[q] = sh_x[r][q];
            const int eq = __builtin_amdgcn_readfirstlane(sh_eq[r]);
            if (eq == 0 && !(((r < 64 ? hit >> r : hit_hi >> (r - 64))) & 1)) {
#pragma unroll
              for (int q = 0; q < kFixChunk; ++q) v[q] = submul(v[q], cv[u], x[q]);
            } else {
              const double pr = sh_p[r];
              const bool own = t == sh_l[r];
#pragma unroll
              for (int q = 0; q < kFixChunk; ++q) {
                double nv;
                if ((eq >> q) & 1) nv = -__ddiv_rn(cv[u], pr);
                else nv = submul(v[q], cv[u], x[q]);
                v[q] = own ? x[q] : nv;
              }
            }
          }
        }
#pragma unroll
        for (int u = 0; u < 8; ++u) cv[u] = cvn[u];
      }
#pragma unroll
      for (int q = 0; q < kFixChunk; ++q)
        if (q < ns) {
          if (img_col) img_col[(int64_t)(s0 + q) * mp + t] = v[q];
          else A[(int64_t)t * ld + sh_e[pk[q]]] = v[q];
        }
    }
  } else if (job == 1) {
    for (int idx = threadIdx.x; idx < np * kFixChunk; idx += blockDim.x) {
      const int r = idx / kFixChunk, q = idx % kFixChunk;
      const int i = q < ns ? sh_l[sh_pick[s0 + q]] : -1;
      sh_x[r][q] = (i >= 0 && i < m_local) ? col_ring[(int64_t)r * mp + i] : 0.0;
    }
    if ((int)threadIdx.x < np) {
      int mask = 0;
      for (int q = 0; q < ns; ++q) mask |= (sh_l[sh_pick[s0 + q]] == sh_l[threadIdx.x]) << q;
      sh_eq[threadIdx.x] = mask;
    }
    __syncthreads();
    const unsigned long long hit = __ballot((unsigned)(sh_e[lane] - t_wave) < 64u);
    const unsigned long long hit_hi = __ballot((unsigned)(sh_e[64 + lane] - t_wave) < 64u);
    if (t < (int)ld) {
      double v[kFixChunk];
#pragma unroll
      for (int q = 0; q < kFixChunk; ++q) v[q] = (q < ns && t < n) ? row0_ring[(int64_t)pk[q] * ld + t] : 0.0;
      double pv[8], pvn[8];
#pragma unroll
      for (int u = 0; u < 8; ++u) pv[u] = (u < np) ? prow_ring[(int64_t)u * ld + t] : 0.0;
      for (int r0 = 0; r0 < np; r0 += 8) {
#pragma unroll
        for (int u = 0; u < 8; ++u) pvn[u] = (r0 + 8 + u < np) ? prow_ring[(int64_t)(r0 + 8 + u) * ld + t] : 0.0;
#pragma unroll
        for (int u = 0; u < 8; ++u) {
          const int r = r0 + u;
          if (r < np) {
            double x[kFixChunk];
#pragma unroll
            for (int q = 0; q < kFixChunk; ++q) x[q] = sh_x[r][q];
            const int eq = __builtin_amdgcn_readfirstlane(sh_eq[r]);
            if (eq == 0 && !(((r < 64 ? hit >> r : hit_hi >> (r - 64))) & 1)) {
#pragma unroll
              for (int q = 0; q < kFixChunk; ++q) v[q] = submul(v[q], x[q], pv[u]);
            } else {
              const double pr = sh_p[r];
              const bool own = t == sh_e[r];
#pragma unroll
              for (int q = 0; q < kFixChunk; ++q) {
                double nv;
                if (own) nv = -__ddiv_rn(x[q], pr);
                else nv = submul(v[q], x[q], pv[u]);
                v[q] = ((eq >> q) & 1) ? pv[u] : nv;
              }
            }
          }
        }
#pragma unroll
        for (int u = 0; u < 8; ++u) pv[u] = pvn[u];
      }
#pragma unroll
      for (int q = 0; q < kFixChunk; ++q) {
        const int i = q < ns ? sh_l[pk[q]] : -1;
        if (i >= 0 && i < m_local) {
          if (img_row) img_row[(int64_t)(s0 + q) * ld + t] = v[q];
          else A[(int64_t)i * ld + t] = v[q];
        }
      }
    }
  } else {
    const unsigned long long hit = __ballot((unsigned)(sh_l[lane] - t_wave) < 64u);
    const unsigned long long hit_hi = __ballot((unsigned)(sh_l[64 + lane] - t_wave) < 64u);
    if (t < m_local) {
      double bi = b_src[t];
      for (int r0 = 0; r0 < np; r0 += 8) {
        double cv[8];
#pragma unroll
        for (int q = 0; q < 8; ++q) cv[q] = (r0 + q < np) ? col_ring[(int64_t)(r0 + q) * mp + t] : 0.0;
#pragma unroll
        for (int q = 0; q < 8; ++q) {
          const int r = r0 + q;
          if (r < np) {
            const double nb = submul(bi, cv[q], sh_bl[r]);
            bi = nb;
            if ((r < 64 ? hit >> r : hit_hi >> (r - 64)) & 1) { if (t == sh_l[r]) bi = sh_bl[r]; }
          }
        }
      }
      b[t] = bi;
    }
  }
}

__global__ __launch_bounds__(256) void k_block_fixup_scatter(double* __restrict__ A, int64_t ld, int m_local, int row0,
                                                             const double* __restrict__ img_col,
                                                             const double* __restrict__ img_row, int64_t mp,
                                                             const LpxCtl* __restrict__ ring, int kmax,
                                                             long long* __restrict__ clk) {
  if (clk && blockIdx.x < 8 && blockIdx.y == 0 && blockIdx.z == 0 && threadIdx.x == 0) {
    const unsigned x = xcc_id() & 7u;
    clk[x * 4 + 2] = __builtin_amdgcn_s_memtime(); clk[x * 4 + 3] = wall_clock64();
  }
  __shared__ int sh_key[kBlockMax], sh_pick[kBlockMax + kFixChunk];
  __shared__ int sh_np, sh_npick;
  const int s0 = blockIdx.y * kFixChunk, job = blockIdx.z;
  if ((int64_t)blockIdx.x * blockDim.x >= (job == 1 ? ld : (int64_t)m_local)) return;
  const int np = ring_count128(ring, kmax, &sh_np);
  if (s0 >= np) return;
  if ((int)threadIdx.x < kBlockMax) {
    const bool live = (int)threadIdx.x < np;
    const LpxCtl& q = ring[live ? threadIdx.x : 0];
    sh_key[threadIdx.x] = live ? (job == 1 ? q.l - row0 : q.e_cur) : -1;
  }
  __syncthreads();
  if (threadIdx.x < 64) fix_pick_chains(sh_key, np, sh_pick, &sh_npick);
  __syncthreads();
  const int npick = sh_npick;
  if (s0 >= npick) return;
  const int ns = min(kFixChunk, npick - s0);
  const int t = blockIdx.x * blockDim.x + threadIdx.x;
  double v[kFixChunk];
  if (job == 0) {
    if (t >= m_local) return;
#pragma unroll
    for (int q = 0; q < kFixChunk; ++q) v[q] = q < ns ? img_col[(int64_t)(s0 + q) * mp + t] : 0.0;
#pragma unroll
    for (int q = 0; q < kFixChunk; ++q)
      if (q < ns) A[(int64_t)t * ld + sh_key[sh_pick[s0 + q]]] = v[q];
  } else {
    if (t >= (int)ld) return;
#pragma unroll
    for (int q = 0; q < kFixChunk; ++q) {
      const int i = q < ns ? sh_key[sh_pick[s0 + q]] : -1;
      v[q] = (i >= 0 && i < m_local) ? img_row[(int64_t)(s0 + q) * ld + t] : 0.0;
    }
#pragma unroll
    for (int q = 0; q < kFixChunk; ++q) {
      const int i = q < ns ? sh_key[sh_pick[s0 + q]] : -1;
      if (i >= 0 && i < m_local) A[(int64_t)i * ld + t] = v[q];
    }
  }
}
```

Baseline: 24350.

## Overlap fixup row/column copy beside the MFMA sweep using skip masks

```diff
diff --git a/include/lpx.h b/include/lpx.h
--- a/include/lpx.h
+++ b/include/lpx.h
@@ -69,7 +69,8 @@
   LPX_OPT_FUSED = 18,
   LPX_OPT_CHAIN_FORM = 19,
   LPX_OPT_FIXUP_SIDE = 20,
-  LPX_OPT_COUNT = 21
+  LPX_OPT_SIDE_COPY = 21,
+  LPX_OPT_COUNT = 22
 } lpx_option;
 int lpx_state_set_option(lpx_state* s, int32_t key, int64_t value);
 int lpx_state_get_option(const lpx_state* s, int32_t key, int64_t* value);
diff --git a/linear_programming_solver_amd/_lib.py b/linear_programming_solver_amd/_lib.py
--- a/linear_programming_solver_amd/_lib.py
+++ b/linear_programming_solver_amd/_lib.py
@@ -14,7 +14,7 @@
 OPTIONS = {"block": 0, "chain": 1, "overlap": 2, "overlap_serial": 3, "overlap_mask": 4, "chain_wgs": 5,
            "chain_fences": 6, "sweep_rows": 7, "nt": 8, "batch": 9, "chain_trace": 10, "update_u": 11,
            "update_rows": 12, "a2_offset": 13, "sweep_form": 14, "multi_onehop": 15, "sweep_cus": 16, "chain_cus": 17,
-           "fused": 18, "chain_form": 19, "fixup_side": 20}
+           "fused": 18, "chain_form": 19, "fixup_side": 20, "side_copy": 21}
 
 DEFAULT_FUSED = None
 
diff --git a/linear_programming_solver_amd/csrc/lpx_dispatch.cpp b/linear_programming_solver_amd/csrc/lpx_dispatch.cpp
--- a/linear_programming_solver_amd/csrc/lpx_dispatch.cpp
+++ b/linear_programming_solver_amd/csrc/lpx_dispatch.cpp
@@ -60,9 +60,10 @@
 const char* sweep_kernel_name(int code) { return plain::sweep_kernel_name(code); }
 int launch_block_sweep(const Buffers& B, const BlockRing& R, int n, int m_local, int row0, int K, int rows_per_wg,
                        bool nt, hipStream_t s, const double* A_src, const double* b_src, hipEvent_t after_sweep, int cus,
-                       int form, int* kernel_used, const FixSide* side, hipEvent_t stop, hipEvent_t before_sweep) {
+                       int form, int* kernel_used, const FixSide* side, hipEvent_t stop, hipEvent_t before_sweep,
+                       bool* copy_beside) {
   return LPX_PICK(B, launch_block_sweep)(B, R, n, m_local, row0, K, rows_per_wg, nt, s, A_src, b_src, after_sweep, cus,
-                                         form, kernel_used, side, stop, before_sweep);
+                                         form, kernel_used, side, stop, before_sweep, copy_beside);
 }
 void launch_fill_column(double* A, int64_t ld, int m, int col, double value, hipStream_t s) {
   plain::launch_fill_column(A, ld, m, col, value, s);
diff --git a/linear_programming_solver_amd/csrc/lpx_engine.cpp b/linear_programming_solver_amd/csrc/lpx_engine.cpp
--- a/linear_programming_solver_amd/csrc/lpx_engine.cpp
+++ b/linear_programming_solver_amd/csrc/lpx_engine.cpp
@@ -73,6 +73,7 @@
     {"LPX_FUSED", 2, 0, 2},
     {"LPX_CHAIN_FORM", 1, 0, 1},
     {"LPX_FIXUP_SIDE", 4, 0, 4},
+    {"LPX_SIDE_COPY", 1, 0, 1},
 };
 
 static const int64_t* env_defaults() {
@@ -170,6 +171,8 @@
   (void)hipFree(s->R.census);
   (void)hipFree(const_cast<double*>(s->R.zeros));
   (void)hipFree(s->R.tickets);
+  (void)hipFree(s->R.sweep_masks);
+  (void)hipFree(s->R.fix_picks);
   (void)hipFree(s->R.sweep_fail);
   (void)hipFree(s->R.clk);
   (void)hipFree(s->R.col_packed);
@@ -219,6 +222,7 @@
   for (hipStream_t t : s->ov_fix) if (t) (void)hipStreamDestroy(t);
   for (hipEvent_t e : s->ev_ov_fix) if (e) (void)hipEventDestroy(e);
   for (hipEvent_t e : s->ev_ov_pack) if (e) (void)hipEventDestroy(e);
+  for (hipEvent_t e : s->ev_ov_copy) if (e) (void)hipEventDestroy(e);
   if (s->own_stream) (void)hipStreamDestroy(s->own_stream);
   delete s;
 }
@@ -558,6 +562,10 @@
   HIP_TRY(hipMemsetAsync(const_cast<double*>(s->R.zeros), 0, 256, s->stream));
   HIP_TRY(hipMalloc((void**)&s->R.tickets, 2 * (size_t)lpxk::sweep_ticket_slots(s->B.ld) * 128));
   HIP_TRY(hipMemsetAsync(s->R.tickets, 0, 2 * (size_t)lpxk::sweep_ticket_slots(s->B.ld) * 128, s->stream));
+  HIP_TRY(hipMalloc((void**)&s->R.sweep_masks, 2 * (size_t)lpxk::sweep_mask_words(s->B.ld, mp) * sizeof(unsigned)));
+  HIP_TRY(hipMemsetAsync(s->R.sweep_masks, 0, 2 * (size_t)lpxk::sweep_mask_words(s->B.ld, mp) * sizeof(unsigned), s->stream));
+  HIP_TRY(hipMalloc((void**)&s->R.fix_picks, 2 * 2 * (size_t)lpxk::kFixPickStride * sizeof(int)));
+  HIP_TRY(hipMemsetAsync(s->R.fix_picks, 0, 2 * 2 * (size_t)lpxk::kFixPickStride * sizeof(int), s->stream));
   HIP_TRY(hipMalloc((void**)&s->R.sweep_fail, 128));
   HIP_TRY(hipMemsetAsync(s->R.sweep_fail, 0, 128, s->stream));
   HIP_TRY(hipMalloc((void**)&s->R.clk, 256));
@@ -633,7 +641,8 @@
 }
 
 int launch_sweep_profiled(lpx_state* s, int K, hipStream_t stream, const Buffers& B, const lpxk::BlockRing& R,
-                                 const double* A_src, const double* b_src, const lpxk::FixSide* side, hipEvent_t stop) {
+                                 const double* A_src, const double* b_src, const lpxk::FixSide* side, hipEvent_t stop,
+                                 bool* copy_beside) {
   const bool sample = s->prof > 0 && (s->prof_seq++ % s->prof) == 0;
   if (sample) {
     if (s->ev_used + 2 > s->ev.size()) {
@@ -651,14 +660,14 @@
                                                 s->nontemporal, stream, A_src, b_src,
                                                 sample ? s->ev[s->ev_used + 1] : nullptr, cus,
                                                 (int)s->opt[LPX_OPT_SWEEP_FORM], &kernel_used, side, stop,
-                                                sample ? s->ev[s->ev_used] : nullptr);
+                                                sample ? s->ev[s->ev_used] : nullptr, copy_beside);
   s->info.sweep_kernel = kernel_used;
   if (sample) s->ev_used += 2;
   HIP_TRY(hipGetLastError());
   return 0;
 }
 static int launch_sweep_profiled(lpx_state* s, int K) {
-  return launch_sweep_profiled(s, K, s->stream, s->B, s->R, nullptr, nullptr, nullptr, nullptr);
+  return launch_sweep_profiled(s, K, s->stream, s->B, s->R, nullptr, nullptr, nullptr, nullptr, nullptr);
 }
 
 lpxk::BlockRing ring_half(const lpx_state* s, int h) {
@@ -672,6 +681,8 @@
   if (R.fix_row) R.fix_row += o * s->B.ld;
   if (R.col_packed) R.col_packed += (int64_t)h * (R.mp / 4 + 1) * (4 * lpxk::kColPackedRowBytes / sizeof(double));
   if (R.tickets) R.tickets += (int64_t)h * lpxk::sweep_ticket_slots(s->B.ld) * 32;
+  if (R.sweep_masks) R.sweep_masks += (int64_t)h * lpxk::sweep_mask_words(s->B.ld, R.mp);
+  if (R.fix_picks) R.fix_picks += (int64_t)h * 2 * lpxk::kFixPickStride;
   R.up += o;
   return R;
 }
@@ -743,6 +754,7 @@
   for (int k = 0; k < 2; k++) {
     if (!s->ev_ov_fix[k]) HIP_TRY(hipEventCreateWithFlags(&s->ev_ov_fix[k], hipEventDisableTiming));
     if (!s->ev_ov_pack[k]) HIP_TRY(hipEventCreateWithFlags(&s->ev_ov_pack[k], hipEventDisableTiming));
+    if (!s->ev_ov_copy[k]) HIP_TRY(hipEventCreateWithFlags(&s->ev_ov_copy[k], hipEventDisableTiming));
   }
   if (s->ov_fix[mode]) return 0;
   bool made = false;
@@ -795,6 +807,8 @@
     (void)hipGetLastError();
     fix_mode = 0;
   }
+  const bool side_copy = fix_mode > 0 && s->opt[LPX_OPT_SIDE_COPY] != 0;
+  bool copied[2] = {false, false};
   auto issue_block = [&](int k) -> int {
     const int nb = block_len(K, max_pivots, decided);
     if (nb <= 0) return 1;
@@ -808,6 +822,7 @@
                                                    chain_wgs, fences, trace, d_snap + h, s->ov_chain, nullptr, s->ev_ov_chain[h]);
     } else {
       if (k >= 2) HIP_TRY(hipStreamWaitEvent(s->ov_chain, s->ev_ov_sweep[h], 0));
+      if (k >= 2 && copied[h]) HIP_TRY(hipStreamWaitEvent(s->ov_chain, s->ev_ov_copy[h], 0));
       Brd.A = Abuf[k == 0 ? 0 : (k - 1) & 1];
       Brd.b = bbuf[k == 0 ? 0 : (k - 1) & 1];
       s->info.chain_wgs = lpxk::launch_block_chain(Brd, s->R, s->n, s->m, nb, h, h ^ 1, k > 0 ? nb_prev : 0, k == 0,
@@ -823,9 +838,12 @@
     Buffers Bdst = s->B;
     Bdst.A = Abuf[h ^ 1];
     Bdst.b = bbuf[h ^ 1];
-    const lpxk::FixSide side{fix_mode > 0 ? s->ov_fix[fix_mode] : nullptr, s->ev_ov_chain[h], s->ev_ov_fix[h], s->ev_ov_pack[h]};
+    const lpxk::FixSide side{fix_mode > 0 ? s->ov_fix[fix_mode] : nullptr, s->ev_ov_chain[h], s->ev_ov_fix[h], s->ev_ov_pack[h],
+                             k >= 1 ? s->ev_ov_sweep[h ^ 1] : nullptr, side_copy ? s->ev_ov_copy[h] : nullptr,
+                             (k >= 1 && copied[h ^ 1]) ? s->ev_ov_copy[h ^ 1] : nullptr};
+    copied[h] = false;
     if (int rc = launch_sweep_profiled(s, nb, s->ov_sweep, Bdst, ring_half(s, h), Abuf[h], bbuf[h], fix_mode > 0 ? &side : nullptr,
-                                       s->ev_ov_sweep[h])) return rc;
+                                       s->ev_ov_sweep[h], &copied[h])) return rc;
     decided += nb;
     nb_prev = nb;
     nblk = k + 1;
@@ -844,6 +862,8 @@
   (void)hipEventRecord(s->ev_ov_join[2], s->ov_sweep);
   (void)hipStreamWaitEvent(s->stream, s->ev_ov_join[1], 0);
   (void)hipStreamWaitEvent(s->stream, s->ev_ov_join[2], 0);
+  for (int h = 0; h < 2; h++)
+    if (copied[h]) (void)hipStreamWaitEvent(s->stream, s->ev_ov_copy[h], 0);
   if (nblk & 1) {
     std::swap(s->B.A, s->A2);
     std::swap(s->B.b, s->b2);
diff --git a/linear_programming_solver_amd/csrc/lpx_internal.h b/linear_programming_solver_amd/csrc/lpx_internal.h
--- a/linear_programming_solver_amd/csrc/lpx_internal.h
+++ b/linear_programming_solver_amd/csrc/lpx_internal.h
@@ -55,6 +55,7 @@
   hipStream_t ov_fix[4] = {nullptr, nullptr, nullptr, nullptr};
   hipEvent_t ev_ov_fix[2] = {nullptr, nullptr};
   hipEvent_t ev_ov_pack[2] = {nullptr, nullptr};
+  hipEvent_t ev_ov_copy[2] = {nullptr, nullptr};
   double* d_cand = nullptr;
   LpxCtl* h_ctl = nullptr;
   LpxCtl* h_snap = nullptr;
@@ -100,7 +101,8 @@
 int device_cus(const lpx_state* s);
 int launch_sweep_profiled(lpx_state* s, int K, hipStream_t stream, const Buffers& B, const lpxk::BlockRing& R,
                           const double* A_src, const double* b_src, const lpxk::FixSide* side = nullptr,
-                          hipEvent_t stop = nullptr);
+                          hipEvent_t stop = nullptr,
+                          bool* copy_beside = nullptr);
 int ensure_fix_side(lpx_state* s, int mode);
 lpxk::BlockRing ring_half(const lpx_state* s, int h);
 void launch_seed_entering(lpx_state* s, const lpxk::LoopStart& start = lpxk::LoopStart{});
diff --git a/linear_programming_solver_amd/csrc/lpx_kernels.h b/linear_programming_solver_amd/csrc/lpx_kernels.h
--- a/linear_programming_solver_amd/csrc/lpx_kernels.h
+++ b/linear_programming_solver_amd/csrc/lpx_kernels.h
@@ -81,6 +81,8 @@
   double* fix_row;
   double* col_packed;
   unsigned* tickets;
+  unsigned* sweep_masks;
+  int* fix_picks;
   unsigned* sweep_fail;
   long long* clk;
   const double* zeros;
@@ -102,9 +104,12 @@
   unsigned spin_max;
 };
 enum SweepKernel { kSweepNone = 0, kSweepTiles = 1, kSweepMulti = 2, kSweepSteady = 3, kSweepPipe64 = 4, kSweepDma = 5, kSweepPull = 6, kSweepPull64 = 7, kSweepOne64 = 8, kSweepMfma64 = 9, kSweepMfma642 = 10, kSweepMfma128 = 11 };
-struct FixSide { hipStream_t stream; hipEvent_t ready, done, packed; };
+struct FixSide { hipStream_t stream; hipEvent_t ready, done, packed, swept_before, copied, copied_before; };
+inline int64_t sweep_mask_words(int64_t ld, int64_t mp) { return 2 * (ld / 64 + 1) + mp / 16 + 2; }
 constexpr int kColPackedRowBytes = 1024;
 constexpr int kSweep128Ranges = 3;
+constexpr int kSweep128MaskTiles = 4096;
+constexpr int kFixPickStride = 160;
 struct RestoreEntry { int32_t is_basic; int32_t index; double k; };
 
 constexpr int kBatchLdsMax = 163840;
diff --git a/linear_programming_solver_amd/csrc/lpx_kernels.hip b/linear_programming_solver_amd/csrc/lpx_kernels.hip
--- a/linear_programming_solver_amd/csrc/lpx_kernels.hip
+++ b/linear_programming_solver_amd/csrc/lpx_kernels.hip
@@ -963,9 +963,11 @@
     hipLaunchKernelGGL((k_sweep64_mfma2<NT_, OOP_>), dim3(1), dim3(256), 0, s, A, A, ld, 0, R.prow, R.up, 0, 1, R.col_packed, R.tickets, 33, (long long*)nullptr);
     LPX_EACH_NT_OOP(LPX_PRE_MFMA642)
 #undef LPX_PRE_MFMA642
-    hipLaunchKernelGGL(k_pack_multipliers_mfma128, dim3(1), dim3(256), 0, s, R.col, R.mp, R.up, 0, 0, R.col_packed, R.tickets, 0, (long long*)nullptr);
+    hipLaunchKernelGGL(k_pack_multipliers_mfma128, dim3(1), dim3(256), 0, s, R.col, R.mp, R.up, 0, 0, R.col_packed, R.tickets, 0, (long long*)nullptr,
+                       (unsigned*)nullptr, 0, 0);
 #define LPX_PRE_MFMA128(NT_, OOP_) \
-    hipLaunchKernelGGL((k_sweep128_mfma<NT_, OOP_>), dim3(1), dim3(256), 0, s, A, A, ld, 0, R.prow, R.up, 0, 0, R.col_packed, R.tickets, 1);
+    hipLaunchKernelGGL((k_sweep128_mfma<NT_, OOP_>), dim3(1), dim3(256), 0, s, A, A, ld, 0, R.prow, R.up, 0, 0, R.col_packed, R.tickets, 1, \
+                       (const unsigned*)nullptr);
     LPX_EACH_NT_OOP(LPX_PRE_MFMA128)
 #undef LPX_PRE_MFMA128
 #endif
@@ -983,9 +985,9 @@
 #undef LPX_PRE_TILES
 #undef LPX_EACH_NT_OOP
   hipLaunchKernelGGL(k_block_fixup, dim3(1, 1, 3), dim3(256), 0, s, A, ld, 0, 0, 0, B.b, R.prow, R.col, R.col0, R.row0,
-                     R.mp, R.up, 0, B.b, (long long*)nullptr, (double*)nullptr, (double*)nullptr);
+                     R.mp, R.up, 0, B.b, (long long*)nullptr, (double*)nullptr, (double*)nullptr, (int*)nullptr);
   hipLaunchKernelGGL(k_block_fixup_scatter, dim3(1, 1, 2), dim3(256), 0, s, A, ld, 0, 0, (const double*)nullptr, (const double*)nullptr,
-                     R.mp, R.up, 0, (long long*)nullptr);
+                     R.mp, R.up, 0, (long long*)nullptr, (const int*)nullptr);
   ChainArgs P{};
   P.ctl = B.ctl; P.up = R.up; P.nb = 0;
   P.bar = R.chain_bar; P.bar_next = R.chain_bar + 32;
@@ -1125,19 +1127,24 @@
 }
 #endif
 
+static int sweep128_ranges(int m_local) { return std::max(1, std::min(kSweep128Ranges, m_local / 16)); }
 #if LPX_FUSED
-static void launch_sweep128_mfma(const Buffers& B, const BlockRing& R, int m_local, int kmax, bool nt, const double* A_src,
-                                 hipStream_t s, int cus, const FixSide* side, hipEvent_t t0, hipEvent_t t1) {
+static void launch_sweep128_mfma(const Buffers& B, const BlockRing& R, int m_local, int row0, int kmax, bool nt, const double* A_src,
+                                 hipStream_t s, int cus, const FixSide* side, hipEvent_t t0, hipEvent_t t1, unsigned* masks) {
   const int nsub = (int)(B.ld / 64);
   const int ntiles = m_local / 16;
-  const int nranges = std::max(1, std::min(kSweep128Ranges, ntiles));
+  const int nranges = sweep128_ranges(m_local);
   LPX_LAUNCH_STOP(k_pack_multipliers_mfma128, dim3(ntiles), dim3(256), pack_stream(side, s), pack_stop(side), R.col, R.mp, R.up, kmax,
-                  ntiles, R.col_packed, R.tickets, 1 + nsub * nranges, R.clk);
+                  ntiles, R.col_packed, R.tickets, 1 + nsub * nranges, R.clk, masks, nsub, row0);
   pack_done(side, s);
   const dim3 grid(std::max(1, std::min(2 * cus, nsub * nranges))), block(256);
 #define LPX_LAUNCH_MFMA128(NT_, OOP_)                                                                                    \
-  LPX_LAUNCH_TIMED((k_sweep128_mfma<NT_, OOP_>), grid, block, s, t0, t1, B.A, A_src, B.ld, m_local, R.prow, R.up, kmax, nsub, \
-                   R.col_packed, R.tickets, nranges)
+  do {                                                                                                                   \
+    if (t0) LPX_LAUNCH_TIMED((k_sweep128_mfma<NT_, OOP_>), grid, block, s, t0, t1, B.A, A_src, B.ld, m_local, R.prow, R.up, kmax, nsub, \
+                             R.col_packed, R.tickets, nranges, (const unsigned*)masks);                                  \
+    else LPX_LAUNCH_STOP((k_sweep128_mfma<NT_, OOP_>), grid, block, s, t1, B.A, A_src, B.ld, m_local, R.prow, R.up, kmax, nsub, \
+                         R.col_packed, R.tickets, nranges, (const unsigned*)masks);                                      \
+  } while (0)
   if (A_src) { if (nt) LPX_LAUNCH_MFMA128(true, true); else LPX_LAUNCH_MFMA128(false, true); }
   else { if (nt) LPX_LAUNCH_MFMA128(true, false); else LPX_LAUNCH_MFMA128(false, false); }
 #undef LPX_LAUNCH_MFMA128
@@ -1187,9 +1194,11 @@
 
 int launch_block_sweep(const Buffers& B, const BlockRing& R, int n, int m_local, int row0, int K, int rows_per_wg,
                        bool nt, hipStream_t s, const double* A_src, const double* b_src, hipEvent_t after_sweep,
-                       int cus, int form, int* kernel_used, const FixSide* side, hipEvent_t stop, hipEvent_t before_sweep) {
+                       int cus, int form, int* kernel_used, const FixSide* side, hipEvent_t stop, hipEvent_t before_sweep,
+                       bool* copy_beside) {
   int used = kSweepNone;
   if (kernel_used) *kernel_used = used;
+  if (copy_beside) *copy_beside = false;
   if (K < 1) {
     if (before_sweep) (void)hipEventRecord(before_sweep, s);
     if (after_sweep) (void)hipEventRecord(after_sweep, s);
@@ -1206,6 +1215,16 @@
   const bool side_fix = side && side->stream && R.fix_col && R.fix_row;
   if (side_fix) (void)hipStreamWaitEvent(side->stream, side->ready, 0);
   else side = nullptr;
+  bool mfma128 = false;
+#if LPX_FUSED
+  mfma128 = K > 64 && form != 3 && m_local % 16 == 0 && m_local >= 16 && B.ld % 512 == 0 && 16 * B.ld * 8 + 1024 < ((int64_t)1 << 32) &&
+            R.tickets && R.col_packed;
+#endif
+  const bool beside = side_fix && mfma128 && A_src && side->copied && pack_stop(side) && R.sweep_masks && R.fix_picks &&
+                      16 * B.ld * 8 + 1024 < ((int64_t)1 << 31) &&
+                      (m_local / 16 + sweep128_ranges(m_local) - 1) / sweep128_ranges(m_local) <= kSweep128MaskTiles;
+  if (copy_beside) *copy_beside = beside;
+  if (side && side->copied_before && !beside) (void)hipStreamWaitEvent(s, side->copied_before, 0);
   if (K <= 16) {
     bracket();
     int rows_per_tile = rows_per_wg <= 0 ? 16 : rows_per_wg;
@@ -1218,16 +1237,13 @@
     rows_per_wg = rows_per_tile;
     used = kSweepTiles;
   } else if (K > 64) {
-    bool mfma128 = false;
-#if LPX_FUSED
-    mfma128 = form != 3 && m_local % 16 == 0 && m_local >= 16 && B.ld % 512 == 0 && 16 * B.ld * 8 + 1024 < ((int64_t)1 << 32) &&
-              R.tickets && R.col_packed;
-#endif
     if (mfma128) {
 #if LPX_FUSED
       timed_own = before_sweep && after_sweep;
       if (!timed_own) bracket();
-      launch_sweep128_mfma(B, R, m_local, K, nt, A_src, s, cus, side, timed_own ? before_sweep : nullptr, timed_own ? after_sweep : nullptr);
+      launch_sweep128_mfma(B, R, m_local, row0, K, nt, A_src, s, cus, side, timed_own ? before_sweep : nullptr,
+                           timed_own ? after_sweep : (beside ? stop : nullptr), beside ? R.sweep_masks : nullptr);
+      if (beside && timed_own && stop) (void)hipEventRecord(stop, s);
 #endif
       rows_per_wg = 16;
       used = kSweepMfma128;
@@ -1348,17 +1364,27 @@
   const int gx = (int)((std::max<int64_t>(m_local, B.ld) + 255) / 256);
   if (side_fix) {
     LPX_LAUNCH_STOP(k_block_fixup, dim3(gx, (K + kFixChunk - 1) / kFixChunk, 3), dim3(256), side->stream, side->done, B.A, B.ld, n, m_local, row0,
-                    B.b, R.prow, R.col, R.col0, R.row0, R.mp, R.up, K, b_src ? b_src : B.b, (long long*)nullptr, R.fix_col, R.fix_row);
+                    B.b, R.prow, R.col, R.col0, R.row0, R.mp, R.up, K, b_src ? b_src : B.b, (long long*)nullptr, R.fix_col, R.fix_row,
+                    beside ? R.fix_picks : (int*)nullptr);
+    if (beside) {
+      if (side->swept_before) (void)hipStreamWaitEvent(side->stream, side->swept_before, 0);
+      LPX_LAUNCH_STOP(k_block_fixup_scatter, dim3(gx, (K + kFixChunk - 1) / kFixChunk, 2), dim3(256), side->stream, side->copied, B.A, B.ld,
+                      m_local, row0, (const double*)R.fix_col, (const double*)R.fix_row, R.mp, R.up, K, (long long*)nullptr,
+                      (const int*)R.fix_picks);
+      return rows_per_wg;
+    }
     (void)hipStreamWaitEvent(s, side->done, 0);
   }
   const bool memset_behind = !probed && R.clk && used != kSweepMfma128;
   hipEvent_t last_stop = memset_behind ? nullptr : stop;
   if (side_fix) {
     LPX_LAUNCH_STOP(k_block_fixup_scatter, dim3(gx, (K + kFixChunk - 1) / kFixChunk, 2), dim3(256), s, last_stop, B.A, B.ld, m_local, row0,
-                    (const double*)R.fix_col, (const double*)R.fix_row, R.mp, R.up, K, probed ? R.clk : (long long*)nullptr);
+                    (const double*)R.fix_col, (const double*)R.fix_row, R.mp, R.up, K, probed ? R.clk : (long long*)nullptr,
+                    (const int*)nullptr);
   } else {
     LPX_LAUNCH_STOP(k_block_fixup, dim3(gx, (K + kFixChunk - 1) / kFixChunk, 3), dim3(256), s, last_stop, B.A, B.ld, n, m_local, row0, B.b, R.prow, R.col,
-                    R.col0, R.row0, R.mp, R.up, K, b_src ? b_src : B.b, probed ? R.clk : (long long*)nullptr, (double*)nullptr, (double*)nullptr);
+                    R.col0, R.row0, R.mp, R.up, K, b_src ? b_src : B.b, probed ? R.clk : (long long*)nullptr, (double*)nullptr, (double*)nullptr,
+                    (int*)nullptr);
   }
   if (memset_behind) {
     (void)hipMemsetAsync(R.clk, 0, 256, s);
diff --git a/linear_programming_solver_amd/csrc/lpx_launchers.inc b/linear_programming_solver_amd/csrc/lpx_launchers.inc
--- a/linear_programming_solver_amd/csrc/lpx_launchers.inc
+++ b/linear_programming_solver_amd/csrc/lpx_launchers.inc
@@ -27,7 +27,8 @@
 int launch_block_sweep(const Buffers& B, const BlockRing& R, int n, int m_local, int row0, int K, int rows_per_wg,
                        bool nt, hipStream_t s, const double* A_src = nullptr, const double* b_src = nullptr,
                        hipEvent_t after_sweep = nullptr, int cus = 0, int form = 0, int* kernel_used = nullptr,
-                       const FixSide* side = nullptr, hipEvent_t stop = nullptr, hipEvent_t before_sweep = nullptr);
+                       const FixSide* side = nullptr, hipEvent_t stop = nullptr, hipEvent_t before_sweep = nullptr,
+                       bool* copy_beside = nullptr);
 void launch_fill_column(double* A, int64_t ld, int m, int col, double value, hipStream_t s);
 void launch_drop_column(double* A, int64_t ld, int m, int n_old, int col, hipStream_t s);
 void launch_restore_objective(const Buffers& B, int n, const RestoreEntry* d_entries, int n_entries, hipStream_t s);
diff --git a/linear_programming_solver_amd/csrc/lpx_sweeps.inc b/linear_programming_solver_amd/csrc/lpx_sweeps.inc
--- a/linear_programming_solver_amd/csrc/lpx_sweeps.inc
+++ b/linear_programming_solver_amd/csrc/lpx_sweeps.inc
@@ -926,11 +926,33 @@
 __global__ __launch_bounds__(256) void k_pack_multipliers_mfma128(const double* __restrict__ col_ring, int64_t mp,
                                                                   const LpxCtl* __restrict__ ring, int kmax, int ntiles,
                                                                   double* __restrict__ colM, unsigned* __restrict__ tickets, int nctr,
-                                                                  long long* __restrict__ clk) {
+                                                                  long long* __restrict__ clk, unsigned* __restrict__ masks, int nsub,
+                                                                  int row0) {
   __shared__ int sh_np;
+  __shared__ unsigned sh_m[2];
   const int np = ring_count128(ring, kmax, &sh_np);
   if (blockIdx.x == 0)
     for (int u = threadIdx.x; u < nctr; u += 256) tickets[u * 32] = 0u;
+  if (masks)
+    for (int item = blockIdx.x; item < nsub + ntiles; item += gridDim.x) {
+      if (threadIdx.x < 2) sh_m[threadIdx.x] = 0u;
+      __syncthreads();
+      if ((int)threadIdx.x < np) {
+        if (item < nsub) {
+          const int e = ring[threadIdx.x].e_cur;
+          if (e >= 0 && (e >> 6) == item) atomicOr(&sh_m[(e >> 5) & 1], 1u << (e & 31));
+        } else {
+          const int l = ring[threadIdx.x].l - row0;
+          if (l >= 0 && (l >> 4) == item - nsub) atomicOr(&sh_m[0], 1u << (l & 15));
+        }
+      }
+      __syncthreads();
+      if (threadIdx.x == 0) {
+        if (item < nsub) { masks[2 * item] = sh_m[0]; masks[2 * item + 1] = sh_m[1]; }
+        else masks[2 * nsub + (item - nsub)] = sh_m[0];
+      }
+      __syncthreads();
+    }
   if (clk && blockIdx.x == 0 && threadIdx.x < 32) clk[threadIdx.x] = 0;
   const int tile = blockIdx.x;
   if (tile >= ntiles) return;
@@ -950,11 +972,14 @@
                                                           const double* __restrict__ prow_ring,
                                                           const LpxCtl* __restrict__ ring, int kmax, int nsub,
                                                           const double* colM,
-                                                          unsigned* tickets, int nranges) {
+                                                          unsigned* tickets, int nranges,
+                                                          const unsigned* __restrict__ masks) {
   constexpr int NG = 32, CT = 4;
   constexpr int kRsrcWord3 = 0x00020000;
   constexpr int kAuxNt = NT ? 2 : 0;
   __shared__ __attribute__((aligned(16))) double sh_b[NG * CT * 64];
+  __shared__ unsigned short sh_rm[kSweep128MaskTiles];
+  __shared__ unsigned sh_cm[2];
   __shared__ int sh_np, sh_chunk;
   const int np = ring_count128(ring, kmax, &sh_np);
   if (np < 1 && !OOP) return;
@@ -984,14 +1009,21 @@
       }
       sub_loaded = sub;
     }
+    if (OOP) {
+      for (int i = threadIdx.x; i < min(ntiles, kSweep128MaskTiles); i += 256) sh_rm[i] = masks ? (unsigned short)masks[2 * nsub + rb0 + i] : (unsigned short)0;
+      if (threadIdx.x < 2) sh_cm[threadIdx.x] = masks ? masks[2 * sub + threadIdx.x] : 0u;
+    }
     __syncthreads();
+    const unsigned cm_lo = OOP ? __builtin_amdgcn_readfirstlane(sh_cm[0]) : 0u;
+    const unsigned cm_hi = OOP ? __builtin_amdgcn_readfirstlane(sh_cm[1]) : 0u;
     if (ntiles > 0) {
       unsigned* const ctr = tickets + 32 * (1 + chunk);
       char* const dst_base = reinterpret_cast<char*>(A + sub * 64) + (int64_t)rb0 * 16 * row_bytes;
       const char* const src_base = OOP ? reinterpret_cast<const char*>(Asrc + sub * 64) + (int64_t)rb0 * 16 * row_bytes : dst_base;
       const double* const colM0 = colM + (int64_t)rb0 * 2048;
-      auto load_tile = [&](int t, d4v (&c)[CT], double (&a)[NG]) {
+      auto load_tile = [&](int t, d4v (&c)[CT], double (&a)[NG], unsigned& rmv) {
         const int tt = max(0, min(t, ntiles - 1));
+        if (OOP) rmv = sh_rm[tt & (kSweep128MaskTiles - 1)];
         const __amdgpu_buffer_rsrc_t rc = __builtin_amdgcn_make_buffer_rsrc(
             const_cast<char*>(src_base) + (int64_t)tt * 16 * row_bytes, 0, -1, kRsrcWord3);
 #pragma unroll
@@ -1009,7 +1041,7 @@
           a[2 * p + 1] = __builtin_bit_cast(double, v2u{x[2], x[3]});
         }
       };
-      auto work_tile = [&](int t, d4v (&c)[CT], const double (&a)[NG]) {
+      auto work_tile = [&](int t, d4v (&c)[CT], const double (&a)[NG], unsigned rmv) {
         const double* const bl = sh_b + lane;
 #pragma unroll
         for (int g = 0; g < NG; ++g)
@@ -1024,13 +1056,19 @@
         }
         const int tt = max(0, min(t, ntiles - 1));
         char* const out = dst_base + (int64_t)tt * 16 * row_bytes;
-        const __amdgpu_buffer_rsrc_t rd = __builtin_amdgcn_make_buffer_rsrc(out, 0, __builtin_amdgcn_readfirstlane((unsigned)t < (unsigned)ntiles ? -1 : 0), kRsrcWord3);
+        constexpr uint32_t kEnd = 0x80000000u;
+        const int nrec = (OOP && masks) ? (int)kEnd : -1;
+        const __amdgpu_buffer_rsrc_t rd = __builtin_amdgcn_make_buffer_rsrc(out, 0, __builtin_amdgcn_readfirstlane((unsigned)t < (unsigned)ntiles ? nrec : 0), kRsrcWord3);
+        const uint32_t rbits = rmv >> (lane >> 4);
+        const unsigned long long cbits = (((unsigned long long)cm_hi << 32) | cm_lo) >> (lane & 15);
 #pragma unroll
         for (int r = 0; r < 4; ++r)
 #pragma unroll
-          for (int ct = 0; ct < CT; ++ct)
-            __builtin_amdgcn_raw_buffer_store_b64(__builtin_bit_cast(v2u, (double)c[ct][r]), rd, off_c + (uint32_t)ct * 128u,
+          for (int ct = 0; ct < CT; ++ct) {
+            const uint32_t theirs = ((rbits >> (4 * r)) << 31) | ((uint32_t)(cbits >> (16 * ct)) << 31);
+            __builtin_amdgcn_raw_buffer_store_b64(__builtin_bit_cast(v2u, (double)c[ct][r]), rd, (off_c | theirs) + (uint32_t)ct * 128u,
                                                   (int)((uint32_t)(4 * r) * rb32), kAuxNt);
+          }
       };
       constexpr int kStepOps = 16 + 16 + 16;
       auto take = [&](unsigned& tk) -> int {
@@ -1039,27 +1077,28 @@
       };
       d4v c0[CT], c1[CT];
       double a0[NG], a1[NG];
+      unsigned m0 = 0u, m1 = 0u;
       unsigned ka, kb = 0;
       ticket_pull(ka, ctr);
       asm volatile("s_waitcnt vmcnt(0)" ::: "memory");
       int t0 = ticket_take(ka);
       if (t0 < ntiles) {
-        load_tile(t0, c0, a0);
+        load_tile(t0, c0, a0, m0);
         ticket_pull(ka, ctr);
         __builtin_amdgcn_s_waitcnt(0x0F70);
 #pragma unroll 1
         do {
           ticket_pull(kb, ctr);
           const int t1 = take(ka);
-          load_tile(t1, c1, a1);
+          load_tile(t1, c1, a1, m1);
           LPX_MFMA_FENCE;
-          work_tile(t0, c0, a0);
+          work_tile(t0, c0, a0, m0);
           LPX_MFMA_FENCE;
           ticket_pull(ka, ctr);
           const int t2 = take(kb);
-          load_tile(t2, c0, a0);
+          load_tile(t2, c0, a0, m0);
           LPX_MFMA_FENCE;
-          work_tile(t1, c1, a1);
+          work_tile(t1, c1, a1, m1);
           LPX_MFMA_FENCE;
           t0 = t2;
         } while (t0 < ntiles);
@@ -1113,7 +1152,8 @@
                                                      const double* __restrict__ row0_ring, int64_t mp,
                                                      const LpxCtl* __restrict__ ring, int kmax,
                                                      const double* b_src, long long* __restrict__ clk,
-                                                     double* __restrict__ img_col, double* __restrict__ img_row) {
+                                                     double* __restrict__ img_col, double* __restrict__ img_row,
+                                                     int* __restrict__ picks) {
   static_assert(kBlockMax == 128, "two words of hit ballots: lane u asks for pending pivots u and 64 + u");
   if (clk && blockIdx.x < 8 && blockIdx.y == 0 && blockIdx.z == 0 && threadIdx.x == 0) {
     const unsigned x = xcc_id() & 7u;
@@ -1126,6 +1166,8 @@
   const int s0 = blockIdx.y * kFixChunk, job = blockIdx.z;
   if ((int64_t)blockIdx.x * blockDim.x >= (job == 1 ? ld : (int64_t)m_local) || (job == 2 && s0 != 0)) return;
   const int np = ring_count128(ring, kmax, &sh_np);
+  const bool publish = picks && job != 2 && blockIdx.x == 0 && blockIdx.y == 0;
+  if (publish && np < 1 && threadIdx.x == 0) picks[job * kFixPickStride] = 0;
   if (job == 2 ? s0 != 0 : s0 >= np) return;
   if ((int)threadIdx.x < kBlockMax) {
     const bool live = (int)threadIdx.x < np;
@@ -1139,6 +1181,10 @@
   if (job != 2 && threadIdx.x < 64) fix_pick_chains(job == 1 ? sh_l : sh_e, np, sh_pick, &sh_npick);
   __syncthreads();
   const int npick = job == 2 ? 0 : sh_npick;
+  if (publish) {
+    if (threadIdx.x == 0) picks[job * kFixPickStride] = npick;
+    if ((int)threadIdx.x < npick) picks[job * kFixPickStride + 1 + threadIdx.x] = (job == 1 ? sh_l : sh_e)[sh_pick[threadIdx.x]];
+  }
   if (job != 2 && s0 >= npick) return;
   const int t = blockIdx.x * blockDim.x + threadIdx.x;
   const int ns = min(kFixChunk, npick - s0);
@@ -1292,7 +1338,7 @@
                                                              const double* __restrict__ img_col,
                                                              const double* __restrict__ img_row, int64_t mp,
                                                              const LpxCtl* __restrict__ ring, int kmax,
-                                                             long long* __restrict__ clk) {
+                                                             long long* __restrict__ clk, const int* __restrict__ picks) {
   if (clk && blockIdx.x < 8 && blockIdx.y == 0 && blockIdx.z == 0 && threadIdx.x == 0) {
     const unsigned x = xcc_id() & 7u;
     clk[x * 4 + 2] = __builtin_amdgcn_s_memtime(); clk[x * 4 + 3] = wall_clock64();
@@ -1301,6 +1347,33 @@
   __shared__ int sh_np, sh_npick;
   const int s0 = blockIdx.y * kFixChunk, job = blockIdx.z;
   if ((int64_t)blockIdx.x * blockDim.x >= (job == 1 ? ld : (int64_t)m_local)) return;
+  if (picks) {
+    const int* const pk = picks + job * kFixPickStride;
+    const int npick = min(pk[0], (int)kBlockMax);
+    if (s0 >= npick) return;
+    const int ns = min(kFixChunk, npick - s0);
+    const int t = blockIdx.x * blockDim.x + threadIdx.x;
+    int key[kFixChunk];
+    double v[kFixChunk];
+#pragma unroll
+    for (int q = 0; q < kFixChunk; ++q) key[q] = q < ns ? pk[1 + s0 + q] : -1;
+    if (job == 0) {
+      if (t >= m_local) return;
+#pragma unroll
+      for (int q = 0; q < kFixChunk; ++q) v[q] = key[q] >= 0 ? img_col[(int64_t)(s0 + q) * mp + t] : 0.0;
+#pragma unroll
+      for (int q = 0; q < kFixChunk; ++q)
+        if (key[q] >= 0 && key[q] < (int)ld) A[(int64_t)t * ld + key[q]] = v[q];
+    } else {
+      if (t >= (int)ld) return;
+#pragma unroll
+      for (int q = 0; q < kFixChunk; ++q) v[q] = (key[q] >= 0 && key[q] < m_local) ? img_row[(int64_t)(s0 + q) * ld + t] : 0.0;
+#pragma unroll
+      for (int q = 0; q < kFixChunk; ++q)
+        if (key[q] >= 0 && key[q] < m_local) A[(int64_t)key[q] * ld + t] = v[q];
+    }
+    return;
+  }
   const int np = ring_count128(ring, kmax, &sh_np);
   if (s0 >= np) return;
   if ((int)threadIdx.x < kBlockMax) {
```

After: 23980. -1.5%, worse.
